# LariWa/Fractal-Image-Compression

Measured on AMD Instinct MI355X. Metric: range-block matches/sec (8x8 R, 16x16 D, 8 iso), higher is better.
Workload: dtype u8

## Files before the change

### fractal-image-compression_amd/capi.py

```python
import ctypes as C
import os
import sys
import re

import numpy as np

_HERE = os.path.dirname(os.path.abspath(__file__))
SO_PATH = os.path.join(_HERE, "libfic_hip.so")
HEADER_PATH = os.path.join(os.path.dirname(_HERE), "include", "fic.h")

FIC_OK = 0
ERROR_NAMES = {
    -1: "FIC_E_GEOMETRY", -2: "FIC_E_WINDOW", -3: "FIC_E_ARGUMENT", -4: "FIC_E_NO_DEVICE",
    -5: "FIC_E_HIP", -6: "FIC_E_NOT_GREY", -7: "FIC_E_STATE", -8: "FIC_E_CAPACITY",
}


class FicError(Exception):

    def __init__(self, code, message):
        super().__init__(f"{ERROR_NAMES.get(code, code)}: {message}")
        self.code = code


def declared_symbols():
    text = open(HEADER_PATH).read()
    return sorted(set(re.findall(r"FIC_API\s+[\w\s\*]+?\b(fic_\w+)\s*\(", text)))


_lib = None


def _torch_first():
    t = sys.modules.get("torch")
    if t is not None:
        try:
            if t.cuda.is_available():
                t.cuda.init()
        except Exception:
            pass


def lib():
    global _lib
    if _lib is not None:
        return _lib
    so = os.environ.get("FIC_HIP_SO") or SO_PATH
    if not os.path.exists(so):
        raise FicError(-5, f"{so} is missing: build it with __graft_entry__.build() "
                           "(hipcc --offload-arch=gfx950); there is no fallback path")
    _torch_first()
    L = C.CDLL(so)
    vp, ip = C.c_void_p, C.POINTER(C.c_int)
    i32p, f32p, u8p = C.POINTER(C.c_int32), C.POINTER(C.c_float), C.POINTER(C.c_uint8)
    sig = {
        "fic_version": (C.c_char_p, []),
        "fic_last_error": (C.c_char_p, []),
        "fic_last_error_code": (C.c_int, []),
        "fic_device_count": (C.c_int, []),
        "fic_geometry": (C.c_int, [C.c_int, C.c_int, C.c_int, ip, ip, ip, ip]),
        "fic_is_greyscale_argb": (C.c_int, [i32p, C.c_int, C.c_int]),
        "fic_encode_gray_argb": (C.c_int, [i32p] + [C.c_int] * 6 + [i32p, f32p, f32p, i32p, i32p]),
        "fic_encode_gray_u8": (C.c_int, [u8p] + [C.c_int] * 6 + [i32p, f32p, f32p, i32p, i32p]),
        "fic_encode_gray_argb_multi": (C.c_int, [i32p] + [C.c_int] * 6 + [i32p, f32p, f32p, i32p, i32p]),
        "fic_encode_gray_u8_multi": (C.c_int, [u8p] + [C.c_int] * 6 + [i32p, f32p, f32p, i32p, i32p]),
        "fic_write_run_gray": (C.c_int64, [i32p, C.c_int, C.c_int, C.c_int, C.c_int, C.c_int, u8p, C.c_int64]),
        "fic_ctx_create": (vp, [C.c_int] * 7),
        "fic_ctx_destroy": (None, [vp]),
        "fic_ctx_set_gray_host": (C.c_int, [vp, u8p]),
        "fic_ctx_set_argb_host": (C.c_int, [vp, i32p]),
        "fic_ctx_set_gray_device": (C.c_int, [vp, vp]),
        "fic_ctx_encode": (C.c_int, [vp, C.c_int, C.c_int, vp]),
        "fic_ctx_sync": (C.c_int, [vp]),
        "fic_ctx_get_results_host": (C.c_int, [vp, i32p, f32p, f32p, i32p, i32p, i32p, f32p]),
        "fic_ctx_result_device_ptrs": (C.c_int, [vp] + [C.POINTER(vp)] * 7),
        "fic_ctx_records_device_ptr": (C.c_int, [vp, C.POINTER(vp)]),
        "fic_ctx_collage_host": (C.c_int, [vp, i32p]),
        "fic_encode_rgb_argb": (C.c_int, [i32p] + [C.c_int] * 5 + [i32p, f32p, f32p, f32p, f32p, i32p, i32p]),
        "fic_rgb_ctx_create": (vp, [C.c_int] * 6),
        "fic_encode_rgb_iso_argb": (C.c_int, [i32p] + [C.c_int] * 6 + [i32p, f32p, f32p, f32p, f32p, i32p, i32p, i32p]),
        "fic_rgb_ctx_create_iso": (vp, [C.c_int] * 7),
        "fic_rgb_ctx_get_iso_host": (C.c_int, [vp, i32p]),
        "fic_rgb_ctx_destroy": (None, [vp]),
        "fic_rgb_ctx_set_argb_host": (C.c_int, [vp, i32p]),
        "fic_rgb_ctx_set_argb_device": (C.c_int, [vp, vp]),
        "fic_rgb_ctx_encode": (C.c_int, [vp, C.c_int, vp]),
        "fic_rgb_ctx_sync": (C.c_int, [vp]),
        "fic_rgb_ctx_set_option": (C.c_int, [vp, C.c_char_p, C.c_int]),
        "fic_rgb_ctx_last_sweep": (C.c_int, [vp]),
        "fic_rgb_ctx_get_results_host": (C.c_int, [vp, i32p, f32p, f32p, f32p, f32p, i32p, i32p]),
        "fic_rgb_ctx_decode_host": (C.c_int, [vp, i32p, f32p, ip]),
        "fic_write_run_rgb": (C.c_int64, [i32p, C.c_int, C.c_int, C.c_int, C.c_int, C.c_int, u8p, C.c_int64]),
        "fic_decode_gray_run": (C.c_int, [u8p, C.c_int64, C.c_int, u8p, C.c_int64, ip, ip, f32p, ip]),
        "fic_ctx_decode_host": (C.c_int, [vp, u8p, f32p, ip]),
        "fic_ctx_set_option": (C.c_int, [vp, C.c_char_p, C.c_int]),
        "fic_ctx_sweep_time": (C.c_int, [vp, C.POINTER(C.c_double), ip, C.c_int]),
        "fic_ctx_info": (C.c_int, [vp, ip]),
        "fic_sweep_ranges_per_pool_read": (C.c_int, [C.c_int, C.c_int, C.c_int]),
        "fic_ctx_last_kernel": (C.c_int, [vp, C.c_char_p, C.c_int]),
        "fic_ctx_sweep_stats": (C.c_int, [vp, C.POINTER(C.c_uint64), C.c_int]),
        "fic_debug_rccl_selftest": (C.c_int, [C.c_int]),
        "fic_debug_gather_fallbacks": (C.c_int, []),
        "fic_debug_float_sum": (C.c_int, [C.c_int, C.c_float, C.POINTER(C.c_uint32), C.c_int, f32p]),
        "fic_debug_float_sum_fallbacks": (C.c_int, []),
        "fic_debug_decode_gray_run": (C.c_int, [u8p, C.c_int64, C.c_int, u8p, C.c_int64, f32p, ip, ip]),
        "fic_debug_sqrt_f64": (C.c_int, [C.c_int, C.c_uint32, C.c_uint32, C.POINTER(C.c_double)]),
        "fic_ctx_debug_pool_host": (C.c_int, [vp, u8p, C.POINTER(C.c_uint32), C.POINTER(C.c_uint32), u8p]),
        "fic_ctx_debug_q_host": (C.c_int, [vp, C.c_int, vp, C.c_int64, C.POINTER(C.c_int64)]),
        "fic_rgb_ctx_debug_q_host": (C.c_int, [vp, C.c_int, vp, C.c_int64, C.POINTER(C.c_int64)]),
        "fic_rgb_ctx_last_kernel": (C.c_int, [vp, C.c_char_p, C.c_int]),
        "fic_rgb_ctx_sweep_stats": (C.c_int, [vp, C.POINTER(C.c_uint64), C.c_int]),
        "fic_encode_gray_quadtree_u8": (C.c_int, [u8p] + [C.c_int] * 6 + [C.c_float, C.c_int, i32p, C.c_int64, ip]),
        "fic_encode_gray_quadtree_argb": (C.c_int, [i32p] + [C.c_int] * 6 + [C.c_float, C.c_int, i32p, C.c_int64, ip]),
        "fic_write_run_quadtree": (C.c_int64, [i32p] + [C.c_int] * 7 + [u8p, C.c_int64]),
        "fic_decode_quadtree_run": (C.c_int, [u8p, C.c_int64, C.c_int, u8p, C.c_int64, ip, ip, f32p, ip]),
        "fic_debug_quadtree_sse": (C.c_int, [u8p] + [C.c_int] * 7 + [C.POINTER(C.c_uint32), C.c_int64]),
        "fic_encode_rgb_quadtree_argb": (C.c_int, [i32p] + [C.c_int] * 5 + [C.c_float, C.c_int, i32p, C.c_int64, ip]),
        "fic_write_run_rgb_quadtree": (C.c_int64, [i32p] + [C.c_int] * 6 + [u8p, C.c_int64]),
        "fic_decode_rgb_quadtree_run": (C.c_int, [u8p, C.c_int64, C.c_int, i32p, C.c_int64, ip, ip, f32p, ip]),
        "fic_debug_rgb_quadtree_sse": (C.c_int, [i32p] + [C.c_int] * 6 + [C.POINTER(C.c_uint32), C.c_int64]),
        "fic_decode_gray_run_zoom": (C.c_int, [u8p, C.c_int64, C.c_int, C.c_int, u8p, C.c_int64, ip, ip, f32p, ip]),
        "fic_decode_rgb_run_zoom": (C.c_int, [u8p, C.c_int64, C.c_int, C.c_int, i32p, C.c_int64, ip, ip, f32p, ip]),
        "fic_decode_quadtree_run_zoom": (C.c_int, [u8p, C.c_int64, C.c_int, C.c_int, u8p, C.c_int64, ip, ip, f32p, ip]),
        "fic_decode_rgb_quadtree_run_zoom": (C.c_int, [u8p, C.c_int64, C.c_int, C.c_int, i32p, C.c_int64, ip, ip, f32p, ip]),
        "fic_ctx_decode_zoom_host": (C.c_int, [vp, C.c_int, u8p, f32p, ip]),
    }
    for name, (res, args) in sig.items():
        fn = getattr(L, name)
        fn.restype = res
        fn.argtypes = args
    _lib = L
    return L


def has_xcheck():
    so = os.environ.get("FIC_HIP_SO") or SO_PATH
    if not os.path.exists(so):
        return False
    return b"+xcheck" in lib().fic_version()


def last_error():
    return lib().fic_last_error().decode("utf-8", "replace")


def check(rc):
    if rc < 0:
        raise FicError(rc, last_error())
    return rc


def ptr(a, t):
    return None if a is None else a.ctypes.data_as(C.POINTER(t))


def geometry(w, h, B):
    v = [C.c_int() for _ in range(4)]
    check(lib().fic_geometry(w, h, B, *[C.byref(x) for x in v]))
    return tuple(x.value for x in v)


def _decode_run_zoom(fn, run, header_bytes, what, dtype, device, avg_error_in, zoom):
    buf = np.frombuffer(bytes(run), np.uint8)
    if buf.size < header_bytes:
        raise FicError(-3, f"{what} shorter than its header")
    z = int(zoom)
    w = int.from_bytes(bytes(run[4:8]), "big", signed=True)
    h = int.from_bytes(bytes(run[8:12]), "big", signed=True)
    cap = max(w, 0) * max(h, 0) * (z * z if z in (1, 2, 4) else 1)
    if cap >= 2 ** 31:
        cap = 0
    out = np.zeros(max(cap, 1), dtype)
    avg = C.c_float(avg_error_in)
    it, wo, ho = C.c_int(), C.c_int(), C.c_int()
    check(fn(ptr(buf, C.c_uint8), buf.size, z, device, ptr(out, C.c_uint8 if dtype == np.uint8 else C.c_int32), cap, C.byref(wo),
             C.byref(ho), C.byref(avg), C.byref(it)))
    return out[:cap], np.float32(avg.value), it.value, wo.value, ho.value


def decode_gray_run(run, device=0, avg_error_in=0.0, zoom=1):
    if zoom != 1:
        out, avg, it, w, h = _decode_run_zoom(lib().fic_decode_gray_run_zoom, run, 20, "run stream", np.uint8, device, avg_error_in, zoom)
        return out.reshape(h, w), avg, it
    buf = np.frombuffer(bytes(run), np.uint8)
    if buf.size < 20:
        raise FicError(-3, "run stream shorter than its header")
    w = int.from_bytes(bytes(run[4:8]), "big", signed=True)
    h = int.from_bytes(bytes(run[8:12]), "big", signed=True)
    cap = max(w, 0) * max(h, 0)
    out = np.zeros(max(cap, 1), np.uint8)
    avg = C.c_float(avg_error_in)
    it, wo, ho = C.c_int(), C.c_int(), C.c_int()
    check(lib().fic_decode_gray_run(ptr(buf, C.c_uint8), buf.size, device, ptr(out, C.c_uint8), cap, C.byref(wo),
                                    C.byref(ho), C.byref(avg), C.byref(it)))
    return out[:cap].reshape(h, w), np.float32(avg.value), it.value


def encode_gray_oneshot(gray, B, wK, n_iso=1, device=0):
    g = np.ascontiguousarray(gray, np.uint8)
    h, w = g.shape
    Rw, Rh, Dw, Dh = geometry(w, h, B)
    nr = Rw * Rh
    r = {"idx_local": np.zeros(nr, np.int32), "a": np.zeros(nr, np.float32), "b": np.zeros(nr, np.float32),
         "iso": np.zeros(nr, np.int32), "qrows": np.zeros((nr, 3), np.int32)}
    check(lib().fic_encode_gray_u8(ptr(g, C.c_uint8), w, h, B, Dw if wK is None else wK, n_iso, device,
                                   ptr(r["idx_local"], C.c_int32), ptr(r["a"], C.c_float), ptr(r["b"], C.c_float),
                                   ptr(r["iso"], C.c_int32), ptr(r["qrows"], C.c_int32)))
    return r


def encode_gray_multi(gray, B, wK, n_iso=1, n_gpus=1, width=None, height=None):
    if width is not None:
        g = np.ascontiguousarray(gray, np.int32).reshape(-1)
        w, h = int(width), int(height)
        if g.size != w * h:
            raise FicError(-3, "argb has the wrong number of pixels")
        fn, p = lib().fic_encode_gray_argb_multi, ptr(g, C.c_int32)
    else:
        g = np.ascontiguousarray(gray, np.uint8)
        h, w = g.shape
        fn, p = lib().fic_encode_gray_u8_multi, ptr(g, C.c_uint8)
    Rw, Rh, Dw, Dh = geometry(w, h, B)
    nr = Rw * Rh
    r = {"idx_local": np.zeros(nr, np.int32), "a": np.zeros(nr, np.float32), "b": np.zeros(nr, np.float32),
         "iso": np.zeros(nr, np.int32), "qrows": np.zeros((nr, 3), np.int32)}
    check(fn(p, w, h, B, Dw if wK is None else wK, n_iso, n_gpus, ptr(r["idx_local"], C.c_int32), ptr(r["a"], C.c_float),
             ptr(r["b"], C.c_float), ptr(r["iso"], C.c_int32), ptr(r["qrows"], C.c_int32)))
    return r


def release_cache():
    lib().fic_release_cache.restype = None
    lib().fic_release_cache()


def decode_rgb_run(run, device=0, avg_error_in=0.0, zoom=1):
    L = lib()
    if zoom != 1:
        return _decode_run_zoom(L.fic_decode_rgb_run_zoom, run, 20, "run stream", np.int32, device, avg_error_in, zoom)
    L.fic_decode_rgb_run.restype = C.c_int
    L.fic_decode_rgb_run.argtypes = [C.POINTER(C.c_uint8), C.c_int64, C.c_int, C.POINTER(C.c_int32), C.c_int64,
                                     C.POINTER(C.c_int), C.POINTER(C.c_int), C.POINTER(C.c_float), C.POINTER(C.c_int)]
    buf = np.frombuffer(bytes(run), np.uint8)
    if buf.size < 20:
        raise FicError(-3, "run stream shorter than its header")
    w = int.from_bytes(bytes(run[4:8]), "big", signed=True)
    h = int.from_bytes(bytes(run[8:12]), "big", signed=True)
    cap = max(w, 0) * max(h, 0)
    out = np.zeros(max(cap, 1), np.int32)
    avg = C.c_float(avg_error_in)
    it, wo, ho = C.c_int(), C.c_int(), C.c_int()
    check(L.fic_decode_rgb_run(ptr(buf, C.c_uint8), buf.size, device, ptr(out, C.c_int32), cap, C.byref(wo), C.byref(ho),
                               C.byref(avg), C.byref(it)))
    return out[:cap], np.float32(avg.value), it.value, w, h


def encode_rgb(argb, w, h, B, wK, device=0, want_collage=False, n_iso=1):
    Rw, Rh, Dw, Dh = geometry(w, h, B)
    nr = Rw * Rh
    argb = np.ascontiguousarray(argb, np.int32).reshape(-1)
    if argb.size != w * h:
        raise FicError(-3, "argb has the wrong number of pixels")
    r = {"idx_local": np.zeros(nr, np.int32), "a": np.zeros(nr, np.float32), "bR": np.zeros(nr, np.float32),
         "bG": np.zeros(nr, np.float32), "bB": np.zeros(nr, np.float32), "iso": np.zeros(nr, np.int32),
         "qrows": np.zeros((nr, 5), np.int32)}
    col = np.zeros(w * h, np.int32) if want_collage else None
    check(lib().fic_encode_rgb_iso_argb(ptr(argb, C.c_int32), w, h, B, wK, n_iso, device, ptr(r["idx_local"], C.c_int32),
                                        ptr(r["a"], C.c_float), ptr(r["bR"], C.c_float), ptr(r["bG"], C.c_float),
                                        ptr(r["bB"], C.c_float), ptr(r["iso"], C.c_int32), ptr(r["qrows"], C.c_int32),
                                        ptr(col, C.c_int32)))
    if want_collage:
        r["collage"] = col
    return r


class RgbEncoder:

    def __init__(self, width, height, B, wK, planes=1, device=0, n_iso=1):
        L = lib()
# ... 236 lines not shown
```

### fractal-image-compression_amd/csrc/fic_capi.cpp

```cpp
#include "fic_internal.h"

namespace ficd {

thread_local std::string g_err;
thread_local int g_err_code = 0;

int fail(int code, const char* fmt, ...)
{
    char buf[512];
    va_list ap;
    va_start(ap, fmt);
    vsnprintf(buf, sizeof(buf), fmt, ap);
    va_end(ap);
    g_err = buf;
    g_err_code = code;
    return code;
}

int check_device(int device)
{
    int ndev = fic_device_count();
    if (ndev <= 0 || device < 0 || device >= ndev) return fail(FIC_E_NO_DEVICE, "no HIP device %d (this library has no CPU path)", device);
    HIP_TRY(hipSetDevice(device));
    return FIC_OK;
// ... 183 lines not shown
    nchunks = (g.Nd + chunk_len - 1) / chunk_len;
    if (fic_launch_sweep_fast(c->b, g, tile0, ntiles, chunk_len, nchunks, s)) return fail(FIC_E_HIP, "k_sweep_fast launch failed");
    *nchunks_out = nchunks;
    return FIC_OK;
}

int d4_available(const FicGeom& g) { return g.full && g.n_iso == 8 && g.NR == 1 && fic_d4_words(g.B) > 0; }
int d4_prep(fic_ctx* c, hipStream_t s)
{
    const FicGeom& g = c->g;
    const size_t NW = (size_t)fic_d4_words(g.B), P = (size_t)g.planes;
    if (!c->d4_rng) HIP_TRY(hipMalloc((void**)&c->d4_rng, P * g.tiles * NW * 64 * 4));
    if (!c->d4_pool) HIP_TRY(hipMalloc((void**)&c->d4_pool, P * g.Nd_pad * NW * 4));
    if (fic_launch_d4_prep(c->b, c->d4_rng, c->d4_pool, g, s)) return fail(FIC_E_HIP, "k_range_d4 / k_pool_d4 launch failed");
    return FIC_OK;
}
int d4_sweep(fic_ctx* c, int tile0, int ntiles, hipStream_t s, int* nchunks_out)
{
    const FicGeom& g = c->g;
    int nchunks = valu_chunk_count(c, (long long)ntiles * g.planes);
    const int chunk_len = (g.Nd + nchunks - 1) / nchunks;
    nchunks = (g.Nd + chunk_len - 1) / chunk_len;
    if (fic_launch_sweep_d4(c->b, c->d4_rng, c->d4_pool, g, tile0, ntiles, chunk_len, nchunks, s))
        return fail(FIC_E_HIP, "k_sweep_d4 launch failed");
    *nchunks_out = nchunks;
    return FIC_OK;
}

#ifdef FIC_BUILD_XCHECK
struct MatrixCoreShape {
    bool iso8;
    bool bf16;
    int steps;
    int ndtiles, ndtiles_alloc;
    int nctiles_alloc;
    int G8, ngroups8;
    int ct1;
};
MatrixCoreShape matrix_core_shape(const FicGeom& g, int kind)
{
    MatrixCoreShape m;
    m.iso8 = g.n_iso == 8;
    m.bf16 = kind == 3 && (g.B <= 8 || g.n_iso == 8);
    m.steps = m.bf16 ? fic_bf16_steps(g.B) : (g.n <= 32 ? 1 : g.n / 32);
    m.ndtiles = (g.Nd + 31) / 32;
    m.ndtiles_alloc = m.ndtiles + 1;
    m.nctiles_alloc = g.Nr_pad / 32 + 32;
    m.G8 = m.bf16 ? fic_bf16_group8(g.B) : fic_mfma8_group(g.B);
    m.ngroups8 = (g.Nr_pad + m.G8 - 1) / m.G8;
    m.ct1 = m.bf16 ? fic_bf16_ct1(g.B) : fic_mfma1_ct(g.B);
    return m;
}
int matrix_core_prep(fic_ctx* c, int kind, hipStream_t s)
{
    const FicGeom& g = c->g;
    const MatrixCoreShape m = matrix_core_shape(g, kind);
    const size_t P = (size_t)g.planes;
    if ((c->mfma_poolB || c->mfma_rngA || c->mfma_sw || c->mfma_rconst) && c->mfma_bf16 != (int)m.bf16) {
        HIP_TRY(hipStreamSynchronize(s));
        void* old[] = {c->mfma_poolB, c->mfma_rngA, c->mfma_sw, c->mfma_rconst};
        for (void* p : old) if (p) (void)hipFree(p);
        c->mfma_poolB = c->mfma_rngA = c->mfma_sw = nullptr;
        c->mfma_rconst = nullptr;
    }
    {
        c->mfma_bf16 = (int)m.bf16;
        const size_t rtiles = m.iso8 ? (size_t)m.ngroups8 * (m.G8 / 4) : (size_t)m.nctiles_alloc;
        if (!c->mfma_poolB) HIP_TRY(hipMalloc(&c->mfma_poolB, P * m.ndtiles_alloc * m.steps * 64 * 16));
        if (!c->mfma_rngA) HIP_TRY(hipMalloc(&c->mfma_rngA, P * rtiles * m.steps * 64 * 16));
        if (!c->mfma_sw) HIP_TRY(hipMalloc(&c->mfma_sw, P * m.ndtiles_alloc * 32 * 8));
        if (!m.bf16 && !c->mfma_rconst)
            HIP_TRY(hipMalloc((void**)&c->mfma_rconst, m.iso8 ? P * rtiles * 16 * sizeof(int) : P * rtiles * 32 * 16));
    }
    if (m.bf16) {
        const int rtiles = m.iso8 ? m.ngroups8 * (m.G8 / 4) : m.nctiles_alloc;
        if (fic_launch_bf16_prep(c->b, c->mfma_poolB, c->mfma_sw, c->mfma_rngA, g, m.ndtiles_alloc, rtiles, s))
            return fail(FIC_E_HIP, "bf16 fragment prep launch failed");
    } else if (m.iso8) {
        if (fic_launch_mfma_prep_pool(c->b.pool_pix, c->mfma_poolB, g, m.ndtiles_alloc, s) ||
            fic_launch_mfma_prep_range(c->b.rng_pix, c->b.rng_st, c->mfma_rngA, c->mfma_rconst, g, m.ngroups8, s))
            return fail(FIC_E_HIP, "mfma prep launch failed");
    } else if (fic_launch_mfma1_prep(c->b, c->mfma_poolB, c->mfma_sw, c->mfma_rngA, c->mfma_rconst, g, m.ndtiles_alloc,
                                     m.nctiles_alloc, s)) {
        return fail(FIC_E_HIP, "mfma1 prep launch failed");
    }
    return FIC_OK;
}
int matrix_core_sweep(fic_ctx* c, int kind, int tile0, int tile1, hipStream_t s, int* nchunks_out)
{
    const FicGeom& g = c->g;
    const MatrixCoreShape m = matrix_core_shape(g, kind);
    const int tsz = 64 * g.NR;
    int nchunks = c->opt_chunks;
    if (nchunks <= 0) {
        const long long ranges = (long long)(tile1 - tile0) * tsz;
        const long long per_wg = m.iso8 ? m.G8 : 32LL * m.ct1;
        const long long base_wg = (ranges + per_wg - 1) / per_wg * g.planes;
        long long want = (4096 + base_wg - 1) / base_wg;
        long long cap = m.ndtiles / 256;
        if (cap < 1) cap = 1;
        long long nc = want < cap ? want : cap;
        if (base_wg * nc < 1024) {
            long long cap2 = m.ndtiles / 32;
            if (cap2 < 1) cap2 = 1;
            long long fill = (1024 + base_wg - 1) / base_wg;
            nc = fill < cap2 ? fill : cap2;
        }
        nchunks = (int)(nc < 1 ? 1 : nc);
    }
    if (nchunks > m.ndtiles) nchunks = m.ndtiles;
    const int tiles_per_chunk = (m.ndtiles + nchunks - 1) / nchunks;
    nchunks = (m.ndtiles + tiles_per_chunk - 1) / tiles_per_chunk;
    if (m.iso8) {
        const int g0 = (tile0 * tsz) / m.G8, g1 = (tile1 * tsz + m.G8 - 1) / m.G8;
        const int rc = m.bf16 ? fic_launch_sweep_bf16(c->b, c->mfma_poolB, c->mfma_sw, c->mfma_rngA, g, m.ngroups8 * (m.G8 / 4), g0,
                                                      g1 - g0, m.ndtiles, m.ndtiles_alloc, tiles_per_chunk, nchunks, s)
                              : fic_launch_sweep_mfma(c->b, c->mfma_poolB, c->mfma_rngA, c->mfma_rconst, g, m.ngroups8, g0,
                                                      g1 - g0, m.ndtiles, m.ndtiles_alloc, tiles_per_chunk, nchunks, s);
        if (rc) return fail(FIC_E_HIP, "8-isometry matrix-core sweep launch failed");
    } else {
        const int ct_begin = tile0 * (tsz / 32), ct_end = tile1 * (tsz / 32);
        const int rc = m.bf16 ? fic_launch_sweep_bf16_1(c->b, c->mfma_poolB, c->mfma_sw, c->mfma_rngA, g, ct_begin, ct_end,
                                                        m.ndtiles, m.ndtiles_alloc, m.nctiles_alloc, tiles_per_chunk, nchunks, s)
                              : fic_launch_sweep_mfma1(c->b, c->mfma_poolB, c->mfma_sw, c->mfma_rngA, c->mfma_rconst, g, ct_begin,
                                                       ct_end, m.ndtiles, m.ndtiles_alloc, m.nctiles_alloc, tiles_per_chunk,
                                                       nchunks, s);
        if (rc) return fail(FIC_E_HIP, "1-isometry matrix-core sweep launch failed");
    }
    *nchunks_out = nchunks;
    return FIC_OK;
}

#else
int matrix_core_prep(fic_ctx*, int, hipStream_t) { return fail(FIC_E_ARGUMENT, "sweep 3 / 4 (cross-check kernels) are not in this build (FIC_BUILD_XCHECK=0)"); }
int matrix_core_sweep(fic_ctx*, int, int, int, hipStream_t, int*) { return fail(FIC_E_ARGUMENT, "sweep 3 / 4 (cross-check kernels) are not in this build (FIC_BUILD_XCHECK=0)"); }
#endif
struct QShape {
    int ndtiles, ndtiles_alloc;
    int unroll;
    int CT;
    int nct_alloc;
};
QShape q_shape(const FicGeom& g)
{
    QShape q;
    q.ndtiles = (g.Nd + 31) / 32;
    q.unroll = fic_q_unroll(g.B, g.n_iso);
    q.ndtiles_alloc = q.ndtiles + 2 * q.unroll;
    q.CT = fic_q_ct(g.B);
    const int nct = g.Nr_pad * fic_q_cols_per_range(g.B, g.n_iso) / 32;
    q.nct_alloc = (nct + q.CT - 1) / q.CT * q.CT + q.CT;
    return q;
}
int q_prep(fic_ctx* c, int tile0, int tile1, hipStream_t s)
{
    const FicGeom& g = c->g;
    const QShape q = q_shape(g);
    const size_t P = (size_t)g.planes, NK = (size_t)g.n / 16;
    if (!c->q_pool) HIP_TRY(hipMalloc(&c->q_pool, P * q.ndtiles_alloc * NK * 64 * 16));
    if (!c->q_flat) HIP_TRY(hipMalloc(&c->q_flat, P * q.ndtiles_alloc * sizeof(uint32_t)));
    if (!c->q_rng) {
        HIP_TRY(hipMalloc(&c->q_rng, P * q.nct_alloc * NK * 64 * 16));
        HIP_TRY(hipMemsetAsync(c->q_rng, 0, P * q.nct_alloc * NK * 64 * 16, s));
    }
    if (!c->q_rngC) HIP_TRY(hipMalloc(&c->q_rngC, P * g.Nr_pad * fic_q_cols_per_range(g.B, g.n_iso) * g.n));
    if (!c->q_E) HIP_TRY(hipMalloc(&c->q_E, P * g.Nr_pad * sizeof(float)));
    if (!c->q_thg) HIP_TRY(hipMalloc(&c->q_thg, (P * g.Nr_pad + (size_t)2 * q.CT * 32 + 64) * sizeof(uint32_t)));
    const int tsz = 64 * g.NR;
    const int grp0 = tile0 * tsz / 64, grp1 = tile1 * tsz / 64;
    if (fic_launch_q_prep(c->b, c->q_pool, c->q_flat, c->q_rng, c->q_rngC, c->q_E, c->q_thg, g, q.ndtiles_alloc, q.nct_alloc, grp0, grp1 - grp0, s))
        return fail(FIC_E_HIP, "k_pool_q / k_range_q launch failed");
    return FIC_OK;
}
int q_sweep(fic_ctx* c, int tile0, int tile1, hipStream_t s, int* nchunks_out, bool fused_fin = false, int r_begin = 0, int r_count = 0)
{
    const FicGeom& g = c->g;
    const QShape q = q_shape(g);
    const int tsz = 64 * g.NR;
    const int cpr = fic_q_cols_per_range(g.B, g.n_iso);
    const int ct_begin = tile0 * tsz * cpr / 32, ct_end = tile1 * tsz * cpr / 32;
    int nchunks = c->opt_chunks;
    if (nchunks <= 0) {
        const long long base_wg = (long long)((ct_end - ct_begin + q.CT - 1) / q.CT) * g.planes;
        const long long resident = 256LL * fic_q_resident(g.B);
        auto ceil_div = [](long long a, long long b) { return (a + b - 1) / b; };
        const long long min_tiles = g.n_iso == 8 ? 30 : 14;
        long long fill = base_wg < resident ? ceil_div(2 * resident, base_wg) : 1;
        if (fill > q.ndtiles / min_tiles) fill = q.ndtiles / min_tiles;
        long long bal = ceil_div(8 * resident, base_wg);
        if (bal > q.ndtiles / 1024) bal = q.ndtiles / 1024;
        const long long nc = fill > bal ? fill : bal;
        nchunks = (int)(nc < 1 ? 1 : nc);
    }
    if (nchunks > q.ndtiles) nchunks = q.ndtiles;
    int tiles_per_chunk = (q.ndtiles + nchunks - 1) / nchunks;
    tiles_per_chunk = (tiles_per_chunk + q.unroll - 1) / q.unroll * q.unroll;
    nchunks = (q.ndtiles + tiles_per_chunk - 1) / tiles_per_chunk;
    if (fused_fin && !c->q_fin) {
        const size_t nfin = (size_t)g.planes * (q.nct_alloc / q.CT + 1);
        HIP_TRY(hipMalloc((void**)&c->q_fin, nfin * sizeof(unsigned int)));
        HIP_TRY(hipMemsetAsync(c->q_fin, 0, nfin * sizeof(unsigned int), s));
    }
    if (fic_launch_sweep_q(c->b, c->q_pool, c->q_flat, c->q_rng, c->q_rngC, c->q_E, c->q_thg, g, ct_begin, ct_end, q.ndtiles, q.ndtiles_alloc,
                           q.nct_alloc, tiles_per_chunk, nchunks, s, c->q_stats, c->opt_noflag, fused_fin ? &c->o : nullptr, c->q_fin,
                           r_begin, r_count))
        return fail(FIC_E_HIP, "k_sweep_q launch failed");
    *nchunks_out = nchunks;
    c->last_tiles_per_chunk = tiles_per_chunk;
    return FIC_OK;
}

}

extern "C" {

#ifdef FIC_BUILD_XCHECK
const char* fic_version(void) { return "fic-hip 0.3 (gfx950, +xcheck sweeps)"; }
#else
const char* fic_version(void) { return "fic-hip 0.3 (gfx950)"; }
#endif
const char* fic_last_error(void) { return g_err.c_str(); }
int fic_last_error_code(void) { return g_err_code; }

int fic_device_count(void)
{
    int n = 0;
    if (hipGetDeviceCount(&n) != hipSuccess) return 0;
    return n;
}

int fic_geometry(int w, int h, int B, int* Rw, int* Rh, int* Dw, int* Dh)
{
    FicGeom g;
    int rc = make_geometry(w, h, B, 1, 1, 1, &g);
    if (rc) return rc;
    if (Rw) *Rw = g.Rw;
    if (Rh) *Rh = g.Rh;
    if (Dw) *Dw = g.Dw;
    if (Dh) *Dh = g.Dh;
    return FIC_OK;
}

int fic_is_greyscale_argb(const int32_t* argb, int w, int h)
{
    if (!argb || w <= 0 || h <= 0) return fail(FIC_E_ARGUMENT, "fic_is_greyscale_argb: bad argument");
    size_t n = (size_t)w * h;
    for (size_t i = 0; i < n; i++) {
        int r = (argb[i] >> 16) & 0xff, g = (argb[i] >> 8) & 0xff, b = argb[i] & 0xff;
        if (r != g || g != b) return 0;
    }
    return 1;
}

int64_t fic_write_run_gray(const int32_t* qrows, int n_ranges, int w, int h, int B, int wK, uint8_t* out,
                           int64_t capacity)
{
    if (!qrows || !out || n_ranges < 0) return fail(FIC_E_ARGUMENT, "fic_write_run_gray: bad argument");
    int64_t need = 20 + 12 * (int64_t)n_ranges;
    if (capacity < need) return fail(FIC_E_CAPACITY, "fic_write_run_gray: need %lld bytes, have %lld", (long long)need, (long long)capacity);
    const int32_t hdr[5] = {0, w, h, B, wK};
    for (int i = 0; i < 5; i++) put_be32(out + 4 * i, hdr[i]);
    uint8_t* p = out + 20;
    for (int64_t i = 0; i < 3 * (int64_t)n_ranges; i++, p += 4) put_be32(p, qrows[i]);
    return need;
}

fic_ctx* fic_ctx_create(int device, int w, int h, int B, int wK, int n_iso, int planes)
{
    FicGeom g;
    if (make_geometry(w, h, B, wK, n_iso, planes, &g)) return nullptr;
    int ndev = fic_device_count();
    if (ndev <= 0) { fail(FIC_E_NO_DEVICE, "no HIP device visible (this library has no CPU path)"); return nullptr; }
    if (device < 0 || device >= ndev) { fail(FIC_E_NO_DEVICE, "device %d out of range (0..%d)", device, ndev - 1); return nullptr; }
    if (hipSetDevice(device) != hipSuccess) { fail(FIC_E_HIP, "hipSetDevice(%d) failed", device); return nullptr; }
    fic_ctx* c = new fic_ctx();
    c->device = device;
    c->g = g;
    memset(&c->b, 0, sizeof(c->b));
    memset(&c->o, 0, sizeof(c->o));
    const size_t P = (size_t)planes;
    int rc = FIC_OK;
    auto A = [&](int r) { if (rc == FIC_OK) rc = r; };
    A(dev_alloc(&c->b.scaled, P * g.Ws * g.Hs));
    A(dev_alloc(&c->b.pool_pix, P * g.Nd_pad * g.n));
    A(dev_alloc(&c->b.pool_st, P * g.Nd_pad));
    A(dev_alloc(&c->b.pool_var, P * g.Nd_pad));
    A(dev_alloc(&c->b.pool_s64, P * g.Nd_pad));
    A(dev_alloc(&c->b.rng_st, P * g.Nr_pad));
    A(dev_alloc(&c->b.key, P * g.Nr_pad));
    A(dev_alloc(&c->o.idx_local, P * g.Nr));
    A(dev_alloc(&c->o.idx_global, P * g.Nr));
    A(dev_alloc(&c->o.iso, P * g.Nr));
    A(dev_alloc(&c->o.a, P * g.Nr));
    A(dev_alloc(&c->o.b, P * g.Nr));
    A(dev_alloc(&c->o.err, P * g.Nr));
    A(dev_alloc(&c->o.qrows, P * g.Nr * 3));
    A(dev_alloc(&c->o.records, P * g.Nr * 6));
    if (rc == FIC_OK) {
        hipError_t e = hipMemset(c->b.pool_pix, 0, P * g.Nd_pad * g.n);
        if (e == hipSuccess) e = hipMemset(c->b.pool_st, 0, P * g.Nd_pad * sizeof(FicDomStat));
        if (e == hipSuccess) e = hipMemset(c->b.pool_var, 0, P * g.Nd_pad * sizeof(uint32_t));
        if (e == hipSuccess) e = hipMemset(c->b.pool_s64, 0, P * g.Nd_pad * sizeof(double));
        if (e == hipSuccess) e = hipStreamSynchronize(nullptr);
        if (e != hipSuccess) rc = fail(FIC_E_HIP, "hipMemset: %s", hipGetErrorString(e));
    }
    if (rc != FIC_OK) {
        ctx_free_all(c);
        delete c;
        return nullptr;
    }
    return c;
}

void fic_ctx_destroy(fic_ctx* c)
{
    if (!c) return;
    (void)hipSetDevice(c->device);
    (void)hipDeviceSynchronize();
    ctx_free_all(c);
    delete c;
}

int fic_ctx_set_gray_host(fic_ctx* c, const uint8_t* gray)
{
    if (!c || !gray) return fail(FIC_E_ARGUMENT, "fic_ctx_set_gray_host: null argument");
    std::lock_guard<std::mutex> lk(c->mu);
    HIP_TRY(hipSetDevice(c->device));
    size_t bytes = (size_t)c->g.planes * c->g.W * c->g.H;
    if (!c->gray_own) { int rc = dev_alloc(&c->gray_own, bytes); if (rc) return rc; }
    HIP_TRY(hipStreamSynchronize(c->last_stream));
    HIP_TRY(hipMemcpy(c->gray_own, gray, bytes, hipMemcpyHostToDevice));
    c->b.gray = c->gray_own;
    c->have_input = true;
    return FIC_OK;
}

int fic_ctx_set_argb_host(fic_ctx* c, const int32_t* argb)
{
    if (!c || !argb) return fail(FIC_E_ARGUMENT, "fic_ctx_set_argb_host: null argument");
    std::lock_guard<std::mutex> lk(c->mu);
    HIP_TRY(hipSetDevice(c->device));
    size_t npix = (size_t)c->g.planes * c->g.W * c->g.H;
    if (!c->gray_own) { int rc = dev_alloc(&c->gray_own, npix); if (rc) return rc; }
    if (!c->argb_stage) { int rc = dev_alloc(&c->argb_stage, npix); if (rc) return rc; }
    HIP_TRY(hipStreamSynchronize(c->last_stream));
    HIP_TRY(hipMemcpy(c->argb_stage, argb, npix * sizeof(int32_t), hipMemcpyHostToDevice));
    if (fic_launch_argb_to_gray(c->argb_stage, c->gray_own, npix, nullptr)) return fail(FIC_E_HIP, "k_argb_to_gray launch failed");
    HIP_TRY(hipStreamSynchronize(nullptr));
    c->b.gray = c->gray_own;
    c->have_input = true;
    return FIC_OK;
}

int fic_ctx_set_gray_device(fic_ctx* c, const void* dev_gray)
{
    if (!c || !dev_gray) return fail(FIC_E_ARGUMENT, "fic_ctx_set_gray_device: null argument");
    std::lock_guard<std::mutex> lk(c->mu);
    c->b.gray = (uint8_t*)dev_gray;
    c->have_input = true;
    return FIC_OK;
}

int fic_ctx_encode(fic_ctx* c, int range_begin, int range_count, void* hip_stream)
{
    if (!c) return fail(FIC_E_ARGUMENT, "fic_ctx_encode: null context");
    std::lock_guard<std::mutex> lk(c->mu);
    if (!c->have_input) return fail(FIC_E_STATE, "fic_ctx_encode: no input image set");
    const FicGeom& g = c->g;
    if (range_count < 0) range_count = g.Nr - range_begin;
    if (range_begin < 0 || range_count < 0 || range_begin + range_count > g.Nr)
        return fail(FIC_E_ARGUMENT, "fic_ctx_encode: range span [%d,%d) outside 0..%d", range_begin, range_begin + range_count, g.Nr);
    HIP_TRY(hipSetDevice(c->device));
    hipStream_t s = (hipStream_t)hip_stream;
    c->last_stream = s;
    if (range_count == 0) return FIC_OK;

    int kind = c->opt_sweep;
    if (kind == 0) {
        const long long pairs = (long long)g.planes * range_count * g.Nd;
        const int valu = d4_available(g) ? 5 : 2;
        kind = !g.full ? 1 : ((pairs >= 2000000LL && g.Nd < (1 << 24)) ? 6 : valu);
        const char* env = getenv("FIC_SWEEP");
        if (env && env[0] >= '2' && env[0] <= '6' && env[1] == '\0' && g.full) {
            const int want = env[0] - '0';
            kind = want == 5 ? valu : want;
        }
    }
    if (kind >= 2 && !g.full) return fail(FIC_E_ARGUMENT, "fast sweep needs full search (wK == Dw == Dh)");
#ifndef FIC_BUILD_XCHECK
    if (kind == 3 || kind == 4) return fail(FIC_E_ARGUMENT, "sweep %d (cross-check kernel) is not in this build (FIC_BUILD_XCHECK=0)", kind);
#endif
    if (kind == 5 && !d4_available(g)) return fail(FIC_E_ARGUMENT, "sweep 5 (k_sweep_d4) needs full search, n_iso = 8 and B = 8");
    if (kind == 6 && g.Nd >= (1 << 24)) return fail(FIC_E_ARGUMENT, "sweep 6 (k_sweep_q) needs a pool of fewer than 2^24 blocks");
    const int tsz = 64 * g.NR;
    const int tile0 = range_begin / tsz;
    const int tile1 = (range_begin + range_count + tsz - 1) / tsz;
    const int ntiles = tile1 - tile0;
    int nchunks = 1;
    int rc = FIC_OK;
    bool fused_prep = false;
    if (kind == 6) {
        const QShape q = q_shape(g);
        fused_prep = fic_q_prep_fused(g, q.ndtiles_alloc, tile1 * (64 * g.NR) / 64 - tile0 * (64 * g.NR) / 64) != 0;
    }
    if (!fused_prep && fic_launch_scale(c->b.gray, c->b.scaled, g, s)) return fail(FIC_E_HIP, "k_scale launch failed");
    if (kind == 6) {
        rc = q_prep(c, tile0, tile1, s);
    } else {
        if (fic_launch_pool(c->b.scaled, c->b.pool_pix, c->b.pool_st, c->b.pool_var, c->b.pool_s64, g, s))
            return fail(FIC_E_HIP, "k_pool launch failed");
        if (kind != 5 && !c->b.rng_pix) {
            int rca = dev_alloc(&c->b.rng_pix, (size_t)g.planes * g.Nr_pad * g.n_iso * g.DW);
            if (rca) return rca;
        }
        if (fic_launch_range(c->b.gray, c->b.rng_pix, c->b.rng_st, g, s, kind == 5 ? 0 : 1)) return fail(FIC_E_HIP, "k_range launch failed");
        HIP_TRY(hipMemset2DAsync(c->b.key + (size_t)tile0 * tsz, (size_t)g.Nr_pad * sizeof(unsigned long long), 0xFF,
                                 (size_t)ntiles * tsz * sizeof(unsigned long long), (size_t)g.planes, s));
        if (kind == 5) rc = d4_prep(c, s);
        else if (kind >= 3) rc = matrix_core_prep(c, kind, s);
    }
    if (rc == FIC_OK) rc = time_begin(c, s);
    if (rc == FIC_OK) {
        if (kind == 1) {
            if (fic_launch_sweep_generic(c->b, g, range_begin, range_count, s)) rc = fail(FIC_E_HIP, "k_sweep_generic launch failed");
        } else if (kind == 6) {
            rc = q_sweep(c, tile0, tile1, s, &nchunks, fused_prep, range_begin, range_count);
        } else if (kind == 5) {
            rc = d4_sweep(c, tile0, tile1 - tile0, s, &nchunks);
        } else if (kind >= 3) {
            rc = matrix_core_sweep(c, kind, tile0, tile1, s, &nchunks);
        } else {
            rc = valu_sweep(c, tile0, tile1 - tile0, s, &nchunks);
        }
    }
    if (rc == FIC_OK) rc = time_end(c, s);
    if (rc != FIC_OK) return rc;
    c->last_chunks = nchunks;
    c->last_kind = kind;
    c->last_fused = fused_prep ? 1 : 0;
    if (!fused_prep &&
        fic_launch_finalize(c->b, c->o, g, range_begin, range_count, s, (kind == 5 || kind == 6) ? 1 : 0)) return fail(FIC_E_HIP, "k_finalize launch failed");
    c->encoded_any = true;
    return FIC_OK;
}

int fic_ctx_sync(fic_ctx* c)
{
    if (!c) return fail(FIC_E_ARGUMENT, "fic_ctx_sync: null context");
    HIP_TRY(hipSetDevice(c->device));
    HIP_TRY(hipStreamSynchronize(c->last_stream));
    return FIC_OK;
}

int fic_ctx_get_results_host(fic_ctx* c, int32_t* idx_local, float* a, float* b, int32_t* iso, int32_t* qrows,
                             int32_t* idx_global, float* err)
{
    if (!c) return fail(FIC_E_ARGUMENT, "fic_ctx_get_results_host: null context");
    if (!c->encoded_any) return fail(FIC_E_STATE, "fic_ctx_get_results_host: nothing encoded yet");
    HIP_TRY(hipSetDevice(c->device));
    HIP_TRY(hipStreamSynchronize(c->last_stream));
    size_t n = (size_t)c->g.planes * c->g.Nr;
    if (n > (size_t)65536) {
        if (idx_local) HIP_TRY(hipMemcpy(idx_local, c->o.idx_local, n * 4, hipMemcpyDeviceToHost));
        if (a) HIP_TRY(hipMemcpy(a, c->o.a, n * 4, hipMemcpyDeviceToHost));
        if (b) HIP_TRY(hipMemcpy(b, c->o.b, n * 4, hipMemcpyDeviceToHost));
        if (iso) HIP_TRY(hipMemcpy(iso, c->o.iso, n * 4, hipMemcpyDeviceToHost));
        if (qrows) HIP_TRY(hipMemcpy(qrows, c->o.qrows, n * 12, hipMemcpyDeviceToHost));
    } else if (idx_local || a || b || iso || qrows) {
        std::lock_guard<std::mutex> lk(c->mu);
        if (!c->host_rec) HIP_TRY(hipHostMalloc((void**)&c->host_rec, n * 6 * sizeof(int32_t), hipHostMallocDefault));
        HIP_TRY(hipMemcpy(c->host_rec, c->o.records, n * 6 * sizeof(int32_t), hipMemcpyDeviceToHost));
        const int32_t* r = c->host_rec;
        for (size_t i = 0; i < n; i++, r += 6) {
            if (idx_local) idx_local[i] = r[0];
            if (a) memcpy(&a[i], &r[1], 4);
            if (b) memcpy(&b[i], &r[2], 4);
            if (iso) iso[i] = r[3];
            if (qrows) { qrows[3 * i] = r[0]; qrows[3 * i + 1] = r[4]; qrows[3 * i + 2] = r[5]; }
        }
    }
    if (idx_global) HIP_TRY(hipMemcpy(idx_global, c->o.idx_global, n * 4, hipMemcpyDeviceToHost));
    if (err) HIP_TRY(hipMemcpy(err, c->o.err, n * 4, hipMemcpyDeviceToHost));
    return FIC_OK;
}

int fic_ctx_result_device_ptrs(fic_ctx* c, void** idx_local, void** a, void** b, void** iso, void** qrows,
                               void** idx_global, void** err)
{
    if (!c) return fail(FIC_E_ARGUMENT, "fic_ctx_result_device_ptrs: null context");
    if (idx_local) *idx_local = c->o.idx_local;
    if (a) *a = c->o.a;
    if (b) *b = c->o.b;
    if (iso) *iso = c->o.iso;
    if (qrows) *qrows = c->o.qrows;
    if (idx_global) *idx_global = c->o.idx_global;
    if (err) *err = c->o.err;
    return FIC_OK;
}

int fic_ctx_records_device_ptr(fic_ctx* c, void** records)
{
    if (!c || !records) return fail(FIC_E_ARGUMENT, "fic_ctx_records_device_ptr: null argument");
    *records = c->o.records;
    return FIC_OK;
}

int fic_ctx_collage_host(fic_ctx* c, int32_t* argb_out)
{
    if (!c || !argb_out) return fail(FIC_E_ARGUMENT, "fic_ctx_collage_host: null argument");
    std::lock_guard<std::mutex> lk(c->mu);
    if (!c->encoded_any) return fail(FIC_E_STATE, "fic_ctx_collage_host: nothing encoded yet");
    HIP_TRY(hipSetDevice(c->device));
    size_t npix = (size_t)c->g.planes * c->g.W * c->g.H;
    if (!c->collage) { int rc = dev_alloc(&c->collage, npix); if (rc) return rc; }
    if (fic_launch_collage(c->b, c->o, c->collage, c->g, c->last_stream)) return fail(FIC_E_HIP, "k_collage launch failed");
    HIP_TRY(hipStreamSynchronize(c->last_stream));
    HIP_TRY(hipMemcpy(argb_out, c->collage, npix * sizeof(int32_t), hipMemcpyDeviceToHost));
    return FIC_OK;
}

int fic_ctx_set_option(fic_ctx* c, const char* name, int value)
{
    if (!c || !name) return fail(FIC_E_ARGUMENT, "fic_ctx_set_option: null argument");
    if (!strcmp(name, "sweep")) {
        if (value < 0 || value > 6)
            return fail(FIC_E_ARGUMENT, "sweep must be 0 (auto), 1 (generic), 2 (fast, VALU), 3 (matrix-core, exact covariances), 4 (matrix-core, i8 operands), 5 (VALU, group-Fourier isometries) or 6 (matrix-core, normalised f16 prune GEMM)");
        c->opt_sweep = value;
    } else if (!strcmp(name, "chunks")) {
        if (value < 0) return fail(FIC_E_ARGUMENT, "chunks must be >= 0");
        c->opt_chunks = value;
    } else if (!strcmp(name, "q_shape")) {
        if (value < 0 || value > 2) return fail(FIC_E_ARGUMENT, "q_shape must be 0 (by pool size), 1 (16x16x32) or 2 (32x32x16)");
        c->g.q_shape = value;
    } else if (!strcmp(name, "q_eshift")) {
        if (value < -12 || value > 4) return fail(FIC_E_ARGUMENT, "q_eshift must be in -12..4");
        c->g.q_eshift = value;
    } else if (!strcmp(name, "q_noflag")) {
        c->opt_noflag = value ? 1 : 0;
    } else if (!strcmp(name, "time_sweep")) {
        c->opt_time = value ? 1 : 0;
    } else if (!strcmp(name, "sweep_stats")) {
        HIP_TRY(hipSetDevice(c->device));
        if (value && !c->q_stats) {
            HIP_TRY(hipMalloc((void**)&c->q_stats, 8 * sizeof(unsigned long long)));
            HIP_TRY(hipMemset(c->q_stats, 0, 8 * sizeof(unsigned long long)));
            HIP_TRY(hipStreamSynchronize(nullptr));
        } else if (!value && c->q_stats) {
            HIP_TRY(hipStreamSynchronize(c->last_stream));
            (void)hipFree(c->q_stats);
            c->q_stats = nullptr;
        }
    } else {
        return fail(FIC_E_ARGUMENT, "unknown option '%s'", name);
    }
    return FIC_OK;
}

int fic_ctx_sweep_time(fic_ctx* c, double* total_ms, int* launches, int reset)
{
    if (!c) return fail(FIC_E_ARGUMENT, "fic_ctx_sweep_time: null context");
    std::lock_guard<std::mutex> lk(c->mu);
    HIP_TRY(hipSetDevice(c->device));
    int rc = flush_events(c);
    if (rc) return rc;
    if (total_ms) *total_ms = c->acc_ms;
    if (launches) *launches = c->acc_n;
    if (reset) { c->acc_ms = 0.0; c->acc_n = 0; }
    return FIC_OK;
}

int fic_ctx_sweep_stats(fic_ctx* c, uint64_t* out8, int reset)
{
    if (!c || !out8) return fail(FIC_E_ARGUMENT, "fic_ctx_sweep_stats: null argument");
    std::lock_guard<std::mutex> lk(c->mu);
    if (!c->q_stats) return fail(FIC_E_STATE, "fic_ctx_sweep_stats: set the option \"sweep_stats\" first");
    HIP_TRY(hipSetDevice(c->device));
    HIP_TRY(hipStreamSynchronize(c->last_stream));
    HIP_TRY(hipMemcpy(out8, c->q_stats, 8 * sizeof(uint64_t), hipMemcpyDeviceToHost));
    if (reset) {
        HIP_TRY(hipMemset(c->q_stats, 0, 8 * sizeof(uint64_t)));
        HIP_TRY(hipStreamSynchronize(nullptr));
    }
    return FIC_OK;
}

int fic_ctx_info(fic_ctx* c, int* out10)
{
    if (!c || !out10) return fail(FIC_E_ARGUMENT, "fic_ctx_info: null argument");
    const FicGeom& g = c->g;
    int v[10] = {g.Rw, g.Rh, g.Nr, g.Dw, g.Dh, g.Nd, g.NR, g.tiles, c->last_chunks, c->last_kind};
    memcpy(out10, v, sizeof(v));
    return FIC_OK;
}

int fic_ctx_last_kernel(fic_ctx* c, char* out, int capacity)
{
    if (!c || !out || capacity < 1) return fail(FIC_E_ARGUMENT, "fic_ctx_last_kernel: bad argument");
    const FicGeom& g = c->g;
    const int NK = g.n / 16, kind = c->last_kind;
    const char* multi = c->last_chunks > 1 ? "true" : "false";
    const bool shorts = kind == 6 && fic_q_multi_kind(c->last_chunks, c->last_tiles_per_chunk) == 2;
    char buf[96];
    if (kind == 6 && fic_q_shape16(g) && shorts) snprintf(buf, sizeof(buf), "k_sweep_q16s<%d>", NK);
    else if (kind == 6 && fic_q_shape16(g)) snprintf(buf, sizeof(buf), "k_sweep_q16<%d, %s>", NK, multi);
    else if (kind == 6 && shorts) snprintf(buf, sizeof(buf), "k_sweep_qs<%d, %d>", NK, g.n_iso == 1 ? 0 : (g.B == 4 ? 1 : 2));
    else if (kind == 6) snprintf(buf, sizeof(buf), "k_sweep_q<%d, %d, %s>", NK, g.n_iso == 1 ? 0 : (g.B == 4 ? 1 : 2), multi);
    else if (kind == 5) snprintf(buf, sizeof(buf), "k_sweep_d4");
    else if (kind == 2) snprintf(buf, sizeof(buf), "k_sweep_fast");
    else if (kind == 1) snprintf(buf, sizeof(buf), "k_sweep_generic");
    else if (kind == 3 || kind == 4) {
        const bool bf16 = kind == 3 && (g.B <= 8 || g.n_iso == 8);
        snprintf(buf, sizeof(buf), "%s%s", bf16 ? "k_sweep_bf16" : "k_sweep_mfma", g.n_iso == 8 ? "" : (bf16 ? "_1" : "1"));
    } else snprintf(buf, sizeof(buf), "(none)");
    snprintf(out, (size_t)capacity, "%s%s", buf, kind == 6 && c->last_fused ? " after k_prep_q8, finalising" : "");
    return FIC_OK;
}

int fic_sweep_ranges_per_pool_read(int kind, int B, int n_iso)
{
    if ((B != 4 && B != 8 && B != 16) || (n_iso != 1 && n_iso != 8)) return 0;
    if (kind == 6) return fic_q_ctw_host(B) * 32 / fic_q_cols_per_range(B, n_iso);
    if (kind == 2 || kind == 5) {
        int NR = 1, NC = 1;
        fic_fast_variant(B, n_iso, &NR, &NC);
        return 64 * (kind == 5 ? 1 : NR);
    }
    return 0;
}

int fic_debug_sqrt_f64(int device, uint32_t first, uint32_t count, double* out)
{
    if (!out || count == 0) return fail(FIC_E_ARGUMENT, "fic_debug_sqrt_f64: bad argument");
    int rc = check_device(device);
    if (rc) return rc;
    double* d = nullptr;
    HIP_TRY(hipMalloc((void**)&d, (size_t)count * sizeof(double)));
    if (fic_launch_sqrt_probe(d, first, count, nullptr)) rc = fail(FIC_E_HIP, "k_sqrt_probe launch failed");
    if (rc == FIC_OK) {
        hipError_t e = hipMemcpy(out, d, (size_t)count * sizeof(double), hipMemcpyDeviceToHost);
        if (e != hipSuccess) rc = fail(FIC_E_HIP, "hipMemcpy: %s", hipGetErrorString(e));
    }
    (void)hipFree(d);
    return rc;
}

int fic_ctx_debug_pool_host(fic_ctx* c, uint8_t* pix, uint32_t* sum, uint32_t* var, uint8_t* scaled)
{
    if (!c) return fail(FIC_E_ARGUMENT, "fic_ctx_debug_pool_host: null context");
    if (!c->encoded_any) return fail(FIC_E_STATE, "fic_ctx_debug_pool_host: nothing encoded yet");
    HIP_TRY(hipSetDevice(c->device));
    HIP_TRY(hipStreamSynchronize(c->last_stream));
    const FicGeom& g = c->g;
    for (int p = 0; p < g.planes; p++) {
        if (pix)
            HIP_TRY(hipMemcpy(pix + (size_t)p * g.Nd * g.n, c->b.pool_pix + (size_t)p * g.Nd_pad * g.n, (size_t)g.Nd * g.n,
                              hipMemcpyDeviceToHost));
        if (var)
            HIP_TRY(hipMemcpy(var + (size_t)p * g.Nd, c->b.pool_var + (size_t)p * g.Nd_pad, (size_t)g.Nd * 4,
                              hipMemcpyDeviceToHost));
        if (sum) {
            std::vector<FicDomStat> st(g.Nd);
            HIP_TRY(hipMemcpy(st.data(), c->b.pool_st + (size_t)p * g.Nd_pad, (size_t)g.Nd * sizeof(FicDomStat),
                              hipMemcpyDeviceToHost));
            for (int i = 0; i < g.Nd; i++) sum[(size_t)p * g.Nd + i] = st[i].sum;
        }
    }
    if (scaled) HIP_TRY(hipMemcpy(scaled, c->b.scaled, (size_t)g.planes * g.Ws * g.Hs, hipMemcpyDeviceToHost));
    return FIC_OK;
}

int fic_ctx_debug_q_host(fic_ctx* c, int which, void* out, int64_t capacity, int64_t* size)
{
    if (!c || !size) return fail(FIC_E_ARGUMENT, "fic_ctx_debug_q_host: null argument");
    if (!c->encoded_any || !c->q_pool) return fail(FIC_E_STATE, "fic_ctx_debug_q_host: no encode through the default sweep (\"sweep\" = 6) yet");
    const FicGeom& g = c->g;
    const QShape q = q_shape(g);
    const size_t P = (size_t)g.planes, NK = (size_t)g.n / 16;
    const void* src = nullptr;
    size_t bytes = 0;
    switch (which) {
    case 0: src = c->q_pool; bytes = P * q.ndtiles_alloc * NK * 64 * 16; break;
    case 1: src = c->q_flat; bytes = P * q.ndtiles_alloc * sizeof(uint32_t); break;
    case 2: src = c->q_rng; bytes = P * q.nct_alloc * NK * 64 * 16; break;
    case 3: src = c->q_E; bytes = P * g.Nr_pad * sizeof(float); break;
    case 4: src = c->b.rng_st; bytes = P * g.Nr_pad * sizeof(FicRngStat); break;
    case 5: src = c->q_rngC; bytes = P * g.Nr_pad * fic_q_cols_per_range(g.B, g.n_iso) * g.n; break;
    default: return fail(FIC_E_ARGUMENT, "fic_ctx_debug_q_host: which must be 0..5");
    }
    *size = (int64_t)bytes;
    if (!out) return FIC_OK;
    if (capacity < (int64_t)bytes) return fail(FIC_E_CAPACITY, "fic_ctx_debug_q_host: %zu bytes needed", bytes);
    HIP_TRY(hipSetDevice(c->device));
    HIP_TRY(hipStreamSynchronize(c->last_stream));
    HIP_TRY(hipMemcpy(out, src, bytes, hipMemcpyDeviceToHost));
    return FIC_OK;
}

}

int ficd::encode_oneshot(const uint8_t* gray, const int32_t* argb, int w, int h, int B, int wK, int n_iso, int device,
                          int32_t* idx_local, float* a, float* b, int32_t* iso, int32_t* qrows)
{
    if ((!gray && !argb) || !idx_local || !a || !b) return fail(FIC_E_ARGUMENT, "fic_encode_gray: null argument");
    fic_ctx* c = cache_take(device, w, h, B, wK, n_iso);
    if (!c) c = fic_ctx_create(device, w, h, B, wK, n_iso, 1);
    if (!c) return g_err_code ? g_err_code : FIC_E_HIP;
    int rc = gray ? fic_ctx_set_gray_host(c, gray) : fic_ctx_set_argb_host(c, argb);
    if (rc == FIC_OK) rc = fic_ctx_encode(c, 0, -1, nullptr);
    if (rc == FIC_OK) rc = fic_ctx_get_results_host(c, idx_local, a, b, iso, qrows, nullptr, nullptr);
    ErrKeep keep;
    if (rc == FIC_OK) cache_give(c);
    else fic_ctx_destroy(c);
    return rc;
}

extern "C" {

void fic_release_cache(void)
{
    std::vector<fic_ctx*> drop;
    {
        std::lock_guard<std::mutex> lk(g_cache_mu);
        drop.swap(g_cache);
    }
    for (fic_ctx* c : drop) fic_ctx_destroy(c);
    release_rgb_cache();
    release_comms();
    release_decoder_arenas();
}

int fic_encode_gray_argb(const int32_t* argb, int w, int h, int B, int wK, int n_iso, int device, int32_t* idx_local,
                         float* a, float* b, int32_t* iso, int32_t* qrows)
{
    return encode_oneshot(nullptr, argb, w, h, B, wK, n_iso, device, idx_local, a, b, iso, qrows);
}

int fic_encode_gray_u8(const uint8_t* gray, int w, int h, int B, int wK, int n_iso, int device, int32_t* idx_local,
                       float* a, float* b, int32_t* iso, int32_t* qrows)
{
    return encode_oneshot(gray, nullptr, w, h, B, wK, n_iso, device, idx_local, a, b, iso, qrows);
}

}
```

### fractal-image-compression_amd/csrc/fic_internal.h

```cpp
#pragma once
#include <hip/hip_runtime.h>
#include <stdarg.h>
#include <stdio.h>
#include <stdlib.h>
#include <string.h>
#include <functional>
#include <mutex>
#include <string>
#include <vector>

#include "../../include/fic.h"
#include "fic_device.h"
#include "fic_launch.h"

namespace ficd {

extern thread_local std::string g_err;
extern thread_local int g_err_code;
int fail(int code, const char* fmt, ...) __attribute__((format(printf, 2, 3)));

#define HIP_TRY(expr)                                                                              \
    do {                                                                                           \
        hipError_t e_ = (expr);                                                                    \
        if (e_ != hipSuccess) return ficd::fail(FIC_E_HIP, "%s: %s", #expr, hipGetErrorString(e_)); \
    } while (0)

struct ErrKeep {
    std::string msg = g_err;
    int code = g_err_code;
    ~ErrKeep() { g_err = msg; g_err_code = code; }
};

int make_geometry(int w, int h, int B, int wK, int n_iso, int planes, FicGeom* out);
int make_decode_geometry(int w, int h, int B, int wK, int n_iso, int planes, int zoom, FicGeom* out);

template <typename T>
int dev_alloc(T** p, size_t count)
{
    HIP_TRY(hipMalloc((void**)p, count * sizeof(T)));
    return FIC_OK;
}
inline size_t align256(size_t v) { return (v + 255) & ~(size_t)255; }

int check_device(int device);

inline void put_be32(uint8_t* p, int32_t v)
{
    uint32_t u = (uint32_t)v;
    p[0] = (uint8_t)(u >> 24); p[1] = (uint8_t)(u >> 16); p[2] = (uint8_t)(u >> 8); p[3] = (uint8_t)u;
}
inline int32_t get_be32(const uint8_t* p)
{
    return (int32_t)(((uint32_t)p[0] << 24) | ((uint32_t)p[1] << 16) | ((uint32_t)p[2] << 8) | (uint32_t)p[3]);
}

fic_ctx* cache_take(int device, int w, int h, int B, int wK, int n_iso);
void cache_give(fic_ctx* c);
int encode_oneshot(const uint8_t* gray, const int32_t* argb, int w, int h, int B, int wK, int n_iso, int device,
                   int32_t* idx_local, float* a, float* b, int32_t* iso, int32_t* qrows);

fic_rgb_ctx* rgb_cache_take(int device, int w, int h, int B, int wK, int n_iso = 1);
void rgb_cache_give(fic_rgb_ctx* c);
void rgb_ctx_views(const fic_rgb_ctx* c, const int32_t** argb, const int32_t** scaled, const int32_t** qrows5);

struct Arena {
    int device = -1;
    size_t bytes = 0;
    char* base = nullptr;
};
int arena_take(int device, size_t bytes, Arena* out);
void arena_give(const Arena& a);
struct DecodeKind {
    size_t px_bytes;
    uint32_t px_start;
    const char* name;
    const char* paint_line;
};
constexpr DecodeKind kDecodeGrey{1, 128u, "decode", "FC:394"}, kDecodeRgb{4, 0xff808080u, "decodeRGB", "FC:477"};
int decode_loop(const DecodeKind& kind, int planes, size_t npix, void* d_image, FicDecodeState* d_state, const float* avg_in,
                float* avg_out, int* iters_out, int* seq_out, hipStream_t s, const std::function<int(int)>& iteration);

void release_decoder_arenas();
void release_rgb_cache();
void release_comms();

}

struct fic_ctx {
    int device = 0;
    FicGeom g;
    FicBuffers b;
    FicOutputs o;
    uint8_t* gray_own = nullptr;
    int32_t* argb_stage = nullptr;
    int32_t* collage = nullptr;
    int32_t* host_rec = nullptr;
    uint8_t* decoded = nullptr;
    FicDecodeState* dec_state = nullptr;
    uint32_t* dec_sq = nullptr;
    void* mfma_poolB = nullptr;
    void* mfma_rngA = nullptr;
    void* mfma_sw = nullptr;
    int* mfma_rconst = nullptr;
    int mfma_bf16 = 0;
    void* q_pool = nullptr;
    void* q_flat = nullptr;
    void* q_rng = nullptr;
    void* q_rngC = nullptr;
    void* q_E = nullptr;
    void* q_thg = nullptr;
    unsigned int* q_fin = nullptr;
    unsigned long long* q_stats = nullptr;
    uint32_t* d4_rng = nullptr;
    uint32_t* d4_pool = nullptr;
    bool have_input = false;
    bool encoded_any = false;
    hipStream_t last_stream = nullptr;
    hipStream_t own_stream = nullptr;
    int opt_sweep = 0, opt_chunks = 0, opt_time = 0, opt_noflag = 0;
    int last_chunks = 0, last_kind = 0, last_fused = 0, last_tiles_per_chunk = 0;
    std::vector<hipEvent_t> ev;
    double acc_ms = 0.0;
    int acc_n = 0;
    std::mutex mu;
};
```

### fractal-image-compression_amd/csrc/fic_launch.h

```cpp
#pragma once
#include <hip/hip_runtime.h>
#include <stdint.h>
#include "fic_device.h"

struct FicBuffers {
    uint8_t* gray;
    uint8_t* scaled;
    uint8_t* pool_pix;
    FicDomStat* pool_st;
    uint32_t* pool_var;
    double* pool_s64;
    uint32_t* rng_pix;
    FicRngStat* rng_st;
    unsigned long long* key;
};

struct FicOutputs {
    int32_t* idx_local;
    int32_t* idx_global;
    int32_t* iso;
    float* a;
    float* b;
    float* err;
    int32_t* qrows;
    int32_t* records;
};

#ifdef __HIPCC__
#include "fic_devfn.h"
__device__ __forceinline__ void finalize_store(const FicOutputs& out, const FicGeom& g, int plane, int j, unsigned long long kk, int wloc,
                                               int gi, int k, uint32_t acc, FicDomStat ds, FicRngStat rs, uint32_t varu)
{
    int dM = (int)(ds.sum >> g.lgn);
    int cov = (int)acc - rs.rM * (int)ds.sum - dM * rs.rem;
    float var = (float)varu;
    float a = __fdiv_rn((float)cov, var);
    if (a < -1.0f) a = -1.0f;
    else if (a > 1.0f) a = 1.0f;
    float b = __fsub_rn((float)rs.rM, __fmul_rn(a, (float)dM));
    size_t o = (size_t)plane * g.Nr + j;
    const int qa = java_f2i(__fmul_rn(a, 100.0f)), qb = java_f2i(b);
    out.qrows[3 * o + 0] = wloc;
    out.qrows[3 * o + 1] = qa;
    out.qrows[3 * o + 2] = qb;
    if (a != a) a = __uint_as_float(0x7FC00000u);
    if (b != b) b = __uint_as_float(0x7FC00000u);
    out.idx_local[o] = wloc;
    out.idx_global[o] = gi;
    out.iso[o] = k;
    out.a[o] = a;
    out.b[o] = b;
    out.err[o] = f32_from_orderable((uint32_t)(kk >> 32));
    int32_t* rec = out.records + 6 * o;
    rec[0] = wloc;
    rec[1] = (int32_t)__float_as_uint(a);
    rec[2] = (int32_t)__float_as_uint(b);
    rec[3] = k;
    rec[4] = qa;
    rec[5] = qb;
}
#endif

int fic_launch_argb_to_gray(const int32_t* argb, uint8_t* gray, size_t npix, hipStream_t s);
int fic_launch_scale(const uint8_t* gray, uint8_t* scaled, const FicGeom& g, hipStream_t s);
int fic_launch_pool(const uint8_t* scaled, uint8_t* pool_pix, FicDomStat* st, uint32_t* var, double* s64,
                    const FicGeom& g, hipStream_t s);
int fic_launch_range(const uint8_t* gray, uint32_t* rng_pix, FicRngStat* rst, const FicGeom& g, hipStream_t s,
                     int with_copies = 1);
int fic_launch_sweep_generic(const FicBuffers& b, const FicGeom& g, int r_begin, int r_count, hipStream_t s);
int fic_fast_variant(int B, int n_iso, int* NR, int* NC);
int fic_launch_sweep_fast(const FicBuffers& b, const FicGeom& g, int tile0, int ntiles, int chunk_len, int nchunks,
                          hipStream_t s);
int fic_launch_finalize(const FicBuffers& b, const FicOutputs& out, const FicGeom& g, int r_begin, int r_count,
                        hipStream_t s, int from_gray = 0);
int fic_launch_collage(const FicBuffers& b, const FicOutputs& out, int32_t* collage, const FicGeom& g, hipStream_t s);
int fic_launch_sqrt_probe(double* out, uint32_t first, uint32_t count, hipStream_t s);

struct FicRgbOutputs {
    int32_t* idx_local;
    int32_t* idx_global;
    float* a;
    float* bR;
    float* bG;
    float* bB;
    int32_t* qrows;
    int32_t* iso = nullptr;
};
struct FicRgbBuffers {
    int32_t* argb;
    int32_t* scaled;
    uint16_t* pool_sum;
    float* pool_cf;
    FicRgbDomStat* pool_st;
    int16_t* rng_t;
    FicRgbRngStat* rng_st;
    unsigned long long* key;
};
struct FicRgbQ {
    void *poolQ = nullptr, *dflat = nullptr, *rngQ = nullptr, *qst = nullptr, *rngE = nullptr, *theta_g = nullptr, *amax = nullptr;
    int ndtiles = 0, ndtiles_alloc = 0, nct_alloc = 0, tiles_per_chunk = 0, nchunks = 0;
    unsigned long long* stats = nullptr;
};
int fic_launch_rgb_encode(const FicRgbBuffers& b, const FicRgbOutputs& out, int32_t* collage, const FicGeom& g,
                          hipStream_t s, const FicRgbQ* q = nullptr);
int fic_launch_rgbq(const uint16_t* pool_sum, const FicRgbDomStat* pool_st, const int16_t* rng_t, const FicRgbRngStat* rng_st,
                    unsigned long long* key, void* poolQ, void* dflat, void* rngQ, void* qst, void* rngE, void* theta_g, void* amax,
                    const FicGeom& g, int ndtiles, int ndtiles_alloc, int nct_alloc, int tiles_per_chunk, int nchunks, hipStream_t s,
                    unsigned long long* stats = nullptr);

int fic_mfma8_group(int B);
int fic_launch_mfma_prep_pool(const uint8_t* pool_pix, void* poolB, const FicGeom& g, int ndtiles_alloc, hipStream_t s);
int fic_launch_mfma_prep_range(const uint32_t* rng_pix, const FicRngStat* rng_st, void* rngA, int* rconst,
                               const FicGeom& g, int ngroups, hipStream_t s);
int fic_launch_sweep_mfma(const FicBuffers& b, const void* poolB, const void* rngA, const int* rconst, const FicGeom& g,
                          int ngroups, int group0, int ngroups_launch, int ndtiles, int ndtiles_alloc, int tiles_per_chunk,
                          int nchunks, hipStream_t s);
int fic_mfma1_ct(int B);
int fic_launch_mfma1_prep(const FicBuffers& b, void* poolA, void* pool_sw, void* rngB, void* rconst, const FicGeom& g,
                          int ndtiles_alloc, int nctiles_alloc, hipStream_t s);
int fic_launch_sweep_mfma1(const FicBuffers& b, const void* poolA, const void* pool_sw, const void* rngB,
                           const void* rconst, const FicGeom& g, int ct_begin, int ct_end, int ndtiles, int ndtiles_alloc,
                           int nctiles_alloc, int tiles_per_chunk, int nchunks, hipStream_t s);
int fic_bf16_steps(int B);
int fic_bf16_group8(int B);
int fic_bf16_ct1(int B);
int fic_launch_bf16_prep(const FicBuffers& b, void* poolF, void* pool_w, void* rngF, const FicGeom& g, int ndtiles_alloc,
                         int nrtiles_alloc, hipStream_t s);
int fic_launch_sweep_bf16(const FicBuffers& b, const void* poolF, const void* pool_w, const void* rngF, const FicGeom& g,
                          int nrtiles_alloc, int group0, int ngroups_launch, int ndtiles, int ndtiles_alloc, int tiles_per_chunk, int nchunks,
                          hipStream_t s);
int fic_launch_sweep_bf16_1(const FicBuffers& b, const void* poolF, const void* pool_w, const void* rngF, const FicGeom& g,
                            int ct_begin, int ct_end, int ndtiles, int ndtiles_alloc, int nctiles_alloc, int tiles_per_chunk,
                            int nchunks, hipStream_t s);
int fic_d4_words(int B);
int fic_launch_d4_prep(const FicBuffers& b, uint32_t* rng_d4, uint32_t* pool_d4, const FicGeom& g, hipStream_t s);
int fic_launch_sweep_d4(const FicBuffers& b, const uint32_t* rng_d4, const uint32_t* pool_d4, const FicGeom& g, int tile0,
                        int ntiles, int chunk_len, int nchunks, hipStream_t s);
int fic_q_ct(int B);
int fic_q_ctw_host(int B);
int fic_q_prep_fused(const FicGeom& g, int ndtiles_alloc, int ngrp);
int fic_q_shape16(const FicGeom& g);
int fic_q_multi_kind(int nchunks, int tiles_per_chunk);
int fic_q_cols_per_range(int B, int n_iso);
int fic_q_unroll(int B, int n_iso);
int fic_q_resident(int B);
int fic_launch_q_prep(const FicBuffers& b, void* poolQ, void* dflat, void* rngQ, void* rngC, void* rngE, void* theta_g,
                      const FicGeom& g, int ndtiles_alloc, int nct_alloc, int grp0, int ngrp, hipStream_t s);
int fic_launch_sweep_q(const FicBuffers& b, const void* poolQ, const void* dflat, const void* rngQ, const void* rngC, const void* rngE,
                       void* theta_g, const FicGeom& g, int ct_begin, int ct_end, int ndtiles, int ndtiles_alloc,
                       int nct_alloc, int tiles_per_chunk, int nchunks, hipStream_t s, unsigned long long* stats = nullptr, int dbg_noflag = 0,
                       const FicOutputs* fin_out = nullptr, unsigned int* fin_count = nullptr, int r_begin = 0, int r_count = 0);
int fic_launch_decode_iteration_rgb(int32_t* scaled, int32_t* image, const int32_t* qrows5, FicDecodeState* state,
                                    uint32_t* sqbuf, int counter, const FicGeom& g, hipStream_t s,
                                    const int32_t* iso = nullptr);
int fic_launch_scale_rgb(const int32_t* argb, int32_t* scaled, const FicGeom& g, hipStream_t s);

int fic_launch_float_sum_probe(float carry, const uint32_t* vals, int count, uint32_t* maps, float* out2, hipStream_t s);
size_t fic_float_sum_map_words(size_t count);
size_t fic_decode_sq_words(size_t planes, size_t wh);
int fic_launch_decode_step(FicDecodeState* state, uint32_t* sqbuf, int counter, int wh, int planes, hipStream_t s);
int fic_launch_decode_iteration(uint8_t* scaled, uint8_t* image, const int32_t* qrows, const int32_t* iso,
                                FicDecodeState* state, uint32_t* sqbuf, int counter, const FicGeom& g, hipStream_t s);

struct QtGrey {
    using Px = uint8_t;
    static constexpr int QW = 3;
    static constexpr bool kIso = true;
    static constexpr int kLeafInts = 3 + QW + 1;
};
struct QtRgb {
    using Px = int32_t;
    static constexpr int QW = 5;
    static constexpr bool kIso = false;
    static constexpr int kLeafInts = 3 + QW;
};
struct FicQtLeaf {
    int32_t x, y, gi, sqoff, q[4];
};
template <typename Fmt>
int fic_launch_leaf_sse(const typename Fmt::Px* image, const typename Fmt::Px* scaled, const int32_t* qrows, const int32_t* iso,
                        uint32_t* sse, const FicGeom& g, hipStream_t s);
template <typename Fmt>
int fic_launch_qt_compact(const uint32_t* const* sse, const int32_t* const* qrows, const int32_t* const* iso, const int* Rw,
                          int nl, int B_max, int Rw_top, int Ntop, float threshold, int* counts, int* offs, int32_t* leaves,
                          hipStream_t s);
template <typename Fmt>
int fic_launch_decode_paint_leaves(const typename Fmt::Px* scaled, typename Fmt::Px* image, const FicQtLeaf* lv, int n,
                                   FicDecodeState* state, uint32_t* sqbuf, int counter, const FicGeom& g, hipStream_t s);
```

### fractal-image-compression_amd/csrc/fic_q.hip

```cpp
#include <hip/hip_runtime.h>
#include <stdint.h>
#include <math.h>
#include <string.h>
#include <stdlib.h>
#include <type_traits>
#include "fic_device.h"
#include "fic_launch.h"
#include "fic_devfn.h"

typedef int v4i __attribute__((ext_vector_type(4)));
typedef float v16f __attribute__((ext_vector_type(16)));
typedef _Float16 f16x8 __attribute__((ext_vector_type(8)));

#define FIC_Q_LEVEL 0.99999237060546875f
#define FIC_Q_TAU_ALL 3.0e38f
#define FIC_Q_TAU_NONE (-1.0f)
#define FIC_Q_LMIN 0.26f
#define FIC_Q_ECOEF 7.0e-4f
#define FIC_Q_EABS 1.6e-5f
#define FIC_Q_QCAP 1280
#define FIC_Q_QFLUSH 256

#ifndef FIC_Q_CTW_B8
#define FIC_Q_CTW_B8 4
#endif
#ifndef FIC_Q_CTW_B4
#define FIC_Q_CTW_B4 8
#endif
#ifndef FIC_Q_WPG
#define FIC_Q_WPG 4
#endif
#ifndef FIC_Q_WAVES_B8
#define FIC_Q_WAVES_B8 2
#endif
#ifndef FIC_Q_WAVES_B4
#define FIC_Q_WAVES_B4 3
#endif
__host__ __device__ constexpr int fic_q_ctw(int NK) { return NK == 4 ? FIC_Q_CTW_B8 : (NK < 4 ? FIC_Q_CTW_B4 : 2); }
#define FIC_Q_THG_NONE 0xBF800000u
#ifndef FIC_Q_GFAST_TILES
#define FIC_Q_GFAST_TILES 48
#endif
#ifndef FIC_Q_SEED
#define FIC_Q_SEED 1
#endif
#define FIC_Q_UNROLL 2

#ifndef FIC_Q_SHAPE16
#define FIC_Q_SHAPE16 1
#endif
__device__ __forceinline__ void frag_slot(int shape16, int NK, int s, int lane, int& row, int& p0)
{
    if (!shape16) {
        row = lane & 31;
        p0 = 16 * s + 8 * (lane >> 5);
    } else {
        const int KS = NK >> 1;
        row = 16 * (s / KS) + (lane & 15);
        p0 = 32 * (s % KS) + 8 * (lane >> 4);
    }
}

__device__ __forceinline__ float q_escale(const FicGeom& g) { return __int_as_float((127 - g.q_eshift) << 23); }

__device__ __forceinline__ int f16_pair(float lo, float hi)
{
    typedef _Float16 h2 __attribute__((ext_vector_type(2)));
    h2 v = {(_Float16)lo, (_Float16)hi};
    return __builtin_bit_cast(int, v);
}

template <int B, bool FUSE>
__device__ __forceinline__ void pool_q_body(int dtile, int plane, const uint8_t* __restrict__ scaled_in, const uint8_t* __restrict__ gray,
                                            uint8_t* __restrict__ scaled_out, uint8_t* __restrict__ pool_pix,
                                            FicDomStat* __restrict__ pool_st, uint32_t* __restrict__ pool_var,
                                            double* __restrict__ pool_s64, v4i* __restrict__ poolQ,
                                            uint32_t* __restrict__ dflat, const FicGeom& g, int ndtiles_alloc, int folded, int shape16)
{
    __shared__ __attribute__((aligned(16))) uint8_t pix[32][256 + 16];
    __shared__ int s_sum[32][16], s_sq[32][16];
    __shared__ float s_w[32];
    __shared__ int s_mean[32];
    __shared__ int s_nonflat;
    constexpr int n = B * B, NK = n / 16;
    if (threadIdx.x == 0) s_nonflat = 0;
    for (int t = threadIdx.x; t < 32 * B; t += 256) {
        const int i = t / B, ry = t % B;
        const int d = dtile * 32 + i;
        uint32_t w[B / 4];
#pragma unroll
        for (int q = 0; q < B / 4; q++) w[q] = 0u;
        if (d < g.Nd) {
            const int c = d % g.Dw, r = d / g.Dw;
            const size_t so = (size_t)plane * g.Ws * g.Hs + (size_t)(r * g.abstand + ry) * g.Ws + c * g.abstand;
            if constexpr (!FUSE) {
                __builtin_memcpy(w, scaled_in + so, B);
            } else {
                const int ys = r * g.abstand + ry, xs0 = c * g.abstand;
                const uint8_t* im = gray + (size_t)plane * g.W * g.H + (size_t)(2 * ys) * g.W + 2 * xs0;
                uint32_t top[B / 2], bot[B / 2];
                __builtin_memcpy(top, im, 2 * B);
                __builtin_memcpy(bot, im + g.W, 2 * B);
#pragma unroll
                for (int x = 0; x < B; x++) {
                    const uint32_t t2 = top[x >> 1] >> (16 * (x & 1)), b2 = bot[x >> 1] >> (16 * (x & 1));
                    const int tap4 = (2 * (xs0 + x) + 1 >= g.H) ? 128 : (int)((b2 >> 8) & 0xffu);
                    const int m = (int)(t2 & 0xffu) + (int)((t2 >> 8) & 0xffu) + (int)(b2 & 0xffu) + tap4;
                    w[x >> 2] |= (uint32_t)(m / 4) << (8 * (x & 3));
                }
                __builtin_memcpy(scaled_out + so, w, B);
            }
        }
        uint32_t sum = 0, sq = 0;
#pragma unroll
        for (int q = 0; q < B / 4; q++) {
            sum = __builtin_amdgcn_sad_u8(w[q], 0u, sum);
            sq = __builtin_amdgcn_udot4(w[q], w[q], sq, false);
            *(uint32_t*)&pix[i][ry * B + 4 * q] = w[q];
        }
        s_sum[i][ry] = (int)sum;
        s_sq[i][ry] = (int)sq;
    }
    __syncthreads();
    for (int t = threadIdx.x; t < 32 * n / 16; t += 256) {
        const int i = t / (n / 16), q = t % (n / 16);
        const int d = dtile * 32 + i;
        if (d < g.Nd) *(uint4*)(pool_pix + ((size_t)plane * g.Nd_pad + d) * n + 16 * q) = *(const uint4*)&pix[i][16 * q];
    }
    if (threadIdx.x < 32) {
        const int i = threadIdx.x, d = dtile * 32 + i;
        int S = 0, Q = 0;
        for (int t = 0; t < B; t++) { S += s_sum[i][t]; Q += s_sq[i][t]; }
        const int m = S >> g.lgn;
        const int var = Q - 2 * m * S + n * m * m;
        const double s64 = __dsqrt_rn((double)var);
        const float s32 = (float)s64;
        float w = 0.0f;
        if (d < g.Nd) {
            const size_t o = (size_t)plane * g.Nd_pad + d;
            FicDomStat st;
            st.sum = (uint32_t)S;
            st.s32 = s32;
            pool_st[o] = st;
            pool_var[o] = (uint32_t)var;
            pool_s64[o] = s64;
            if (var != 0) { w = __fdiv_rn(1.0f, s32); atomicOr(&s_nonflat, 1); }
        }
        s_w[i] = w;
        s_mean[i] = m;
    }
    __syncthreads();
    for (int t = threadIdx.x; t < NK * 64; t += 256) {
        const int lane = t & 63, m = t >> 6;
        int i, pos0;
        frag_slot(shape16, NK, m, lane, i, pos0);
        const int h = lane >> 5;
        const float w = s_w[i];
        const int dM = s_mean[i];
        v4i v;
        if (!folded) {
            const uint2 pw = *(const uint2*)&pix[i][pos0];
            int px[8];
#pragma unroll
            for (int u = 0; u < 8; u++) px[u] = (int)(((u < 4 ? pw.x : pw.y) >> (8 * (u & 3))) & 0xffu);
#pragma unroll
            for (int u = 0; u < 4; u++)
                v[u] = f16_pair(__fmul_rn((float)(px[2 * u] - dM), w), __fmul_rn((float)(px[2 * u + 1] - dM), w));
        } else {
            const bool odd = m >= NK / 2;
            const int p0 = 16 * (odd ? m - NK / 2 : m) + 8 * h;
            const uint2 pw = *(const uint2*)&pix[i][p0], qw = *(const uint2*)&pix[i][n - 8 - p0];
            float f[8];
#pragma unroll
            for (int u = 0; u < 8; u++) {
                const int a = (int)(((u < 4 ? pw.x : pw.y) >> (8 * (u & 3))) & 0xffu);
                const int b = (int)(((u < 4 ? qw.y : qw.x) >> (8 * (3 - (u & 3)))) & 0xffu);
                f[u] = __fmul_rn(__fmul_rn((float)(odd ? a - b : a + b - 2 * dM), w), 0.5f);
            }
#pragma unroll
            for (int u = 0; u < 4; u++) v[u] = f16_pair(f[2 * u], f[2 * u + 1]);
        }
        poolQ[((size_t)plane * ndtiles_alloc + dtile) * NK * 64 + t] = v;
    }
    if (threadIdx.x == 0) dflat[(size_t)plane * ndtiles_alloc + dtile] = s_nonflat ? 0u : 1u;
}
template <int B>
__global__ __launch_bounds__(256) void k_pool_q(const uint8_t* __restrict__ scaled, uint8_t* __restrict__ pool_pix,
                                                FicDomStat* __restrict__ pool_st, uint32_t* __restrict__ pool_var,
                                                double* __restrict__ pool_s64, v4i* __restrict__ poolQ,
                                                uint32_t* __restrict__ dflat, FicGeom g, int ndtiles_alloc, int folded, int shape16)
{
    pool_q_body<B, false>(blockIdx.x, blockIdx.y, scaled, nullptr, nullptr, pool_pix, pool_st, pool_var, pool_s64, poolQ, dflat, g,
                          ndtiles_alloc, folded, shape16);
}

__global__ __launch_bounds__(256) void k_range_q(const uint8_t* __restrict__ gray, FicRngStat* __restrict__ rng_st,
                                                 float* __restrict__ rngE, unsigned long long* __restrict__ key,
                                                 uint32_t* __restrict__ theta_g, v4i* __restrict__ rngQ,
                                                 uint32_t* __restrict__ rngC, FicGeom g, int nct_alloc, int grp0, int mode,
                                                 int staged, int shape16)
{
    __shared__ __attribute__((aligned(16))) uint8_t blk[64 * (256 + 4)];
    extern __shared__ __attribute__((aligned(16))) uint8_t cpy[];
    __shared__ int s_rM[64];
    const int plane = blockIdx.y;
    const int grp = grp0 + blockIdx.x;
    const int B = g.B, n = g.n, DW = g.DW, NK = n / 16;
    const int lgB = B == 4 ? 2 : (B == 8 ? 3 : 4);
    const int stride = n + 4;
    const int j0 = grp * 64;
    const uint8_t* img = gray + (size_t)plane * g.W * g.H;
    for (int i = threadIdx.x; i < 64 * DW; i += 256) {
        const int l = i / DW, wd = i % DW;
        const int j = j0 + l;
        uint32_t v = 0;
        if (j < g.Nr) {
            const int pos = wd * 4;
            const uint8_t* p = img + (size_t)((j / g.Rw) * B + (pos >> lgB)) * g.W + (j % g.Rw) * B + (pos & (B - 1));
            v = *(const uint32_t*)p;
        }
        *(uint32_t*)&blk[l * stride + wd * 4] = v;
    }
    __syncthreads();
    {
        const int l = threadIdx.x >> 2, part = threadIdx.x & 3;
        const uint32_t* w = (const uint32_t*)(blk + l * stride) + part * (DW / 4);
        uint32_t S = 0, Q = 0;
        for (int i = 0; i < DW / 4; i++) {
            S = __builtin_amdgcn_sad_u8(w[i], 0u, S);
            Q = __builtin_amdgcn_udot4(w[i], w[i], Q, false);
        }
        S += (uint32_t)__builtin_amdgcn_update_dpp(0, (int)S, 0xB1, 0xF, 0xF, true);
        Q += (uint32_t)__builtin_amdgcn_update_dpp(0, (int)Q, 0xB1, 0xF, 0xF, true);
        S += (uint32_t)__builtin_amdgcn_update_dpp(0, (int)S, 0x4E, 0xF, 0xF, true);
        Q += (uint32_t)__builtin_amdgcn_update_dpp(0, (int)Q, 0x4E, 0xF, 0xF, true);
        const int j = j0 + l;
        const int rM = (int)(S >> g.lgn);
        if (part == 0) {
            s_rM[l] = rM;
            if (j < g.Nr_pad) {
                const int ss = (int)Q - 2 * rM * (int)S + n * rM * rM;
                const size_t o = (size_t)plane * g.Nr_pad + j;
                FicRngStat st;
                st.rM = j < g.Nr ? rM : 0;
                st.rem = j < g.Nr ? (int)S - (rM << g.lgn) : 0;
                rng_st[o] = st;
                rngE[o] = __fmul_rn(__fadd_rn(__fmul_rn(__fsqrt_rn((float)ss), FIC_Q_ECOEF), FIC_Q_EABS), q_escale(g));
                key[o] = FIC_KEY_NONE;
                theta_g[o] = FIC_Q_THG_NONE;
            }
        }
    }
    __syncthreads();
    const int cpr = mode == 0 ? 1 : (mode == 1 ? 8 : 4);
    const int lgc = mode == 0 ? 0 : (mode == 1 ? 3 : 2);
    const int cols = 64 * cpr;
    const int ct0 = (j0 * cpr) / 32;
    const int cstride = n + 8;
    for (int t = threadIdx.x; t < cols * DW; t += 256) {
        const int col = t / DW, wd = t % DW;
        const int l = col >> lgc, c = col & (cpr - 1);
        if (j0 + l >= g.Nr_pad) break;
        const int k = mode == 2 ? (c == 0 ? 0 : (c == 1 ? 1 : (c == 2 ? 4 : 6))) : c;
        int ax, bx, cx, ay, by, cy;
        iso_affine(iso_inverse(k), B - 1, ax, bx, cx, ay, by, cy);
        const int s0 = cx + cy * B, sx = ax + ay * B, sy = bx + by * B;
        const uint8_t* b = blk + l * stride;
        uint32_t w = 0;
        if (k == 0) {
            w = *(const uint32_t*)(b + 4 * wd);
        } else {
#pragma unroll
            for (int u = 0; u < 4; u++) {
                const int p = 4 * wd + u;
                w |= (uint32_t)b[s0 + sx * (p & (B - 1)) + sy * (p >> lgB)] << (8 * u);
            }
        }
        rngC[((size_t)plane * g.Nr_pad * cpr + (size_t)j0 * cpr + col) * DW + wd] = w;
        if (staged) *(uint32_t*)(cpy + col * cstride + 4 * wd) = w;
    }
    if (staged) __syncthreads();
    for (int t = threadIdx.x; t < (cols / 32) * NK * 64; t += 256) {
        const int lane = t & 63, m = (t >> 6) % NK, ctl = (t >> 6) / NK;
        int c32, pos0;
        frag_slot(shape16, NK, m, lane, c32, pos0);
        const int col = ctl * 32 + c32, h = lane >> 5;
        const int l = col >> lgc, c = col & (cpr - 1);
        const int rM = s_rM[l];
        const bool real = j0 + l < g.Nr;
        int a[8];
        if (staged) {
            const uint8_t* cp = cpy + col * cstride;
            if (mode != 2) {
                const uint2 w = *(const uint2*)(cp + pos0);
#pragma unroll
                for (int u = 0; u < 8; u++) a[u] = (int)(((u < 4 ? w.x : w.y) >> (8 * (u & 3))) & 0xffu) - rM;
            } else {
                const bool odd = m >= NK / 2;
                const int q0 = 16 * (odd ? m - NK / 2 : m) + 8 * h;
                const uint2 w = *(const uint2*)(cp + q0), v = *(const uint2*)(cp + n - 8 - q0);
#pragma unroll
                for (int u = 0; u < 8; u++) {
                    const int c0 = (int)(((u < 4 ? w.x : w.y) >> (8 * (u & 3))) & 0xffu);
                    const int c1 = (int)(((u < 4 ? v.y : v.x) >> (8 * (3 - (u & 3)))) & 0xffu);
                    a[u] = odd ? c0 - c1 : c0 + c1 - 2 * rM;
                }
            }
        } else {
            const int k = mode == 2 ? (c == 0 ? 0 : (c == 1 ? 1 : (c == 2 ? 4 : 6))) : c;
            int ax, bx, cx, ay, by, cy;
            iso_affine(iso_inverse(k), B - 1, ax, bx, cx, ay, by, cy);
            const int s0 = cx + cy * B, sx = ax + ay * B, sy = bx + by * B;
            const uint8_t* b = blk + l * stride;
            if (mode != 2) {
                const int p0 = pos0;
#pragma unroll
                for (int u = 0; u < 8; u++) {
                    const int p = p0 + u;
                    a[u] = (int)b[s0 + sx * (p & (B - 1)) + sy * (p >> lgB)] - rM;
                }
            } else {
                const bool odd = m >= NK / 2;
                const int q0 = 16 * (odd ? m - NK / 2 : m) + 8 * h;
#pragma unroll
                for (int u = 0; u < 8; u++) {
                    const int p = q0 + u, pr = n - 1 - p;
                    const int c0 = b[s0 + sx * (p & (B - 1)) + sy * (p >> lgB)], c1 = b[s0 + sx * (pr & (B - 1)) + sy * (pr >> lgB)];
                    a[u] = odd ? c0 - c1 : c0 + c1 - 2 * rM;
                }
            }
        }
        v4i v;
#pragma unroll
        for (int u = 0; u < 4; u++) v[u] = real ? f16_pair((float)a[2 * u], (float)a[2 * u + 1]) : 0;
        if (ct0 + ctl < nct_alloc) rngQ[((size_t)plane * nct_alloc + ct0 + ctl) * NK * 64 + (size_t)m * 64 + lane] = v;
    }
}

__device__ __forceinline__ void t4x4_bytes(uint32_t a, uint32_t b, uint32_t c, uint32_t d, uint32_t& o0, uint32_t& o1, uint32_t& o2, uint32_t& o3)
{
    const uint32_t t0 = __builtin_amdgcn_perm(b, a, 0x06020400u), t1 = __builtin_amdgcn_perm(b, a, 0x07030501u);
    const uint32_t t2 = __builtin_amdgcn_perm(d, c, 0x06020400u), t3 = __builtin_amdgcn_perm(d, c, 0x07030501u);
    o0 = __builtin_amdgcn_perm(t2, t0, 0x05040100u);
    o1 = __builtin_amdgcn_perm(t3, t1, 0x05040100u);
    o2 = __builtin_amdgcn_perm(t2, t0, 0x07060302u);
    o3 = __builtin_amdgcn_perm(t3, t1, 0x07060302u);
}
__device__ __forceinline__ void b8_transpose(const uint32_t (&r)[16], uint32_t (&o)[16])
{
#pragma unroll
    for (int ty = 0; ty < 2; ty++)
#pragma unroll
        for (int tx = 0; tx < 2; tx++)
            t4x4_bytes(r[2 * (4 * ty + 0) + tx], r[2 * (4 * ty + 1) + tx], r[2 * (4 * ty + 2) + tx], r[2 * (4 * ty + 3) + tx],
                       o[2 * (4 * tx + 0) + ty], o[2 * (4 * tx + 1) + ty], o[2 * (4 * tx + 2) + ty], o[2 * (4 * tx + 3) + ty]);
}
__device__ __forceinline__ void b8_mirror(const uint32_t (&r)[16], uint32_t (&o)[16])
{
#pragma unroll
    for (int y = 0; y < 8; y++) {
        o[2 * y] = __builtin_bswap32(r[2 * y + 1]);
        o[2 * y + 1] = __builtin_bswap32(r[2 * y]);
    }
}
template <int MODE>
__device__ __forceinline__ void range_q8_body(int grp, int plane, const uint8_t* __restrict__ gray, FicRngStat* __restrict__ rng_st,
                                              float* __restrict__ rngE, unsigned long long* __restrict__ key,
                                              uint32_t* __restrict__ theta_g, v4i* __restrict__ rngQ,
                                              uint32_t* __restrict__ rngC, const FicGeom& g, int nct_alloc, int shape16)
{
    constexpr int B = 8, n = 64, DW = 16, NK = 4, CPR = MODE == 0 ? 1 : 4, STR = 80;
    __shared__ __attribute__((aligned(16))) uint8_t blk[64 * STR];
    __shared__ __attribute__((aligned(16))) uint8_t cpy[MODE == 0 ? 16 : 256 * STR];
    __shared__ int s_rM[64];
    const int j0 = grp * 64;
    const uint8_t* img = gray + (size_t)plane * g.W * g.H;
    for (int i = threadIdx.x; i < 64 * B; i += 256) {
        const int l = i >> 3, ry = i & 7;
        const int j = j0 + l;
        uint2 v = make_uint2(0u, 0u);
        if (j < g.Nr) v = *(const uint2*)(img + (size_t)((j / g.Rw) * B + ry) * g.W + (j % g.Rw) * B);
        *(uint2*)&blk[l * STR + ry * B] = v;
    }
    __syncthreads();
    {
        const int l = threadIdx.x >> 2, part = threadIdx.x & 3;
        const uint4 w4 = *(const uint4*)(blk + l * STR + part * 16);
        const uint32_t w[4] = {w4.x, w4.y, w4.z, w4.w};
        uint32_t S = 0, Q = 0;
#pragma unroll
        for (int i = 0; i < 4; i++) {
            S = __builtin_amdgcn_sad_u8(w[i], 0u, S);
            Q = __builtin_amdgcn_udot4(w[i], w[i], Q, false);
        }
        S += (uint32_t)__builtin_amdgcn_update_dpp(0, (int)S, 0xB1, 0xF, 0xF, true);
        Q += (uint32_t)__builtin_amdgcn_update_dpp(0, (int)Q, 0xB1, 0xF, 0xF, true);
        S += (uint32_t)__builtin_amdgcn_update_dpp(0, (int)S, 0x4E, 0xF, 0xF, true);
        Q += (uint32_t)__builtin_amdgcn_update_dpp(0, (int)Q, 0x4E, 0xF, 0xF, true);
        const int j = j0 + l;
        const int rM = (int)(S >> 6);
        if (part == 0) {
            s_rM[l] = rM;
            if (j < g.Nr_pad) {
                const int ss = (int)Q - 2 * rM * (int)S + n * rM * rM;
                const size_t o = (size_t)plane * g.Nr_pad + j;
                FicRngStat st;
                st.rM = j < g.Nr ? rM : 0;
                st.rem = j < g.Nr ? (int)S - (rM << 6) : 0;
                rng_st[o] = st;
                rngE[o] = __fmul_rn(__fadd_rn(__fmul_rn(__fsqrt_rn((float)ss), FIC_Q_ECOEF), FIC_Q_EABS), q_escale(g));
                key[o] = FIC_KEY_NONE;
                theta_g[o] = FIC_Q_THG_NONE;
            }
        }
    }
    if constexpr (MODE == 2) {
        const int c = threadIdx.x >> 6, l = threadIdx.x & 63;
        uint32_t r[16], o[16];
#pragma unroll
        for (int q = 0; q < 4; q++) {
            const uint4 v = *(const uint4*)(blk + l * STR + 16 * q);
            r[4 * q] = v.x; r[4 * q + 1] = v.y; r[4 * q + 2] = v.z; r[4 * q + 3] = v.w;
        }
        if (c == 0) {
#pragma unroll
            for (int q = 0; q < 16; q++) o[q] = r[q];
        } else if (c == 1) {
            uint32_t m[16];
            b8_mirror(r, m);
            b8_transpose(m, o);
        } else if (c == 2) {
            b8_mirror(r, o);
        } else {
            b8_transpose(r, o);
        }
#pragma unroll
        for (int q = 0; q < 4; q++) *(uint4*)(cpy + (l * 4 + c) * STR + 16 * q) = make_uint4(o[4 * q], o[4 * q + 1], o[4 * q + 2], o[4 * q + 3]);
    }
    __syncthreads();
    const uint8_t* const cps = MODE == 0 ? blk : cpy;
    constexpr int cols = 64 * CPR;
    const int ct0 = (j0 * CPR) / 32;
    for (int t = threadIdx.x; t < cols * 4; t += 256) {
        const int col = t >> 2, q = t & 3;
        if (j0 + col / CPR < g.Nr_pad)
            *(uint4*)(rngC + ((size_t)plane * g.Nr_pad * CPR + (size_t)j0 * CPR + col) * DW + 4 * q) = *(const uint4*)(cps + col * STR + 16 * q);
    }
    for (int t = threadIdx.x; t < (cols / 32) * NK * 64; t += 256) {
        const int lane = t & 63, m = (t >> 6) % NK, ctl = (t >> 6) / NK;
        int c32, pos0;
        frag_slot(MODE == 0 ? shape16 : 0, NK, m, lane, c32, pos0);
        const int col = ctl * 32 + c32, h = lane >> 5;
        const int l = col / CPR;
        const int rM = s_rM[l];
        const bool real = j0 + l < g.Nr;
        const uint8_t* cp = cps + col * STR;
        int a[8];
        if constexpr (MODE != 2) {
            const uint2 w = *(const uint2*)(cp + pos0);
#pragma unroll
            for (int u = 0; u < 8; u++) a[u] = (int)(((u < 4 ? w.x : w.y) >> (8 * (u & 3))) & 0xffu) - rM;
        } else {
            const bool odd = m >= NK / 2;
            const int q0 = 16 * (odd ? m - NK / 2 : m) + 8 * h;
            const uint2 w = *(const uint2*)(cp + q0), v = *(const uint2*)(cp + n - 8 - q0);
#pragma unroll
            for (int u = 0; u < 8; u++) {
                const int c0 = (int)(((u < 4 ? w.x : w.y) >> (8 * (u & 3))) & 0xffu);
                const int c1 = (int)(((u < 4 ? v.y : v.x) >> (8 * (3 - (u & 3)))) & 0xffu);
                a[u] = odd ? c0 - c1 : c0 + c1 - 2 * rM;
            }
        }
        v4i v;
#pragma unroll
        for (int u = 0; u < 4; u++) v[u] = real ? f16_pair((float)a[2 * u], (float)a[2 * u + 1]) : 0;
        if (ct0 + ctl < nct_alloc) rngQ[((size_t)plane * nct_alloc + ct0 + ctl) * NK * 64 + (size_t)m * 64 + lane] = v;
    }
}

template <int MODE>
__global__ __launch_bounds__(256) void k_range_q8(const uint8_t* __restrict__ gray, FicRngStat* __restrict__ rng_st,
                                                  float* __restrict__ rngE, unsigned long long* __restrict__ key,
                                                  uint32_t* __restrict__ theta_g, v4i* __restrict__ rngQ,
                                                  uint32_t* __restrict__ rngC, FicGeom g, int nct_alloc, int grp0, int shape16)
{
    range_q8_body<MODE>(grp0 + blockIdx.x, blockIdx.y, gray, rng_st, rngE, key, theta_g, rngQ, rngC, g, nct_alloc, shape16);
}
template <int MODE>
__global__ __launch_bounds__(256) void k_prep_q8(const uint8_t* __restrict__ gray, uint8_t* __restrict__ scaled, uint8_t* __restrict__ pool_pix,
                                                 FicDomStat* __restrict__ pool_st, uint32_t* __restrict__ pool_var,
                                                 double* __restrict__ pool_s64, v4i* __restrict__ poolQ, uint32_t* __restrict__ dflat,
                                                 FicRngStat* __restrict__ rng_st, float* __restrict__ rngE,
                                                 unsigned long long* __restrict__ key, uint32_t* __restrict__ theta_g,
                                                 v4i* __restrict__ rngQ, uint32_t* __restrict__ rngC, FicGeom g, int ndtiles_alloc,
                                                 int nct_alloc, int grp0, int shape16)
{
    if ((int)blockIdx.x < ndtiles_alloc)
        pool_q_body<8, true>(blockIdx.x, blockIdx.y, nullptr, gray, scaled, pool_pix, pool_st, pool_var, pool_s64, poolQ, dflat, g, ndtiles_alloc,
                             MODE == 2 ? 1 : 0, shape16);
    else
        range_q8_body<MODE>(grp0 + (int)blockIdx.x - ndtiles_alloc, blockIdx.y, gray, rng_st, rngE, key, theta_g, rngQ, rngC, g, nct_alloc, shape16);
}

struct QArgs {
    const v4i* poolQ;
    const uint32_t* dflat;
    const uint8_t* pool_pix;
    const FicDomStat* pool_st;
    const double* pool_s64;
    const v4i* rngQ;
    const uint32_t* rngC;
    const FicRngStat* rng_st;
    const float* rngE;
    unsigned long long* key;
    uint32_t* theta_g;
    const int16_t* rgb_rng;
    const uint16_t* rgb_pool;
    const FicRgbDomStat* rgb_dst;
    unsigned long long* stats;
    int Nd, Nd_pad, Nr, Nr_pad, n, lgn, W, H, Rw;
    int ndtiles, ndtiles_loop, ndtiles_alloc, nct_alloc;
    int ct_begin, ct_end;
    int nctg;
    int tiles_per_chunk, nchunks, planes;
    unsigned int* fin_count;
    FicOutputs out;
    FicGeom geom;
    const uint8_t* gray;
    const uint32_t* pool_var;
    int r_begin, r_end;
    int dbg_noflag;
};

__device__ __forceinline__ v16f mfma_f16(v4i a, v4i b, v16f c)
{
    return __builtin_amdgcn_mfma_f32_32x32x16_f16(__builtin_bit_cast(f16x8, a), __builtin_bit_cast(f16x8, b), c, 0, 0, 0);
}
__device__ __forceinline__ float max3f(float a, float b, float c) { return fmaxf(fmaxf(a, b), c); }
__device__ __forceinline__ float max16_abs(const v16f& a)
{
    const float m0 = max3f(fabsf(a[0]), fabsf(a[1]), fabsf(a[2]));
    const float m1 = max3f(fabsf(a[3]), fabsf(a[4]), fabsf(a[5]));
    const float m2 = max3f(fabsf(a[6]), fabsf(a[7]), fabsf(a[8]));
    const float m3 = max3f(fabsf(a[9]), fabsf(a[10]), fabsf(a[11]));
    const float m4 = max3f(fabsf(a[12]), fabsf(a[13]), fabsf(a[14]));
    return max3f(max3f(m0, m1, m2), max3f(m3, m4, fabsf(a[15])), 0.0f);
}
__device__ __forceinline__ float max16_sum(const v16f& a, const v16f& b)
{
    float v[16];
#pragma unroll
    for (int e = 0; e < 16; e++) v[e] = fabsf(a[e]) + fabsf(b[e]);
    const float m0 = fmaxf(fmaxf(v[0], v[1]), v[2]), m1 = fmaxf(fmaxf(v[3], v[4]), v[5]), m2 = fmaxf(fmaxf(v[6], v[7]), v[8]);
    const float m3 = fmaxf(fmaxf(v[9], v[10]), v[11]), m4 = fmaxf(fmaxf(v[12], v[13]), v[14]);
    return fmaxf(fmaxf(fmaxf(m0, m1), m2), fmaxf(fmaxf(m3, m4), v[15]));
}

template <int MODE> struct QMode {
    static constexpr int CSHIFT = (MODE == 0 || MODE == 3) ? 0 : ((MODE == 1 || MODE == 4) ? 3 : 2);
    static constexpr int NISO = (MODE == 0 || MODE == 3) ? 1 : 8;
    static constexpr bool RGB = MODE == 3 || MODE == 4;
};
template <int MODE> __device__ __forceinline__ int q_col_iso(int c) { return MODE == 2 ? (c == 0 ? 0 : (c == 1 ? 1 : (c == 2 ? 4 : 6))) : c; }

__device__ __forceinline__ void q_key_min(unsigned long long* keyp, unsigned long long best)
{
    if (best < __hip_atomic_load(keyp, __ATOMIC_RELAXED, __HIP_MEMORY_SCOPE_AGENT)) atomicMin(keyp, best);
}

template <int NK, int MODE>
__device__ __forceinline__ void q_flush(const QArgs& A, const uint32_t* myq, int qn, int plane, int ctw0, int lane)
{
    constexpr int NISO = QMode<MODE>::NISO, CSHIFT = QMode<MODE>::CSHIFT;
    constexpr int B = NK == 1 ? 4 : (NK == 4 ? 8 : 16);
    const FicRngStat* rst = A.rng_st + (size_t)plane * A.Nr_pad;
    const double* p64 = A.pool_s64 + (size_t)plane * A.Nd_pad;
    const FicDomStat* pst = A.pool_st + (size_t)plane * A.Nd_pad;
    unsigned long long* keyp = A.key + (size_t)plane * A.Nr_pad;
    const uint32_t* cop = A.rngC + (size_t)plane * A.Nr_pad * (1 << CSHIFT) * (A.n / 4);
    for (int base = 0; base < qn; base += 64) {
        const int i = base + lane;
        if (i < qn) {
            const uint32_t ent = myq[i];
            const uint32_t d = ent & 0x00FFFFFFu;
            if (d >= (uint32_t)A.Nd) continue;
            const int col = ctw0 * 32 + (int)(ent >> 24);
            if constexpr (MODE == 4) {
                const int j = col >> 3, k = col & 7;
                const FicRngStat rs = rst[j];
                const FicRgbDomStat ds = A.rgb_dst[d];
                const int16_t* rt = A.rgb_rng + (size_t)j * (B * B);
                const uint16_t* ps = A.rgb_pool + (size_t)d * (B * B);
                int ax, bx, cx, ay, by, cy;
                iso_affine(k, B - 1, ax, bx, cx, ay, by, cy);
                const int ox = ay * B + ax, oy = by * B + bx, o0 = cy * B + cx;
                float kov = 0.0f;
                for (int y = 0; y < B; y++) {
#pragma unroll 4
                    for (int x = 0; x < B; x++)
                        kov = __fadd_rn(kov, (float)((int)rt[y * B + x] * ((int)ps[o0 + x * ox + y * oy] - ds.msum)));
                }
                const float vRf = (float)rs.rem;
                float r = (rs.rem == 0 || ds.vD == 0) ? 0.0f : __fdiv_rn(kov, __fmul_rn(vRf, (float)ds.vD));
                r = __fmul_rn(r, r);
                const float e = __fmul_rn(__fmul_rn(vRf, vRf), __fsub_rn(1.0f, r));
                q_key_min(&keyp[j], ((unsigned long long)f32_orderable(e) << 32) | (d * 8u + (uint32_t)k));
                continue;
            }
            if constexpr (MODE == 3) {
                const FicRngStat rs = rst[col];
                const FicRgbDomStat ds = A.rgb_dst[d];
                const uint4* rt = (const uint4*)(A.rgb_rng + (size_t)col * (B * B));
                const uint4* ps = (const uint4*)(A.rgb_pool + (size_t)d * (B * B));
                float kov = 0.0f;
#pragma unroll 4
                for (int q = 0; q < B * B / 8; q++) {
                    const uint4 r4 = rt[q], p4 = ps[q];
                    const uint32_t rw[4] = {r4.x, r4.y, r4.z, r4.w}, pw[4] = {p4.x, p4.y, p4.z, p4.w};
#pragma unroll
                    for (int u = 0; u < 4; u++) {
                        kov = __fadd_rn(kov, (float)((int)(int16_t)(rw[u] & 0xffffu) * ((int)(pw[u] & 0xffffu) - ds.msum)));
                        kov = __fadd_rn(kov, (float)((int)(int16_t)(rw[u] >> 16) * ((int)(pw[u] >> 16) - ds.msum)));
                    }
                }
                const float vRf = (float)rs.rem;
                float r = (rs.rem == 0 || ds.vD == 0) ? 0.0f : __fdiv_rn(kov, __fmul_rn(vRf, (float)ds.vD));
                r = __fmul_rn(r, r);
                const float e = __fmul_rn(__fmul_rn(vRf, vRf), __fsub_rn(1.0f, r));
                q_key_min(&keyp[col], ((unsigned long long)f32_orderable(e) << 32) | d);
                continue;
            }
            const int j = col >> CSHIFT, k = q_col_iso<MODE>(col & ((1 << CSHIFT) - 1));
            const int k2 = k == 0 ? 2 : (k == 1 ? 3 : k + 1);
            const unsigned long long cur = __hip_atomic_load(&keyp[j], __ATOMIC_RELAXED, __HIP_MEMORY_SCOPE_AGENT);
            const FicRngStat rs = rst[j];
            const int Sd = (int)pst[d].sum;
            const double s64 = p64[d];
            const uint4* cw = (const uint4*)(cop + (size_t)col * (B * B / 4));
            const uint4* dw = (const uint4*)(A.pool_pix + ((size_t)plane * A.Nd_pad + d) * A.n);
            uint32_t s = 0, s2 = 0;
#pragma unroll
            for (int q = 0; q < B * B / 16; q++) {
                const uint4 c4 = cw[q], d4 = dw[q];
                s = __builtin_amdgcn_udot4(c4.x, d4.x, s, false);
                s = __builtin_amdgcn_udot4(c4.y, d4.y, s, false);
                s = __builtin_amdgcn_udot4(c4.z, d4.z, s, false);
                s = __builtin_amdgcn_udot4(c4.w, d4.w, s, false);
                if constexpr (MODE == 2) {
                    const uint4 m4 = dw[B * B / 16 - 1 - q];
                    s2 = __builtin_amdgcn_udot4(c4.x, __builtin_bswap32(m4.w), s2, false);
                    s2 = __builtin_amdgcn_udot4(c4.y, __builtin_bswap32(m4.z), s2, false);
                    s2 = __builtin_amdgcn_udot4(c4.z, __builtin_bswap32(m4.y), s2, false);
                    s2 = __builtin_amdgcn_udot4(c4.w, __builtin_bswap32(m4.x), s2, false);
                }
            }
            const int base_c = rs.rM * Sd + (Sd >> A.lgn) * rs.rem;
            const float err = exact_error((int)s - base_c, rs.rem, s64);
            unsigned long long best = ((unsigned long long)f32_orderable(err) << 32) | (d * (uint32_t)NISO + (uint32_t)k);
            if constexpr (MODE == 2) {
                const float err2 = exact_error((int)s2 - base_c, rs.rem, s64);
                const unsigned long long b2 = ((unsigned long long)f32_orderable(err2) << 32) | (d * (uint32_t)NISO + (uint32_t)k2);
                best = b2 < best ? b2 : best;
            }
            if (best < cur) atomicMin(&keyp[j], best);
        }
    }
}

template <int MODE, bool SEED = false>
__device__ __forceinline__ float q_share_max(float v)
{
    if constexpr (QMode<MODE>::CSHIFT >= 2) {
        v = fmaxf(v, __uint_as_float((uint32_t)__builtin_amdgcn_update_dpp(0, (int)__float_as_uint(v), 0xB1, 0xF, 0xF, true)));
        v = fmaxf(v, __uint_as_float((uint32_t)__builtin_amdgcn_update_dpp(0, (int)__float_as_uint(v), 0x4E, 0xF, 0xF, true)));
    }
    if constexpr (QMode<MODE>::CSHIFT == 3)
        v = fmaxf(v, __uint_as_float((uint32_t)__builtin_amdgcn_update_dpp(0, (int)__float_as_uint(v), 0x141, 0xF, 0xF, true)));
    if constexpr (SEED) {
        const int partner = (int)((threadIdx.x & 63u) ^ 32u) << 2;
        return fmaxf(v, __int_as_float(__builtin_amdgcn_ds_bpermute(partner, __float_as_int(v))));
    } else {
        const uint32_t u = __float_as_uint(v);
        const auto r = __builtin_amdgcn_permlane32_swap(u, u, false, false);
        return fmaxf(__uint_as_float(r[0]), __uint_as_float(r[1]));
    }
}

template <int NK, int MODE>
__device__ __forceinline__ void q_finalize_tail(const QArgs& A, int plane, int gx, int* s_wdone, int lane)
{
    (void)lane;
    if constexpr (QMode<MODE>::RGB) {
        return;
    } else {
        constexpr int CSHIFT = QMode<MODE>::CSHIFT, NISO = QMode<MODE>::NISO;
        constexpr int B = NK == 1 ? 4 : (NK == 4 ? 8 : 16);
        constexpr int CT = FIC_Q_WPG * fic_q_ctw(NK);
        asm volatile("s_waitcnt vmcnt(0) lgkmcnt(0)" ::: "memory");
        __syncthreads();
        if (threadIdx.x == 0) {
            unsigned int* cnt = A.fin_count + (size_t)plane * A.nctg + gx;
            const int last = __hip_atomic_fetch_add(cnt, 1u, __ATOMIC_RELAXED, __HIP_MEMORY_SCOPE_AGENT) == (unsigned)A.nchunks - 1u;
            if (last) __hip_atomic_store(cnt, 0u, __ATOMIC_RELAXED, __HIP_MEMORY_SCOPE_AGENT);
            *s_wdone = last;
        }
        __syncthreads();
        if (!*(volatile int*)s_wdone) return;
        const FicGeom& g = A.geom;
        const int j0 = ((A.ct_begin + gx * CT) * 32) >> CSHIFT, nj = (CT * 32) >> CSHIFT;
        for (int jj = (int)threadIdx.x; jj < nj; jj += 64 * FIC_Q_WPG) {
            const int j = j0 + jj;
            if (j < A.r_begin || j >= A.r_end) continue;
            unsigned long long kk;
            const unsigned long long none = FIC_KEY_NONE;
            asm volatile("global_atomic_umin_x2 %0, %1, %2, off sc0\n\ts_waitcnt vmcnt(0)"
                         : "=&v"(kk) : "v"(A.key + (size_t)plane * A.Nr_pad + j), "v"(none) : "memory");
            const uint32_t c = (uint32_t)kk;
            const int wloc = (int)(c / (uint32_t)NISO), k = (int)(c % (uint32_t)NISO);
            const int gi = wloc;
            const uint32_t* pp = (const uint32_t*)(A.pool_pix + ((size_t)plane * A.Nd_pad + gi) * A.n);
            const uint8_t* blk = A.gray + (size_t)plane * g.W * g.H + (size_t)((j / g.Rw) * B) * g.W + (j % g.Rw) * B;
            uint32_t acc = 0, s2;
            iso_dot<B, false>(blk, g.W, k, pp, acc, s2);
            finalize_store(A.out, g, plane, j, kk, wloc, gi, k, acc, A.pool_st[(size_t)plane * A.Nd_pad + gi],
                           A.rng_st[(size_t)plane * A.Nr_pad + j], A.pool_var[(size_t)plane * A.Nd_pad + gi]);
        }
    }
}

template <int NK, int MODE, bool MULTI, bool GFAST>
__device__ __forceinline__ void sweep_q_body(const QArgs& A)
{
    constexpr int CTW = fic_q_ctw(NK), CT = FIC_Q_WPG * CTW;
    constexpr int CSHIFT = QMode<MODE>::CSHIFT;
    constexpr bool FOLD = MODE == 2;
    constexpr int NKA = FOLD ? NK / 2 : NK;
    __shared__ uint32_t sQ[FIC_Q_WPG][FIC_Q_QCAP + 4];
    const int lane = threadIdx.x & 63;
    const int wave = __builtin_amdgcn_readfirstlane(threadIdx.x >> 6);
    int combo_, gx_;
    xcd_decode(blockIdx.x, A.nchunks * A.planes, A.nctg, combo_, gx_);
    const int plane = combo_ / A.nchunks;
    const int chunk = combo_ % A.nchunks;
    const int ctw0 = A.ct_begin + gx_ * CT + wave * CTW;
    const int dt0 = chunk * A.tiles_per_chunk;
    int dt1 = dt0 + A.tiles_per_chunk;
    if (dt1 > A.ndtiles_loop) dt1 = A.ndtiles_loop;
    __shared__ int s_wdone;
    if (dt0 >= A.ndtiles || ctw0 >= A.ct_end) {
        if (A.fin_count) q_finalize_tail<NK, MODE>(A, plane, gx_, &s_wdone, lane);
        return;
    }
    const unsigned long long clk0 = A.stats ? clock64() : 0ull, tick0 = A.stats ? wall_clock64() : 0ull;
    int nci = A.ct_end - ctw0;
    if (nci > CTW) nci = CTW;

    const int jcol = lane & 31, half = lane >> 5;
    const FicRngStat* rst = A.rng_st + (size_t)plane * A.Nr_pad;
    uint32_t* const thg = A.theta_g + (size_t)plane * A.Nr_pad;
    uint32_t* const myq = sQ[wave];
    uint32_t* const myqn = myq + FIC_Q_QCAP;
    const uint32_t myqn_lds = (uint32_t)(uintptr_t)(__attribute__((address_space(3))) uint32_t*)myqn;
    if (lane == 0) *myqn = 0u;

    v4i rb[CTW][NK];
    {
        const v4i* rp = A.rngQ + ((size_t)plane * A.nct_alloc + ctw0) * NK * 64 + lane;
#pragma unroll
        for (int ci = 0; ci < CTW; ci++)
#pragma unroll
            for (int m = 0; m < NK; m++) rb[ci][m] = rp[(ci * NK + m) * 64];
    }
    float tau[CTW], E[CTW], lmn[CTW];
    float gl[GFAST ? CTW : 1];
#pragma unroll
    for (int ci = 0; ci < (GFAST ? CTW : 1); ci++) gl[ci] = -1.0f;
    uint32_t okbits = 0, raise = 0;
#pragma unroll
    for (int ci = 0; ci < CTW; ci++) {
        const int col = (ctw0 + ci) * 32 + jcol;
        const int j = col >> CSHIFT;
        const bool ok = j < A.Nr && ci < nci;
        const int rem = ok ? rst[j].rem : 0;
        E[ci] = ok ? A.rngE[(size_t)plane * A.Nr_pad + j] : 0.0f;
        tau[ci] = (ok && rem != 0 && !A.dbg_noflag) ? FIC_Q_TAU_NONE : FIC_Q_TAU_ALL;
        lmn[ci] = FIC_Q_LMIN * (float)rem;
        okbits |= ok ? 1u << ci : 0u;
        raise |= (ok && rem != 0) ? 1u << ci : 0u;
    }

    const v4i* pa = A.poolQ + (size_t)plane * A.ndtiles_alloc * NK * 64 + lane;
    const uint32_t AS4* pflat = (const uint32_t AS4*)(uintptr_t)(A.dflat + (size_t)plane * A.ndtiles_alloc);
    const v16f zero = {0, 0, 0, 0, 0, 0, 0, 0, 0, 0, 0, 0, 0, 0, 0, 0};
    int qn = 0;
    unsigned st_slow = 0, st_pairs = 0;

    auto flush = [&]() __attribute__((always_inline)) {
        q_flush<NK, MODE>(A, myq, qn, plane, ctw0, lane);
        qn = 0;
        if (lane == 0) *myqn = 0u;
        __builtin_amdgcn_s_waitcnt(0x0F70);
    };
    auto val = [&](const v16f& acc, const v16f& acc2, int e) __attribute__((always_inline)) {
        return FOLD ? fabsf(acc[e]) + fabsf(acc2[e]) : fabsf(acc[e]);
    };
    auto slow_tile = [&](const v16f& acc, const v16f& acc2, float mx, int ci, int dt, bool first) __attribute__((always_inline)) {
        if (!first && __builtin_amdgcn_ballot_w64(mx > 0.0f) == 0 && pflat[dt] != 0u) return;
        st_slow++;
        const bool ok = (okbits >> ci) & 1u;
        const bool mayraise = (raise >> ci) & 1u;
        const int colw = ci * 32 + jcol;
        const int jg = ((ctw0 + ci) * 32 + jcol) >> CSHIFT;
        const uint32_t g = (MULTI && !GFAST && mayraise) ? thg[jg] : FIC_Q_THG_NONE;
        const uint32_t ent0 = (uint32_t)(dt * 32 + 4 * half) | ((uint32_t)colw << 24);
        if (first) {
            const float lo = __fsub_rn(q_share_max<MODE>(ok ? mx : 0.0f), E[ci]);
            if (mayraise && lo >= lmn[ci]) tau[ci] = fmaxf(tau[ci], __fsub_rn(__fmul_rn(lo, FIC_Q_LEVEL), E[ci]));
        }
        const bool cand0 = first && dt == 0 && half == 0 && ok && (jcol & ((1 << CSHIFT) - 1)) == 0;
        uint32_t hm = 0;
#pragma unroll
        for (int e = 15; e >= 0; e--)
            hm = __builtin_amdgcn_alignbit(hm, __float_as_uint(__fsub_rn(tau[ci], val(acc, acc2, e))), 31);
        if (!ok) hm = 0;
        if (cand0) hm |= 1u;
        const int cnt = __builtin_popcount(hm);
        if (cnt != 0) {
            uint32_t w;
            asm volatile("ds_add_rtn_u32 %0, %1, %2\n\ts_waitcnt lgkmcnt(0)" : "=v"(w) : "v"(myqn_lds), "v"((uint32_t)cnt) : "memory");
            int e = __builtin_ctz(hm);
            myq[w] = ent0 + (uint32_t)((e & 3) + 8 * (e >> 2));
            for (uint32_t h = hm & (hm - 1); h; h &= h - 1) {
                e = __builtin_ctz(h);
                myq[++w] = ent0 + (uint32_t)((e & 3) + 8 * (e >> 2));
            }
        }
        const float mp = cnt != 0 ? mx : -1.0f;
        const float lo2 = q_share_max<MODE>((mayraise && mp >= 0.0f) ? __fsub_rn(mp, E[ci]) : -1.0f);
        if (mayraise && lo2 >= 0.0f) {
            const float lb = __fsub_rn(__fmul_rn(lo2, FIC_Q_LEVEL), E[ci]);
            tau[ci] = fmaxf(tau[ci], lb);
            if (MULTI && lo2 >= lmn[ci] && lb > 0.0f && half == 0 && (jcol & ((1 << CSHIFT) - 1)) == 0) atomicMax((int*)&thg[jg], __float_as_int(lb));
        }
        if (MULTI && !GFAST && mayraise) tau[ci] = fmaxf(tau[ci], __uint_as_float(g));
        const int tot = __builtin_amdgcn_readfirstlane((int)*(volatile __attribute__((address_space(3))) uint32_t*)(__attribute__((address_space(3))) uint32_t*)myqn);
        st_pairs += (unsigned)(tot - qn);
        qn = tot;
        if (qn > FIC_Q_QFLUSH) flush();
    };
    auto tile_mfma = [&](const v4i (&at)[NK], const v4i (&bt)[NK], v16f& acc, v16f& acc2) __attribute__((always_inline)) {
        acc = zero;
#pragma unroll
        for (int m = 0; m < NKA; m++) acc = mfma_f16(at[m], bt[m], acc);
        if constexpr (FOLD) {
            acc2 = zero;
#pragma unroll
            for (int m = NKA; m < NK; m++) acc2 = mfma_f16(at[m], bt[m], acc2);
        }
    };

    v4i a0[NK], a1[NK];
    v16f acc, acc2 = zero;
    if constexpr (MULTI && FIC_Q_SEED) {
        if (dt0 != 0) {
#pragma unroll
            for (int m = 0; m < NK; m++) a0[m] = pa[(size_t)m * 64];
#pragma unroll
            for (int ci = 0; ci < CTW; ci++) {
                tile_mfma(a0, rb[ci], acc, acc2);
                const float mx = FOLD ? max16_sum(acc, acc2) : max16_abs(acc);
                const bool ok = (okbits >> ci) & 1u, mayraise = (raise >> ci) & 1u;
                const float lo = __fsub_rn(q_share_max<MODE, true>(ok ? mx : 0.0f), E[ci]);
                if (mayraise && lo > 0.0f) tau[ci] = fmaxf(tau[ci], __fsub_rn(__fmul_rn(lo, FIC_Q_LEVEL), E[ci]));
            }
        }
    }
#pragma unroll
    for (int m = 0; m < NK; m++) a0[m] = pa[((size_t)dt0 * NK + m) * 64];
#pragma unroll
    for (int m = 0; m < NK; m++) a1[m] = pa[((size_t)(dt0 + 1) * NK + m) * 64];
    tile_mfma(a0, rb[0], acc, acc2);

    auto refresh_thg = [&](auto ph) __attribute__((always_inline)) {
        if constexpr (MULTI && GFAST) {
            constexpr int PH = decltype(ph)::value, H = CTW / 2;
#pragma unroll
            for (int c = PH * H; c < PH * H + H; c++) {
                tau[c] = fmaxf(tau[c], gl[c]);
                gl[c] = __uint_as_float(thg[((ctw0 + c) * 32 + jcol) >> CSHIFT]);
            }
        }
    };
    auto step = [&](int dt, v4i (&ac)[NK], const v4i (&an)[NK], const bool first, auto ph) __attribute__((always_inline)) {
#pragma unroll
        for (int ci = 0; ci < CTW; ci++) {
            v16f nacc, nacc2 = zero;
            if (ci + 1 < CTW) tile_mfma(ac, rb[ci + 1], nacc, nacc2);
            else tile_mfma(an, rb[0], nacc, nacc2);
            if (ci == CTW - 2) {
#pragma unroll
                for (int m = 0; m < NK; m++) ac[m] = pa[((size_t)(dt + 2) * NK + m) * 64];
                refresh_thg(ph);
            }
            const float mx = FOLD ? max16_sum(acc, acc2) : max16_abs(acc);
            const bool hit = mx > tau[ci];
            if constexpr (NK == 4 && !FOLD) {
                __builtin_amdgcn_sched_group_barrier(0x8, 2, 0);
                __builtin_amdgcn_sched_group_barrier(0x2, 3, 0);
                __builtin_amdgcn_sched_group_barrier(0x8, 1, 0);
                __builtin_amdgcn_sched_group_barrier(0x2, 3, 0);
                __builtin_amdgcn_sched_group_barrier(0x8, 1, 0);
                __builtin_amdgcn_sched_group_barrier(0x2, 3, 0);
            } else if constexpr (NK == 4 && FOLD) {
#ifndef FIC_Q_SCHED
#define FIC_Q_SCHED 3
#endif
#if FIC_Q_SCHED == 0
                __builtin_amdgcn_sched_group_barrier(0x8, 2, 0);
                __builtin_amdgcn_sched_group_barrier(0x2, 8, 0);
                __builtin_amdgcn_sched_group_barrier(0x8, 1, 0);
                __builtin_amdgcn_sched_group_barrier(0x2, 8, 0);
                __builtin_amdgcn_sched_group_barrier(0x8, 1, 0);
                __builtin_amdgcn_sched_group_barrier(0x2, 9, 0);
#elif FIC_Q_SCHED == 2
                __builtin_amdgcn_sched_group_barrier(0x8, 4, 0);
                __builtin_amdgcn_sched_group_barrier(0x2, 25, 0);
#elif FIC_Q_SCHED == 3
                __builtin_amdgcn_sched_group_barrier(0x8, 1, 0);
                __builtin_amdgcn_sched_group_barrier(0x2, 6, 0);
                __builtin_amdgcn_sched_group_barrier(0x8, 1, 0);
                __builtin_amdgcn_sched_group_barrier(0x2, 6, 0);
                __builtin_amdgcn_sched_group_barrier(0x8, 1, 0);
                __builtin_amdgcn_sched_group_barrier(0x2, 6, 0);
                __builtin_amdgcn_sched_group_barrier(0x8, 1, 0);
                __builtin_amdgcn_sched_group_barrier(0x2, 7, 0);
#endif
            }
            if (__builtin_expect((__builtin_amdgcn_ballot_w64(hit) != 0) | first, 0)) slow_tile(acc, acc2, mx, ci, dt, first);
            acc = nacc;
            if constexpr (FOLD) acc2 = nacc2;
        }
    };
#ifdef FIC_Q_PHASES
    const unsigned long long ph1 = clock64();
#endif
    for (int dt = dt0; dt < dt1; dt += 2) {
        step(dt, a0, a1, dt == dt0, std::integral_constant<int, 0>());
        step(dt + 1, a1, a0, false, std::integral_constant<int, 1>());
    }
#ifdef FIC_Q_PHASES
    const unsigned long long ph2 = clock64();
#endif
    flush();
#ifdef FIC_Q_PHASES
    if (A.stats && lane == 0 && (blockIdx.x & 15) == 0 && wave == 0) {
        atomicAdd(&A.stats[0], ph1 - clk0);
        atomicAdd(&A.stats[1], ph2 - ph1);
        atomicAdd(&A.stats[2], (unsigned long long)clock64() - ph2);
        atomicAdd(&A.stats[4], (unsigned long long)(clock64() - clk0));
        atomicAdd(&A.stats[5], (unsigned long long)(wall_clock64() - tick0));
        atomicAdd(&A.stats[6], 1ull);
        atomicAdd(&A.stats[3], (unsigned long long)st_slow);
        atomicAdd(&A.stats[7], (unsigned long long)st_pairs);
    }
    if (false)
#endif
    if (A.stats && lane == 0) {
        atomicAdd(&A.stats[0], (unsigned long long)(dt1 - dt0) * (unsigned)nci);
        atomicAdd(&A.stats[1], (unsigned long long)st_slow);
        atomicAdd(&A.stats[2], (unsigned long long)st_pairs);
        atomicAdd(&A.stats[3], 1ull);
        if ((blockIdx.x & 15) == 0 && wave == 0) {
            atomicAdd(&A.stats[4], (unsigned long long)(clock64() - clk0));
            atomicAdd(&A.stats[5], (unsigned long long)(wall_clock64() - tick0));
            atomicAdd(&A.stats[6], 1ull);
        }
    }
    if (A.fin_count) q_finalize_tail<NK, MODE>(A, plane, gx_, &s_wdone, lane);
}

typedef float v4f __attribute__((ext_vector_type(4)));
__device__ __forceinline__ v4f mfma16_f16(v4i a, v4i b, v4f c)
{
    return __builtin_amdgcn_mfma_f32_16x16x32_f16(__builtin_bit_cast(f16x8, a), __builtin_bit_cast(f16x8, b), c, 0, 0, 0);
}
__device__ __forceinline__ float max8_abs(const v4f& x0, const v4f& x1)
{
    const float m0 = max3f(fabsf(x0[0]), fabsf(x0[1]), fabsf(x0[2])), m1 = max3f(fabsf(x0[3]), fabsf(x1[0]), fabsf(x1[1]));
    return max3f(m0, m1, max3f(fabsf(x1[2]), fabsf(x1[3]), 0.0f));
}
template <bool SEED = false>
__device__ __forceinline__ float q16_share_max(float v)
{
    const int partner = (int)((threadIdx.x & 63u) ^ 16u) << 2;
    const float w = fmaxf(v, __int_as_float(__builtin_amdgcn_ds_bpermute(partner, __float_as_int(v))));
    if constexpr (SEED) return fmaxf(w, __int_as_float(__builtin_amdgcn_ds_bpermute((int)((threadIdx.x & 63u) ^ 32u) << 2, __float_as_int(w))));
    const uint32_t uw = __float_as_uint(w);
    const auto q = __builtin_amdgcn_permlane32_swap(uw, uw, false, false);
    return fmaxf(__uint_as_float(q[0]), __uint_as_float(q[1]));
}
template <int NK, bool MULTI, bool GFAST>
__device__ __forceinline__ void sweep_q16_body(const QArgs& A)
{
    constexpr int CTW = fic_q_ctw(NK), CT = FIC_Q_WPG * CTW, CU = 2 * CTW, KS = NK / 2;
    __shared__ uint32_t sQ[FIC_Q_WPG][FIC_Q_QCAP + 4];
    const int lane = threadIdx.x & 63;
    const int wave = __builtin_amdgcn_readfirstlane(threadIdx.x >> 6);
    int combo_, gx_;
    xcd_decode(blockIdx.x, A.nchunks * A.planes, A.nctg, combo_, gx_);
    const int plane = combo_ / A.nchunks;
    const int chunk = combo_ % A.nchunks;
    const int ctw0 = A.ct_begin + gx_ * CT + wave * CTW;
    const int dt0 = chunk * A.tiles_per_chunk;
    int dt1 = dt0 + A.tiles_per_chunk;
    if (dt1 > A.ndtiles_loop) dt1 = A.ndtiles_loop;
    __shared__ int s_wdone;
    if (dt0 >= A.ndtiles || ctw0 >= A.ct_end) {
        if (A.fin_count) q_finalize_tail<NK, 0>(A, plane, gx_, &s_wdone, lane);
        return;
    }
    const unsigned long long clk0 = A.stats ? clock64() : 0ull, tick0 = A.stats ? wall_clock64() : 0ull;
    int nci = A.ct_end - ctw0;
    if (nci > CTW) nci = CTW;

    const int c16 = lane & 15, g4 = lane >> 4;
    const FicRngStat* rst = A.rng_st + (size_t)plane * A.Nr_pad;
    uint32_t* const thg = A.theta_g + (size_t)plane * A.Nr_pad;
    uint32_t* const myq = sQ[wave];
    uint32_t* const myqn = myq + FIC_Q_QCAP;
    const uint32_t myqn_lds = (uint32_t)(uintptr_t)(__attribute__((address_space(3))) uint32_t*)myqn;
    if (lane == 0) *myqn = 0u;

    v4i rb[CTW][NK];
    {
        const v4i* rp = A.rngQ + ((size_t)plane * A.nct_alloc + ctw0) * NK * 64 + lane;
#pragma unroll
        for (int ci = 0; ci < CTW; ci++)
#pragma unroll
            for (int m = 0; m < NK; m++) rb[ci][m] = rp[(ci * NK + m) * 64];
    }
    float tau[CU], E[CU], lmn[CU];
    float gl[GFAST ? CU : 1];
#pragma unroll
    for (int cj = 0; cj < (GFAST ? CU : 1); cj++) gl[cj] = -1.0f;
    uint32_t okbits = 0, raise = 0;
#pragma unroll
    for (int cj = 0; cj < CU; cj++) {
        const int j = ctw0 * 32 + cj * 16 + c16;
        const bool ok = j < A.Nr && (cj >> 1) < nci;
        const int rem = ok ? rst[j].rem : 0;
        E[cj] = ok ? A.rngE[(size_t)plane * A.Nr_pad + j] : 0.0f;
        tau[cj] = (ok && rem != 0 && !A.dbg_noflag) ? FIC_Q_TAU_NONE : FIC_Q_TAU_ALL;
        lmn[cj] = FIC_Q_LMIN * (float)rem;
        okbits |= ok ? 1u << cj : 0u;
        raise |= (ok && rem != 0) ? 1u << cj : 0u;
    }
    const v4i* pa = A.poolQ + (size_t)plane * A.ndtiles_alloc * NK * 64 + lane;
    const uint32_t AS4* pflat = (const uint32_t AS4*)(uintptr_t)(A.dflat + (size_t)plane * A.ndtiles_alloc);
    const v4f zero = {0, 0, 0, 0};
    int qn = 0;
    unsigned st_slow = 0, st_pairs = 0;

    auto flush = [&]() __attribute__((always_inline)) {
        q_flush<NK, 0>(A, myq, qn, plane, ctw0, lane);
        qn = 0;
        if (lane == 0) *myqn = 0u;
        __builtin_amdgcn_s_waitcnt(0x0F70);
    };
    auto val = [&](const v4f& x0, const v4f& x1, int e) __attribute__((always_inline)) { return fabsf(e < 4 ? x0[e] : x1[e - 4]); };
    auto slow_unit = [&](const v4f& x0, const v4f& x1, float mx, int cj, int dt, bool first) __attribute__((always_inline)) {
        if (!first && __builtin_amdgcn_ballot_w64(mx > 0.0f) == 0 && pflat[dt] != 0u) return;
        st_slow++;
        const bool ok = (okbits >> cj) & 1u;
        const bool mayraise = (raise >> cj) & 1u;
        const int colw = cj * 16 + c16;
        const int jg = ctw0 * 32 + colw;
        const uint32_t g = (MULTI && !GFAST && mayraise) ? thg[jg] : FIC_Q_THG_NONE;
        const uint32_t ent0 = (uint32_t)(dt * 32 + 4 * g4) | ((uint32_t)colw << 24);
        if (first) {
            const float lo = __fsub_rn(q16_share_max<>(ok ? mx : 0.0f), E[cj]);
            if (mayraise && lo >= lmn[cj]) tau[cj] = fmaxf(tau[cj], __fsub_rn(__fmul_rn(lo, FIC_Q_LEVEL), E[cj]));
        }
        const bool cand0 = first && dt == 0 && g4 == 0 && ok;
        uint32_t hm = 0;
#pragma unroll
        for (int e = 7; e >= 0; e--)
            hm = __builtin_amdgcn_alignbit(hm, __float_as_uint(__fsub_rn(tau[cj], val(x0, x1, e))), 31);
        if (!ok) hm = 0;
        if (cand0) hm |= 1u;
        const int cnt = __builtin_popcount(hm);
        if (cnt != 0) {
            uint32_t w;
            asm volatile("ds_add_rtn_u32 %0, %1, %2\n\ts_waitcnt lgkmcnt(0)" : "=v"(w) : "v"(myqn_lds), "v"((uint32_t)cnt) : "memory");
            int e = __builtin_ctz(hm);
            myq[w] = ent0 + (uint32_t)((e & 3) + 16 * (e >> 2));
            for (uint32_t h = hm & (hm - 1); h; h &= h - 1) {
                e = __builtin_ctz(h);
                myq[++w] = ent0 + (uint32_t)((e & 3) + 16 * (e >> 2));
            }
        }
        const float mp = cnt != 0 ? mx : -1.0f;
        const float lo2 = q16_share_max<>((mayraise && mp >= 0.0f) ? __fsub_rn(mp, E[cj]) : -1.0f);
        if (mayraise && lo2 >= 0.0f) {
            const float lb = __fsub_rn(__fmul_rn(lo2, FIC_Q_LEVEL), E[cj]);
            tau[cj] = fmaxf(tau[cj], lb);
            if (MULTI && lo2 >= lmn[cj] && lb > 0.0f && g4 == 0) atomicMax((int*)&thg[jg], __float_as_int(lb));
        }
        if (MULTI && !GFAST && mayraise) tau[cj] = fmaxf(tau[cj], __uint_as_float(g));
        const int tot = __builtin_amdgcn_readfirstlane((int)*(volatile __attribute__((address_space(3))) uint32_t*)(__attribute__((address_space(3))) uint32_t*)myqn);
        st_pairs += (unsigned)(tot - qn);
        qn = tot;
        if (qn > FIC_Q_QFLUSH) flush();
    };
    auto unit_mfma = [&](const v4i (&at)[NK], int cj, v4f& x0, v4f& x1) __attribute__((always_inline)) {
        x0 = zero;
        x1 = zero;
#pragma unroll
        for (int ks = 0; ks < KS; ks++) x0 = mfma16_f16(at[ks], rb[cj >> 1][(cj & 1) * KS + ks], x0);
#pragma unroll
        for (int ks = 0; ks < KS; ks++) x1 = mfma16_f16(at[KS + ks], rb[cj >> 1][(cj & 1) * KS + ks], x1);
    };

    v4i a0[NK], a1[NK];
    v4f x0, x1;
    if constexpr (MULTI && FIC_Q_SEED) {
        if (dt0 != 0) {
#pragma unroll
            for (int m = 0; m < NK; m++) a0[m] = pa[(size_t)m * 64];
#pragma unroll
            for (int cj = 0; cj < CU; cj++) {
                unit_mfma(a0, cj, x0, x1);
                const float mx = max8_abs(x0, x1);
                const bool ok = (okbits >> cj) & 1u, mayraise = (raise >> cj) & 1u;
                const float lo = __fsub_rn(q16_share_max<true>(ok ? mx : 0.0f), E[cj]);
                if (mayraise && lo > 0.0f) tau[cj] = fmaxf(tau[cj], __fsub_rn(__fmul_rn(lo, FIC_Q_LEVEL), E[cj]));
            }
        }
    }
#pragma unroll
    for (int m = 0; m < NK; m++) a0[m] = pa[((size_t)dt0 * NK + m) * 64];
#pragma unroll
    for (int m = 0; m < NK; m++) a1[m] = pa[((size_t)(dt0 + 1) * NK + m) * 64];
    unit_mfma(a0, 0, x0, x1);
    auto refresh_thg = [&](auto ph) __attribute__((always_inline)) {
        if constexpr (MULTI && GFAST) {
            constexpr int PH = decltype(ph)::value, H = CU / 2;
#pragma unroll
            for (int c = PH * H; c < PH * H + H; c++) {
                tau[c] = fmaxf(tau[c], gl[c]);
                gl[c] = __uint_as_float(thg[ctw0 * 32 + c * 16 + c16]);
            }
        }
    };
    auto step = [&](int dt, v4i (&ac)[NK], const v4i (&an)[NK], const bool first, auto ph) __attribute__((always_inline)) {
#pragma unroll
        for (int cj = 0; cj < CU; cj++) {
            v4f n0, n1;
            if (cj + 1 < CU) unit_mfma(ac, cj + 1, n0, n1);
            else unit_mfma(an, 0, n0, n1);
            if (cj == CU - 2) {
#pragma unroll
                for (int m = 0; m < NK; m++) ac[m] = pa[((size_t)(dt + 2) * NK + m) * 64];
                refresh_thg(ph);
            }
            const float mx = max8_abs(x0, x1);
            const bool hit = mx > tau[cj];
            if (__builtin_expect((__builtin_amdgcn_ballot_w64(hit) != 0) | first, 0)) slow_unit(x0, x1, mx, cj, dt, first);
            x0 = n0;
            x1 = n1;
        }
    };
    for (int dt = dt0; dt < dt1; dt += 2) {
        step(dt, a0, a1, dt == dt0, std::integral_constant<int, 0>());
        step(dt + 1, a1, a0, false, std::integral_constant<int, 1>());
    }
    flush();
    if (A.stats && lane == 0) {
        atomicAdd(&A.stats[0], (unsigned long long)(dt1 - dt0) * (unsigned)nci);
        atomicAdd(&A.stats[1], (unsigned long long)st_slow);
        atomicAdd(&A.stats[2], (unsigned long long)st_pairs);
        atomicAdd(&A.stats[3], 1ull);
        if ((blockIdx.x & 15) == 0 && wave == 0) {
            atomicAdd(&A.stats[4], (unsigned long long)(clock64() - clk0));
            atomicAdd(&A.stats[5], (unsigned long long)(wall_clock64() - tick0));
            atomicAdd(&A.stats[6], 1ull);
        }
    }
    if (A.fin_count) q_finalize_tail<NK, 0>(A, plane, gx_, &s_wdone, lane);
}

template <int NK, int MODE, bool MULTI>
__global__ __launch_bounds__(64 * FIC_Q_WPG, NK == 4 ? FIC_Q_WAVES_B8 : (NK < 4 ? FIC_Q_WAVES_B4 : 1)) void k_sweep_q(QArgs A)
{
    sweep_q_body<NK, MODE, MULTI, false>(A);
}
template <int NK, int MODE>
__global__ __launch_bounds__(64 * FIC_Q_WPG, NK == 4 ? FIC_Q_WAVES_B8 : (NK < 4 ? FIC_Q_WAVES_B4 : 1)) void k_sweep_qs(QArgs A)
{
    sweep_q_body<NK, MODE, true, true>(A);
}
template <int NK, bool MULTI>
__global__ __launch_bounds__(64 * FIC_Q_WPG, NK == 4 ? FIC_Q_WAVES_B8 : 1) void k_sweep_q16(QArgs A)
{
    sweep_q16_body<NK, MULTI, false>(A);
}
template <int NK>
__global__ __launch_bounds__(64 * FIC_Q_WPG, NK == 4 ? FIC_Q_WAVES_B8 : 1) void k_sweep_q16s(QArgs A)
{
    sweep_q16_body<NK, true, true>(A);
}

template <int NK, int MODE>
static void q_launch_nm(int multi, dim3 grid, dim3 block, hipStream_t s, const QArgs& A)
{
    if (multi == 2) hipLaunchKernelGGL((k_sweep_qs<NK, MODE>), grid, block, 0, s, A);
    else if (multi) hipLaunchKernelGGL((k_sweep_q<NK, MODE, true>), grid, block, 0, s, A);
    else hipLaunchKernelGGL((k_sweep_q<NK, MODE, false>), grid, block, 0, s, A);
}
int fic_q_multi_kind(int nchunks, int tiles_per_chunk) { return nchunks <= 1 ? 0 : (tiles_per_chunk <= FIC_Q_GFAST_TILES ? 2 : 1); }
static bool q_launch(int NK, int mode, int multi, dim3 grid, dim3 block, hipStream_t s, const QArgs& A, int shape16 = 0)
{
    if (shape16 && mode == 0 && NK == 4) {
        if (multi == 2) hipLaunchKernelGGL((k_sweep_q16s<4>), grid, block, 0, s, A);
        else if (multi) hipLaunchKernelGGL((k_sweep_q16<4, true>), grid, block, 0, s, A);
        else hipLaunchKernelGGL((k_sweep_q16<4, false>), grid, block, 0, s, A);
    } else if (shape16 && mode == 0 && NK == 16) {
        if (multi == 2) hipLaunchKernelGGL((k_sweep_q16s<16>), grid, block, 0, s, A);
        else if (multi) hipLaunchKernelGGL((k_sweep_q16<16, true>), grid, block, 0, s, A);
        else hipLaunchKernelGGL((k_sweep_q16<16, false>), grid, block, 0, s, A);
    } else if (NK == 1 && mode == 0) q_launch_nm<1, 0>(multi, grid, block, s, A);
    else if (NK == 1 && mode == 1) q_launch_nm<1, 1>(multi, grid, block, s, A);
    else if (NK == 1 && mode == 3) q_launch_nm<1, 3>(multi, grid, block, s, A);
    else if (NK == 4 && mode == 0) q_launch_nm<4, 0>(multi, grid, block, s, A);
    else if (NK == 4 && mode == 2) q_launch_nm<4, 2>(multi, grid, block, s, A);
    else if (NK == 4 && mode == 3) q_launch_nm<4, 3>(multi, grid, block, s, A);
    else if (NK == 16 && mode == 0) q_launch_nm<16, 0>(multi, grid, block, s, A);
    else if (NK == 16 && mode == 2) q_launch_nm<16, 2>(multi, grid, block, s, A);
    else if (NK == 16 && mode == 3) q_launch_nm<16, 3>(multi, grid, block, s, A);
    else if (NK == 1 && mode == 4) q_launch_nm<1, 4>(multi, grid, block, s, A);
    else if (NK == 4 && mode == 4) q_launch_nm<4, 4>(multi, grid, block, s, A);
    else if (NK == 16 && mode == 4) q_launch_nm<16, 4>(multi, grid, block, s, A);
    else return false;
    return true;
}
int fic_q_ct(int B) { return FIC_Q_WPG * fic_q_ctw(B * B / 16); }
int fic_q_ctw_host(int B) { return fic_q_ctw(B * B / 16); }
int fic_q_mode(int B, int n_iso) { return n_iso == 1 ? 0 : (B == 4 ? 1 : 2); }
int fic_q_cols_per_range(int B, int n_iso) { const int m = fic_q_mode(B, n_iso); return m == 0 ? 1 : (m == 1 ? 8 : 4); }
int fic_q_unroll(int B, int n_iso) { (void)B; (void)n_iso; return FIC_Q_UNROLL; }
int fic_q_shape16(const FicGeom& g)
{
    const long long ndtiles = (g.Nd + 31) / 32;
    int want = g.q_shape;
    if (want == 0) {
        const char* env = getenv("FIC_Q_SHAPE");
        if (env && (env[0] == '1' || env[0] == '2') && env[1] == '\0') want = env[0] - '0';
    }
    if (!FIC_Q_SHAPE16 || g.n_iso != 1 || g.B < 8 || want == 2) return 0;
    return (want == 1 || ndtiles * (g.n / 16) >= 100000) ? 1 : 0;
}
int fic_q_resident(int B) { return (B == 4 ? FIC_Q_WAVES_B4 : (B == 8 ? FIC_Q_WAVES_B8 : 1)) * 4 / FIC_Q_WPG; }

int fic_q_prep_fused(const FicGeom& g, int ndtiles_alloc, int ngrp)
{
    return (g.B == 8 && (long long)g.planes * (ndtiles_alloc + ngrp) <= 1024) ? 1 : 0;
}
int fic_launch_q_prep(const FicBuffers& b, void* poolQ, void* dflat, void* rngQ, void* rngC, void* rngE, void* theta_g,
                      const FicGeom& g, int ndtiles_alloc, int nct_alloc, int grp0, int ngrp, hipStream_t s)
{
    const int mode = fic_q_mode(g.B, g.n_iso);
    const int shape16 = fic_q_shape16(g);
    if (fic_q_prep_fused(g, ndtiles_alloc, ngrp)) {
        auto pk = mode == 0 ? k_prep_q8<0> : k_prep_q8<2>;
        hipLaunchKernelGGL(pk, dim3(ndtiles_alloc + ngrp, g.planes), dim3(256), 0, s, (const uint8_t*)b.gray, b.scaled, b.pool_pix, b.pool_st,
                           b.pool_var, b.pool_s64, (v4i*)poolQ, (uint32_t*)dflat, b.rng_st, (float*)rngE, b.key, (uint32_t*)theta_g,
                           (v4i*)rngQ, (uint32_t*)rngC, g, ndtiles_alloc, nct_alloc, grp0, shape16);
        FIC_LAUNCH_CHECK();
        return 0;
    }
    auto pool = g.B == 4 ? k_pool_q<4> : (g.B == 8 ? k_pool_q<8> : k_pool_q<16>);
    hipLaunchKernelGGL(pool, dim3(ndtiles_alloc, g.planes), dim3(256), 0, s, (const uint8_t*)b.scaled, b.pool_pix,
                       b.pool_st, b.pool_var, b.pool_s64, (v4i*)poolQ, (uint32_t*)dflat, g, ndtiles_alloc, mode == 2 ? 1 : 0, shape16);
    FIC_LAUNCH_CHECK();
    const size_t stage_bytes = (size_t)64 * fic_q_cols_per_range(g.B, g.n_iso) * (g.n + 8);
    const int staged = stage_bytes <= 40 * 1024 ? 1 : 0;
    if (g.B == 8 && mode != 1) {
        auto rk = mode == 0 ? k_range_q8<0> : k_range_q8<2>;
        hipLaunchKernelGGL(rk, dim3(ngrp, g.planes), dim3(256), 0, s, (const uint8_t*)b.gray, b.rng_st, (float*)rngE, b.key,
                           (uint32_t*)theta_g, (v4i*)rngQ, (uint32_t*)rngC, g, nct_alloc, grp0, shape16);
    } else {
        hipLaunchKernelGGL(k_range_q, dim3(ngrp, g.planes), dim3(256), staged ? stage_bytes : 0, s, (const uint8_t*)b.gray, b.rng_st,
                           (float*)rngE, b.key, (uint32_t*)theta_g, (v4i*)rngQ, (uint32_t*)rngC, g, nct_alloc, grp0, mode, staged, shape16);
    }
    FIC_LAUNCH_CHECK();
    return 0;
}

int fic_launch_sweep_q(const FicBuffers& b, const void* poolQ, const void* dflat, const void* rngQ, const void* rngC, const void* rngE,
                       void* theta_g, const FicGeom& g, int ct_begin, int ct_end, int ndtiles, int ndtiles_alloc,
                       int nct_alloc, int tiles_per_chunk, int nchunks, hipStream_t s, unsigned long long* stats, int dbg_noflag,
                       const FicOutputs* fin_out, unsigned int* fin_count, int r_begin, int r_count)
{
    QArgs A;
    A.stats = stats;
    A.dbg_noflag = dbg_noflag;
    A.fin_count = fin_out ? fin_count : nullptr;
    if (fin_out) A.out = *fin_out; else memset(&A.out, 0, sizeof(A.out));
    A.geom = g; A.gray = b.gray; A.pool_var = b.pool_var; A.r_begin = r_begin; A.r_end = r_begin + r_count;
    A.poolQ = (const v4i*)poolQ; A.dflat = (const uint32_t*)dflat; A.pool_pix = b.pool_pix; A.pool_st = b.pool_st;
    A.pool_s64 = b.pool_s64; A.rngQ = (const v4i*)rngQ; A.rngC = (const uint32_t*)rngC; A.rng_st = b.rng_st;
    A.rngE = (const float*)rngE; A.key = b.key; A.theta_g = (uint32_t*)theta_g;
    A.Nd = g.Nd; A.Nd_pad = g.Nd_pad; A.Nr = g.Nr; A.Nr_pad = g.Nr_pad; A.n = g.n; A.lgn = g.lgn; A.W = g.W; A.H = g.H; A.Rw = g.Rw;
    const int unroll = fic_q_unroll(g.B, g.n_iso);
    A.ndtiles = ndtiles; A.ndtiles_loop = (ndtiles + unroll - 1) / unroll * unroll; A.ndtiles_alloc = ndtiles_alloc; A.nct_alloc = nct_alloc;
    A.ct_begin = ct_begin; A.ct_end = ct_end; A.tiles_per_chunk = tiles_per_chunk; A.nchunks = nchunks;
    const int CT = fic_q_ct(g.B);
    A.nctg = (ct_end - ct_begin + CT - 1) / CT;
    A.planes = g.planes;
    A.rgb_rng = nullptr; A.rgb_pool = nullptr; A.rgb_dst = nullptr;
    if (ct_begin + A.nctg * CT > nct_alloc || g.Nd >= (1 << 24) || A.ndtiles_loop + unroll > ndtiles_alloc || tiles_per_chunk % unroll)
        return (int)hipErrorInvalidValue;
    dim3 grid((unsigned)(nchunks * g.planes) * (unsigned)A.nctg), block(64 * FIC_Q_WPG);
    const int mode = fic_q_mode(g.B, g.n_iso);
    if (!q_launch(g.B * g.B / 16, mode, fic_q_multi_kind(nchunks, tiles_per_chunk), grid, block, s, A, fic_q_shape16(g))) return (int)hipErrorInvalidValue;
    FIC_LAUNCH_CHECK();
    return 0;
}

__global__ __launch_bounds__(256) void k_pool_qrgb(const uint16_t* __restrict__ pool_sum, const FicRgbDomStat* __restrict__ dst,
                                                   v4i* __restrict__ poolQ, uint32_t* __restrict__ dflat,
                                                   uint32_t* __restrict__ amax, FicGeom g)
{
    __shared__ uint32_t s_norm;
    const int n = g.n, NK = n / 16;
    const int dtile = blockIdx.x;
    if (threadIdx.x == 0) s_norm = 0u;
    __syncthreads();
    if (threadIdx.x < 32) {
        const int d = dtile * 32 + threadIdx.x;
        float norm = 0.0f;
        if (d < g.Nd) {
            const FicRgbDomStat ds = dst[d];
            if (ds.vD != 0) {
                const uint16_t* ps = pool_sum + (size_t)d * n;
                long long s2 = 0;
                for (int i = 0; i < n; i++) {
                    const int gd = (int)ps[i] - ds.msum;
                    s2 += gd * gd;
                }
                norm = __fmul_rn(__fdiv_rn(__fsqrt_rn((float)s2), (float)ds.vD), 1.001f);
            }
        }
        atomicMax(&s_norm, __float_as_uint(norm));
    }
    for (int t = threadIdx.x; t < NK * 64; t += 256) {
        const int lane = t & 63, m = t >> 6;
        const int d = dtile * 32 + (lane & 31), h = lane >> 5;
        v4i v = {0, 0, 0, 0};
        if (d < g.Nd) {
            const FicRgbDomStat ds = dst[d];
            if (ds.vD != 0) {
                const uint16_t* p = pool_sum + (size_t)d * n + 16 * m + 8 * h;
                const float vd = (float)ds.vD;
#pragma unroll
                for (int u = 0; u < 4; u++)
                    v[u] = f16_pair(__fdiv_rn((float)((int)p[2 * u] - ds.msum), vd), __fdiv_rn((float)((int)p[2 * u + 1] - ds.msum), vd));
            }
        }
        poolQ[(size_t)dtile * NK * 64 + t] = v;
    }
    __syncthreads();
    if (threadIdx.x == 0) {
        dflat[dtile] = s_norm ? 0u : 1u;
        if (s_norm) atomicMax(amax, s_norm);
    }
}

__global__ __launch_bounds__(256) void k_range_qrgb(const int16_t* __restrict__ rng_t, const FicRgbRngStat* __restrict__ rst,
                                                    FicRngStat* __restrict__ qst, float* __restrict__ rngE,
                                                    unsigned long long* __restrict__ key, uint32_t* __restrict__ theta_g,
                                                    v4i* __restrict__ rngQ, const uint32_t* __restrict__ amax, FicGeom g,
                                                    int nct_alloc, int cshift)
{
    const int n = g.n, NK = n / 16;
    const int j0 = blockIdx.x * 64;
    if (threadIdx.x < (64 >> cshift)) {
        const int j = (j0 >> cshift) + threadIdx.x;
        if (j < g.Nr) {
            const int16_t* rt = rng_t + (size_t)j * n;
            long long s2 = 0;
            for (int i = 0; i < n; i++) s2 += (int)rt[i] * (int)rt[i];
            const float am = __uint_as_float(*amax);
            FicRngStat st;
            st.rM = 0;
            st.rem = rst[j].vR;
            qst[j] = st;
            rngE[j] = __fmul_rn(__fadd_rn(__fmul_rn(__fmul_rn(__fmul_rn(__fsqrt_rn((float)s2), 1.0001f), am), FIC_Q_ECOEF),
                                          __fmul_rn(FIC_Q_EABS, __fadd_rn(1.0f, am))), q_escale(g));
            key[j] = FIC_KEY_NONE;
            theta_g[j] = FIC_Q_THG_NONE;
        }
    }
    for (int t = threadIdx.x; t < 2 * NK * 64; t += 256) {
        const int lane = t & 63, m = (t >> 6) % NK, ctl = (t >> 6) / NK;
        const int col = j0 + ctl * 32 + (lane & 31), h = lane >> 5;
        const int j = col >> cshift;
        v4i v = {0, 0, 0, 0};
        if (j < g.Nr) {
            if (cshift == 0) {
                const int16_t* p = rng_t + (size_t)j * n + 16 * m + 8 * h;
#pragma unroll
                for (int u = 0; u < 4; u++) v[u] = f16_pair((float)p[2 * u], (float)p[2 * u + 1]);
            } else {
                const int16_t* p = rng_t + (size_t)j * n;
                const int kinv = iso_inverse(col & 7), p0 = 16 * m + 8 * h;
                float f[8];
#pragma unroll
                for (int u = 0; u < 8; u++) f[u] = (float)p[iso_source(kinv, g.B, (p0 + u) % g.B, (p0 + u) / g.B)];
#pragma unroll
                for (int u = 0; u < 4; u++) v[u] = f16_pair(f[2 * u], f[2 * u + 1]);
            }
        }
        const int ct = j0 / 32 + ctl;
        if (ct < nct_alloc) rngQ[((size_t)ct * NK + m) * 64 + lane] = v;
    }
}

int fic_launch_rgbq(const uint16_t* pool_sum, const FicRgbDomStat* pool_st, const int16_t* rng_t, const FicRgbRngStat* rng_st,
                    unsigned long long* key, void* poolQ, void* dflat, void* rngQ, void* qst, void* rngE, void* theta_g, void* amax,
                    const FicGeom& g, int ndtiles, int ndtiles_alloc, int nct_alloc, int tiles_per_chunk, int nchunks, hipStream_t s,
                    unsigned long long* stats)
{
    if (hipMemsetAsync(amax, 0, sizeof(uint32_t), s) != hipSuccess) return (int)hipErrorUnknown;
    hipLaunchKernelGGL(k_pool_qrgb, dim3(ndtiles_alloc), dim3(256), 0, s, pool_sum, pool_st, (v4i*)poolQ, (uint32_t*)dflat,
                       (uint32_t*)amax, g);
    FIC_LAUNCH_CHECK();
    const int CT = fic_q_ct(g.B);
    const int cshift = g.n_iso == 8 ? 3 : 0;
    const int nct = (int)((((long long)g.Nr << cshift) + 31) / 32);
    hipLaunchKernelGGL(k_range_qrgb, dim3(nct_alloc / 2), dim3(256), 0, s, rng_t, rng_st, (FicRngStat*)qst, (float*)rngE, key,
                       (uint32_t*)theta_g, (v4i*)rngQ, (const uint32_t*)amax, g, nct_alloc, cshift);
    FIC_LAUNCH_CHECK();
    QArgs A;
    A.stats = stats;
    A.dbg_noflag = 0;
    A.fin_count = nullptr; memset(&A.out, 0, sizeof(A.out)); A.geom = g; A.gray = nullptr; A.pool_var = nullptr; A.r_begin = 0; A.r_end = 0;
    A.poolQ = (const v4i*)poolQ; A.dflat = (const uint32_t*)dflat; A.pool_pix = nullptr; A.pool_st = nullptr; A.pool_s64 = nullptr;
    A.rngQ = (const v4i*)rngQ; A.rngC = nullptr; A.rng_st = (const FicRngStat*)qst; A.rngE = (const float*)rngE; A.key = key;
    A.theta_g = (uint32_t*)theta_g;
    A.rgb_rng = rng_t; A.rgb_pool = pool_sum; A.rgb_dst = pool_st;
    A.Nd = g.Nd; A.Nd_pad = g.Nd; A.Nr = g.Nr; A.Nr_pad = g.Nr; A.n = g.n; A.lgn = g.lgn; A.W = g.W; A.H = g.H; A.Rw = g.Rw;
    const int unroll = FIC_Q_UNROLL;
    A.ndtiles = ndtiles; A.ndtiles_loop = (ndtiles + unroll - 1) / unroll * unroll; A.ndtiles_alloc = ndtiles_alloc; A.nct_alloc = nct_alloc;
    A.ct_begin = 0; A.ct_end = nct; A.tiles_per_chunk = tiles_per_chunk; A.nchunks = nchunks;
    A.nctg = (nct + CT - 1) / CT;
    A.planes = 1;
    if (A.nctg * CT > nct_alloc || (nct_alloc & 1) || g.Nd >= (1 << 24) || A.ndtiles_loop + unroll > ndtiles_alloc || tiles_per_chunk % unroll)
        return (int)hipErrorInvalidValue;
    dim3 grid((unsigned)nchunks * (unsigned)A.nctg), block(64 * FIC_Q_WPG);
    if (!q_launch(g.B * g.B / 16, cshift ? 4 : 3, fic_q_multi_kind(nchunks, tiles_per_chunk), grid, block, s, A)) return (int)hipErrorInvalidValue;
    FIC_LAUNCH_CHECK();
    return 0;
}
```

### fractal-image-compression_amd/host.py

```python
import ctypes as C
import io

import numpy as np

from . import capi
from .capi import FicError


class RasterImage:

    def __init__(self, width, height, argb=None):
        self.width = int(width)
        self.height = int(height)
        if argb is None:
            argb = np.zeros(self.width * self.height, np.int32)
        self.argb = np.ascontiguousarray(argb, np.int32).reshape(-1)
        if self.argb.size != self.width * self.height:
            raise ValueError("argb has the wrong number of pixels")

    @classmethod
    def from_gray(cls, gray):
        g = np.ascontiguousarray(gray, np.uint8)
        u = g.astype(np.uint32)
        argb = (0xFF000000 | (u << 16) | (u << 8) | u).astype(np.uint32).view(np.int32)
        return cls(g.shape[1], g.shape[0], argb.reshape(-1))

    def red(self):
        return ((self.argb.view(np.uint32) >> 16) & 0xFF).astype(np.uint8).reshape(self.height, self.width)


class _DevArray:

    def __init__(self, ptr, shape, typestr):
        self.__cuda_array_interface__ = {"shape": tuple(shape), "typestr": typestr, "data": (int(ptr), False),
                                         "version": 2, "strides": None}


class Encoder:

    def __init__(self, width, height, B, wK=None, n_iso=1, planes=1, device=0):
        L = capi.lib()
        self.width, self.height, self.B, self.n_iso, self.planes, self.device = width, height, B, n_iso, planes, device
        Rw, Rh, Dw, Dh = capi.geometry(width, height, B)
        if wK is None:
            if Dw != Dh:
                raise FicError(-2, "full search (wK=None) needs a square block grid, as in the reference (FC:89-96)")
            wK = Dw
        self.wK = wK
        self.Rw, self.Rh, self.Dw, self.Dh = Rw, Rh, Dw, Dh
        self.n_ranges, self.n_domains = Rw * Rh, Dw * Dh
        self._h = L.fic_ctx_create(device, width, height, B, wK, n_iso, planes)
        if not self._h:
            raise FicError(L.fic_last_error_code() or -3, capi.last_error())
        self._keep = None
        info = (C.c_int * 10)()
        capi.check(L.fic_ctx_info(self._h, info))
        self.ranges_per_tile = 64 * info[6]

    def close(self):
        if getattr(self, "_h", None):
            capi.lib().fic_ctx_destroy(self._h)
            self._h = None

    def __del__(self):
        try:
            self.close()
        except Exception:
            pass

    def __enter__(self):
        return self

    def __exit__(self, *a):
        self.close()

    def set_gray(self, gray):
        L = capi.lib()
        n = self.planes * self.height * self.width
        if hasattr(gray, "data_ptr"):
            if not gray.is_cuda or gray.dtype.itemsize != 1 or not gray.is_contiguous() or gray.numel() != n:
                raise FicError(-3, "device input must be a contiguous uint8 CUDA tensor [planes,H,W]")
            self._keep = gray
            capi.check(L.fic_ctx_set_gray_device(self._h, C.c_void_p(gray.data_ptr())))
        else:
            g = np.ascontiguousarray(gray, np.uint8)
            if g.size != n:
                raise FicError(-3, f"input has {g.size} pixels, expected {n}")
            capi.check(L.fic_ctx_set_gray_host(self._h, capi.ptr(g, C.c_uint8)))

    def set_argb(self, argb):
        a = np.ascontiguousarray(argb, np.int32)
        if a.size != self.planes * self.height * self.width:
            raise FicError(-3, "argb has the wrong number of pixels")
        capi.check(capi.lib().fic_ctx_set_argb_host(self._h, capi.ptr(a, C.c_int32)))

    def set_option(self, name, value):
        capi.check(capi.lib().fic_ctx_set_option(self._h, name.encode(), int(value)))

    def encode(self, range_begin=0, range_count=-1, stream=None):
        s = 0 if stream is None else int(getattr(stream, "cuda_stream", stream))
        capi.check(capi.lib().fic_ctx_encode(self._h, range_begin, range_count, C.c_void_p(s)))

    def sync(self):
        capi.check(capi.lib().fic_ctx_sync(self._h))

    def sweep_time(self, reset=True):
        ms, n = C.c_double(), C.c_int()
        capi.check(capi.lib().fic_ctx_sweep_time(self._h, C.byref(ms), C.byref(n), 1 if reset else 0))
        return ms.value, n.value

    def sweep_stats(self, reset=True):
        v = (C.c_uint64 * 8)()
        capi.check(capi.lib().fic_ctx_sweep_stats(self._h, v, 1 if reset else 0))
        d = dict(zip(["tiles", "flagged_tiles", "exact_pairs", "waves", "wave_cycles", "wave_ticks", "waves_sampled"], [int(x) for x in v]))
        d["clock_ghz"] = d["wave_cycles"] / d["wave_ticks"] / 10.0 if d["wave_ticks"] else None
        return d

    def last_kernel(self):
        buf = C.create_string_buffer(96)
        capi.check(capi.lib().fic_ctx_last_kernel(self._h, buf, 96))
        return buf.value.decode()

    def info(self):
        v = (C.c_int * 10)()
        capi.check(capi.lib().fic_ctx_info(self._h, v))
        keys = ["Rw", "Rh", "Nr", "Dw", "Dh", "Nd", "NR", "tiles", "chunks", "sweep_kind"]
        return dict(zip(keys, list(v)))

    def results(self):
        P, N = self.planes, self.n_ranges
        r = {
            "idx_local": np.zeros((P, N), np.int32), "a": np.zeros((P, N), np.float32),
            "b": np.zeros((P, N), np.float32), "iso": np.zeros((P, N), np.int32),
            "qrows": np.zeros((P, N, 3), np.int32), "idx_global": np.zeros((P, N), np.int32),
            "err": np.zeros((P, N), np.float32),
        }
        capi.check(capi.lib().fic_ctx_get_results_host(
            self._h, capi.ptr(r["idx_local"], C.c_int32), capi.ptr(r["a"], C.c_float), capi.ptr(r["b"], C.c_float),
            capi.ptr(r["iso"], C.c_int32), capi.ptr(r["qrows"], C.c_int32), capi.ptr(r["idx_global"], C.c_int32),
            capi.ptr(r["err"], C.c_float)))
        return r

    def results_device(self):
        import torch
        p = [C.c_void_p() for _ in range(7)]
        capi.check(capi.lib().fic_ctx_result_device_ptrs(self._h, *[C.byref(x) for x in p]))
        P, N = self.planes, self.n_ranges
        dev = torch.device("cuda", self.device)

        def t(ptr, shape, ts):
            return torch.as_tensor(_DevArray(ptr.value, shape, ts), device=dev)

        return {"idx_local": t(p[0], (P, N), "<i4"), "a": t(p[1], (P, N), "<f4"), "b": t(p[2], (P, N), "<f4"),
                "iso": t(p[3], (P, N), "<i4"), "qrows": t(p[4], (P, N, 3), "<i4"),
                "idx_global": t(p[5], (P, N), "<i4"), "err": t(p[6], (P, N), "<f4")}

    def records_device(self):
        import torch
        p = C.c_void_p()
        capi.check(capi.lib().fic_ctx_records_device_ptr(self._h, C.byref(p)))
        return torch.as_tensor(_DevArray(p.value, (self.planes, self.n_ranges, 6), "<i4"), device=torch.device("cuda", self.device))

    def collage(self):
        out = np.zeros((self.planes, self.height * self.width), np.int32)
        capi.check(capi.lib().fic_ctx_collage_host(self._h, capi.ptr(out, C.c_int32)))
        return out

    def decode(self, zoom=1):
        P = self.planes
        avg = np.zeros(P, np.float32)
        it = np.zeros(P, np.int32)
        if zoom != 1:
            z = int(zoom) if zoom in (1, 2, 4) else 1
            out = np.zeros((P, z * self.height, z * self.width), np.uint8)
            capi.check(capi.lib().fic_ctx_decode_zoom_host(self._h, int(zoom), capi.ptr(out, C.c_uint8), capi.ptr(avg, C.c_float),
                                                           capi.ptr(it, C.c_int)))
            return out, avg, it
        out = np.zeros((P, self.height, self.width), np.uint8)
        capi.check(capi.lib().fic_ctx_decode_host(self._h, capi.ptr(out, C.c_uint8), capi.ptr(avg, C.c_float),
                                                  capi.ptr(it, C.c_int)))
        return out, avg, it

    def debug_pool(self):
        P, Nd, n = self.planes, self.n_domains, self.B * self.B
        pix = np.zeros((P, Nd, n), np.uint8)
        s = np.zeros((P, Nd), np.uint32)
        v = np.zeros((P, Nd), np.uint32)
        sc = np.zeros((P, self.height // 2, self.width // 2), np.uint8)
        capi.check(capi.lib().fic_ctx_debug_pool_host(self._h, capi.ptr(pix, C.c_uint8), capi.ptr(s, C.c_uint32),
                                                      capi.ptr(v, C.c_uint32), capi.ptr(sc, C.c_uint8)))
        return {"pix": pix, "sum": s, "var": v, "scaled": sc}

    Q_STORES = ("pool", "flat", "rng", "E", "rng_st", "rngC")

    def debug_q(self, which):
        i = self.Q_STORES.index(which)
        size = C.c_int64()
        capi.check(capi.lib().fic_ctx_debug_q_host(self._h, i, None, 0, C.byref(size)))
        out = np.zeros(size.value, np.uint8)
        capi.check(capi.lib().fic_ctx_debug_q_host(self._h, i, out.ctypes.data_as(C.c_void_p), out.size, C.byref(size)))
        return out


def encode_rgb_per_channel(rgb, B, wK=None, n_iso=1, device=0, sweep=0):
    a = np.ascontiguousarray(rgb, np.uint8)
    if a.ndim == 3:
        a = a[None]
    n, h, w, _ = a.shape
    planes = np.ascontiguousarray(a.transpose(0, 3, 1, 2)).reshape(n * 3, h, w)
    with Encoder(w, h, B, wK, n_iso, n * 3, device) as enc:
        if sweep:
            enc.set_option("sweep", sweep)
        enc.set_gray(planes)
        enc.encode()
        r = enc.results()
    return {k: v.reshape((n, 3) + v.shape[1:]) for k, v in r.items()}


def encode_gray(gray, B, wK=None, n_iso=1, device=0, sweep=0, chunks=0, q_shape=0):
    g = np.ascontiguousarray(gray, np.uint8)
    with Encoder(g.shape[1], g.shape[0], B, wK, n_iso, 1, device) as enc:
        if sweep:
            enc.set_option("sweep", sweep)
        if chunks:
            enc.set_option("chunks", chunks)
        if q_shape:
            enc.set_option("q_shape", q_shape)
        enc.set_gray(g)
        enc.encode()
        r = enc.results()
        out = {k: v[0] for k, v in r.items()}
        out["wK"] = enc.wK
        return out


class FractalCompression:

    blockgroesse = 8
    widthKernel = 2
    n_iso = 1
    device = 0
    imageInfo = None
    imageIso = None
    _last = None

    @staticmethod
    def isGreyScale(image):
        rc = capi.lib().fic_is_greyscale_argb(capi.ptr(image.argb, C.c_int32), image.width, image.height)
        return bool(capi.check(rc))

    @classmethod
    def encode(cls, image, out):
        if cls.isGreyScale(image):
            return cls.encodeGrayScale(image, out)
        return cls.encodeRGB(image, out)

    avgError = np.float32(0.0)

    @classmethod
    def getAvgError(cls):
        return cls.avgError

    @classmethod
    def decode(cls, inputStream):
        data = inputStream.read() if hasattr(inputStream, "read") else bytes(inputStream)
        if len(data) >= 4 and int.from_bytes(data[:4], "big", signed=True) != 0:
            return cls._decode_rgb(data)
        return cls._decode_gray(data)

    @classmethod
    def _decode_gray(cls, run):
        gray, avg, _ = capi.decode_gray_run(run, cls.device, float(cls.avgError))
        cls.avgError = avg
        return RasterImage.from_gray(gray)

    @classmethod
    def _decode_rgb(cls, run):
        argb, avg, _, w, h = capi.decode_rgb_run(run, cls.device, float(cls.avgError))
        cls.avgError = avg
        return RasterImage(w, h, argb)
# ... 85 lines not shown
```

### include/fic.h

```cpp
#ifndef FIC_H
#define FIC_H

#include <stdint.h>

#ifdef __cplusplus
extern "C" {
#endif

#define FIC_API __attribute__((visibility("default")))

#define FIC_OK 0
#define FIC_E_GEOMETRY (-1)
#define FIC_E_WINDOW (-2)
#define FIC_E_ARGUMENT (-3)
#define FIC_E_NO_DEVICE (-4)
#define FIC_E_HIP (-5)
#define FIC_E_NOT_GREY (-6)
#define FIC_E_STATE (-7)
#define FIC_E_CAPACITY (-8)

typedef struct fic_ctx fic_ctx;

FIC_API const char* fic_version(void);
FIC_API const char* fic_last_error(void);
FIC_API int fic_last_error_code(void);
FIC_API int fic_device_count(void);

FIC_API int fic_geometry(int w, int h, int B, int* Rw, int* Rh, int* Dw, int* Dh);

FIC_API int fic_is_greyscale_argb(const int32_t* argb, int w, int h);

FIC_API int fic_encode_gray_argb(const int32_t* argb, int w, int h, int B, int wK, int n_iso, int device,
                                 int32_t* idx_local, float* a, float* b, int32_t* iso, int32_t* qrows);
FIC_API int fic_encode_gray_u8(const uint8_t* gray, int w, int h, int B, int wK, int n_iso, int device,
                               int32_t* idx_local, float* a, float* b, int32_t* iso, int32_t* qrows);

FIC_API int fic_encode_gray_argb_multi(const int32_t* argb, int w, int h, int B, int wK, int n_iso, int n_gpus,
                                       int32_t* idx_local, float* a, float* b, int32_t* iso, int32_t* qrows);
FIC_API int fic_encode_gray_u8_multi(const uint8_t* gray, int w, int h, int B, int wK, int n_iso, int n_gpus,
                                     int32_t* idx_local, float* a, float* b, int32_t* iso, int32_t* qrows);

FIC_API void fic_release_cache(void);

FIC_API int64_t fic_write_run_gray(const int32_t* qrows, int n_ranges, int w, int h, int B, int wK, uint8_t* out,
                                   int64_t capacity);

FIC_API fic_ctx* fic_ctx_create(int device, int w, int h, int B, int wK, int n_iso, int planes);
FIC_API void fic_ctx_destroy(fic_ctx* ctx);

FIC_API int fic_ctx_set_gray_host(fic_ctx* ctx, const uint8_t* gray);
FIC_API int fic_ctx_set_argb_host(fic_ctx* ctx, const int32_t* argb);
FIC_API int fic_ctx_set_gray_device(fic_ctx* ctx, const void* dev_gray);

FIC_API int fic_ctx_encode(fic_ctx* ctx, int range_begin, int range_count, void* hip_stream);
FIC_API int fic_ctx_sync(fic_ctx* ctx);

FIC_API int fic_ctx_get_results_host(fic_ctx* ctx, int32_t* idx_local, float* a, float* b, int32_t* iso,
                                     int32_t* qrows, int32_t* idx_global, float* err);
FIC_API int fic_ctx_result_device_ptrs(fic_ctx* ctx, void** idx_local, void** a, void** b, void** iso, void** qrows,
                                       void** idx_global, void** err);

FIC_API int fic_ctx_records_device_ptr(fic_ctx* ctx, void** records);

FIC_API int fic_ctx_collage_host(fic_ctx* ctx, int32_t* argb_out);

FIC_API int fic_encode_rgb_argb(const int32_t* argb, int w, int h, int B, int wK, int device, int32_t* idx_local,
                                float* a, float* bR, float* bG, float* bB, int32_t* qrows5, int32_t* collage_argb);
typedef struct fic_rgb_ctx fic_rgb_ctx;
FIC_API fic_rgb_ctx* fic_rgb_ctx_create(int device, int w, int h, int B, int wK, int planes);
FIC_API void fic_rgb_ctx_destroy(fic_rgb_ctx* ctx);
FIC_API int fic_rgb_ctx_set_argb_host(fic_rgb_ctx* ctx, const int32_t* argb);
FIC_API int fic_rgb_ctx_set_argb_device(fic_rgb_ctx* ctx, const void* dev_argb);
FIC_API int fic_rgb_ctx_encode(fic_rgb_ctx* ctx, int with_collage, void* hip_stream);
FIC_API int fic_rgb_ctx_sync(fic_rgb_ctx* ctx);
FIC_API int fic_rgb_ctx_set_option(fic_rgb_ctx* ctx, const char* name, int value);
FIC_API int fic_rgb_ctx_last_sweep(fic_rgb_ctx* ctx);
FIC_API int fic_rgb_ctx_last_kernel(fic_rgb_ctx* ctx, char* out, int capacity);
FIC_API int fic_rgb_ctx_sweep_stats(fic_rgb_ctx* ctx, uint64_t* out8, int reset);
FIC_API int fic_rgb_ctx_get_results_host(fic_rgb_ctx* ctx, int32_t* idx_local, float* a, float* bR, float* bG, float* bB,
                                         int32_t* qrows5, int32_t* collage_argb);
FIC_API int fic_rgb_ctx_decode_host(fic_rgb_ctx* ctx, int32_t* argb_out, float* avg_error_out, int* iterations_out);
FIC_API int fic_encode_rgb_iso_argb(const int32_t* argb, int w, int h, int B, int wK, int n_iso, int device, int32_t* idx_local,
                                    float* a, float* bR, float* bG, float* bB, int32_t* iso, int32_t* qrows5,
                                    int32_t* collage_argb);
FIC_API fic_rgb_ctx* fic_rgb_ctx_create_iso(int device, int w, int h, int B, int wK, int n_iso, int planes);
FIC_API int fic_rgb_ctx_get_iso_host(fic_rgb_ctx* ctx, int32_t* iso);

FIC_API int64_t fic_write_run_rgb(const int32_t* qrows5, int n_ranges, int w, int h, int B, int wK, uint8_t* out,
                                  int64_t capacity);

FIC_API int fic_decode_gray_run(const uint8_t* run, int64_t len, int device, uint8_t* gray_out, int64_t capacity,
                                int* w, int* h, float* avg_error_io, int* iterations);
FIC_API int fic_decode_rgb_run(const uint8_t* run, int64_t len, int device, int32_t* argb_out,
                               int64_t capacity_pixels, int* w, int* h, float* avg_error_io, int* iterations);
FIC_API int fic_ctx_decode_host(fic_ctx* ctx, uint8_t* gray_out, float* avg_error_out, int* iterations_out);

FIC_API int fic_decode_gray_run_zoom(const uint8_t* run, int64_t len, int zoom, int device, uint8_t* gray_out, int64_t capacity,
                                     int* w, int* h, float* avg_error_io, int* iterations);
FIC_API int fic_decode_rgb_run_zoom(const uint8_t* run, int64_t len, int zoom, int device, int32_t* argb_out,
                                    int64_t capacity_pixels, int* w, int* h, float* avg_error_io, int* iterations);
FIC_API int fic_decode_quadtree_run_zoom(const uint8_t* run, int64_t len, int zoom, int device, uint8_t* gray_out, int64_t capacity,
                                         int* w, int* h, float* avg_error_io, int* iterations);
FIC_API int fic_decode_rgb_quadtree_run_zoom(const uint8_t* run, int64_t len, int zoom, int device, int32_t* argb_out,
                                             int64_t capacity_pixels, int* w, int* h, float* avg_error_io, int* iterations);
FIC_API int fic_ctx_decode_zoom_host(fic_ctx* ctx, int zoom, uint8_t* gray_out, float* avg_error_out, int* iterations_out);

FIC_API int fic_encode_gray_quadtree_u8(const uint8_t* gray, int w, int h, int B_max, int B_min, int wK, int n_iso, float threshold,
                                        int device, int32_t* leaves, int64_t capacity, int* n_leaves);
FIC_API int fic_encode_gray_quadtree_argb(const int32_t* argb, int w, int h, int B_max, int B_min, int wK, int n_iso,
                                          float threshold, int device, int32_t* leaves, int64_t capacity, int* n_leaves);
FIC_API int64_t fic_write_run_quadtree(const int32_t* leaves, int n_leaves, int w, int h, int B_max, int B_min, int wK, int n_iso,
                                       uint8_t* out, int64_t capacity);
FIC_API int fic_decode_quadtree_run(const uint8_t* run, int64_t len, int device, uint8_t* gray_out, int64_t capacity, int* w,
                                    int* h, float* avg_error_io, int* iterations);
FIC_API int fic_debug_quadtree_sse(const uint8_t* gray, int w, int h, int B_max, int B_min, int wK, int n_iso, int device,
                                   uint32_t* sse, int64_t capacity);

FIC_API int fic_encode_rgb_quadtree_argb(const int32_t* argb, int w, int h, int B_max, int B_min, int wK, float threshold,
                                         int device, int32_t* leaves, int64_t capacity, int* n_leaves);
FIC_API int64_t fic_write_run_rgb_quadtree(const int32_t* leaves, int n_leaves, int w, int h, int B_max, int B_min, int wK,
                                           uint8_t* out, int64_t capacity);
FIC_API int fic_decode_rgb_quadtree_run(const uint8_t* run, int64_t len, int device, int32_t* argb_out, int64_t capacity_pixels,
                                        int* w, int* h, float* avg_error_io, int* iterations);
FIC_API int fic_debug_rgb_quadtree_sse(const int32_t* argb, int w, int h, int B_max, int B_min, int wK, int device, uint32_t* sse,
                                       int64_t capacity);

FIC_API int fic_ctx_set_option(fic_ctx* ctx, const char* name, int value);
FIC_API int fic_ctx_sweep_time(fic_ctx* ctx, double* total_ms, int* launches, int reset);
FIC_API int fic_ctx_sweep_stats(fic_ctx* ctx, uint64_t* out8, int reset);
FIC_API int fic_ctx_info(fic_ctx* ctx, int* out10);
FIC_API int fic_ctx_last_kernel(fic_ctx* ctx, char* out, int capacity);
FIC_API int fic_sweep_ranges_per_pool_read(int kind, int B, int n_iso);

FIC_API int fic_debug_sqrt_f64(int device, uint32_t first, uint32_t count, double* out);
FIC_API int fic_debug_float_sum(int device, float carry, const uint32_t* vals, int count, float* out);
FIC_API int fic_debug_float_sum_fallbacks(void);
FIC_API int fic_debug_decode_gray_run(const uint8_t* run, int64_t len, int device, uint8_t* gray_out, int64_t capacity,
                                      float* avg_error_io, int* iterations, int* seq_sums);
FIC_API int fic_debug_rccl_selftest(int n);
FIC_API int fic_debug_gather_fallbacks(void);
FIC_API int fic_ctx_debug_pool_host(fic_ctx* ctx, uint8_t* pix, uint32_t* sum, uint32_t* var, uint8_t* scaled);
FIC_API int fic_ctx_debug_q_host(fic_ctx* ctx, int which, void* out, int64_t capacity, int64_t* size);
FIC_API int fic_rgb_ctx_debug_q_host(fic_rgb_ctx* ctx, int which, void* out, int64_t capacity, int64_t* size);

#ifdef __cplusplus
}
#endif
#endif
```

Before: 137.3 million.

## Always fuse prep and finalize for B=8; build range fragments inside sweep

For 8x8 ranges, the fused prep+finalize path is now enabled by default (env/option overridable) instead of only for small grids, cutting the quantised pipeline from five launches to two. When MODE 2 applies and the chunking is suitable, the sweep kernel builds its fp16 range fragments directly from the compact range copy in registers, so prep no longer writes the large rngQ buffer. The scaled-image write in pooling is trimmed to only the bytes later read, and the single-chunk finalize skips the atomic last-block counter. In exchange, sweep blocks do extra per-block work and the fused prep kernel now runs on large grids where it was previously avoided.

```diff
diff --git a/fractal-image-compression_amd/capi.py b/fractal-image-compression_amd/capi.py
--- a/fractal-image-compression_amd/capi.py
+++ b/fractal-image-compression_amd/capi.py
@@ -125,6 +125,8 @@
         "fic_decode_rgb_quadtree_run_zoom": (C.c_int, [u8p, C.c_int64, C.c_int, C.c_int, i32p, C.c_int64, ip, ip, f32p, ip]),
         "fic_ctx_decode_zoom_host": (C.c_int, [vp, C.c_int, u8p, f32p, ip]),
     }
+    optional = {"fic_ctx_last_launches": (C.c_int, [vp, ip, ip])}
+    sig.update({k: v for k, v in optional.items() if hasattr(L, k)})
     for name, (res, args) in sig.items():
         fn = getattr(L, name)
         fn.restype = res
diff --git a/fractal-image-compression_amd/csrc/fic_capi.cpp b/fractal-image-compression_amd/csrc/fic_capi.cpp
--- a/fractal-image-compression_amd/csrc/fic_capi.cpp
+++ b/fractal-image-compression_amd/csrc/fic_capi.cpp
@@ -359,27 +359,35 @@
     q.nct_alloc = (nct + q.CT - 1) / q.CT * q.CT + q.CT;
     return q;
 }
-int q_prep(fic_ctx* c, int tile0, int tile1, hipStream_t s)
+int q_rng_alloc(fic_ctx* c, hipStream_t s)
+{
+    if (c->q_rng) return FIC_OK;
+    const QShape q = q_shape(c->g);
+    const size_t bytes = (size_t)c->g.planes * q.nct_alloc * (c->g.n / 16) * 64 * 16;
+    HIP_TRY(hipMalloc(&c->q_rng, bytes));
+    HIP_TRY(hipMemsetAsync(c->q_rng, 0, bytes, s));
+    return FIC_OK;
+}
+int q_prep(fic_ctx* c, int tile0, int tile1, hipStream_t s, bool fused, bool own_frags)
 {
     const FicGeom& g = c->g;
     const QShape q = q_shape(g);
     const size_t P = (size_t)g.planes, NK = (size_t)g.n / 16;
     if (!c->q_pool) HIP_TRY(hipMalloc(&c->q_pool, P * q.ndtiles_alloc * NK * 64 * 16));
     if (!c->q_flat) HIP_TRY(hipMalloc(&c->q_flat, P * q.ndtiles_alloc * sizeof(uint32_t)));
-    if (!c->q_rng) {
-        HIP_TRY(hipMalloc(&c->q_rng, P * q.nct_alloc * NK * 64 * 16));
-        HIP_TRY(hipMemsetAsync(c->q_rng, 0, P * q.nct_alloc * NK * 64 * 16, s));
-    }
+    if (!own_frags) { int rc = q_rng_alloc(c, s); if (rc) return rc; }
+    c->q_rng_skipped = own_frags;
     if (!c->q_rngC) HIP_TRY(hipMalloc(&c->q_rngC, P * g.Nr_pad * fic_q_cols_per_range(g.B, g.n_iso) * g.n));
     if (!c->q_E) HIP_TRY(hipMalloc(&c->q_E, P * g.Nr_pad * sizeof(float)));
     if (!c->q_thg) HIP_TRY(hipMalloc(&c->q_thg, (P * g.Nr_pad + (size_t)2 * q.CT * 32 + 64) * sizeof(uint32_t)));
     const int tsz = 64 * g.NR;
     const int grp0 = tile0 * tsz / 64, grp1 = tile1 * tsz / 64;
-    if (fic_launch_q_prep(c->b, c->q_pool, c->q_flat, c->q_rng, c->q_rngC, c->q_E, c->q_thg, g, q.ndtiles_alloc, q.nct_alloc, grp0, grp1 - grp0, s))
+    if (fic_launch_q_prep(c->b, c->q_pool, c->q_flat, own_frags ? nullptr : c->q_rng, c->q_rngC, c->q_E, c->q_thg, g, q.ndtiles_alloc, q.nct_alloc,
+                          grp0, grp1 - grp0, s, fused ? 1 : 0))
         return fail(FIC_E_HIP, "k_pool_q / k_range_q launch failed");
     return FIC_OK;
 }
-int q_sweep(fic_ctx* c, int tile0, int tile1, hipStream_t s, int* nchunks_out, bool fused_fin = false, int r_begin = 0, int r_count = 0)
+void q_chunks(const fic_ctx* c, int tile0, int tile1, int* nchunks_out, int* tiles_per_chunk_out)
 {
     const FicGeom& g = c->g;
     const QShape q = q_shape(g);
@@ -403,16 +411,26 @@
     int tiles_per_chunk = (q.ndtiles + nchunks - 1) / nchunks;
     tiles_per_chunk = (tiles_per_chunk + q.unroll - 1) / q.unroll * q.unroll;
     nchunks = (q.ndtiles + tiles_per_chunk - 1) / tiles_per_chunk;
+    *nchunks_out = nchunks;
+    *tiles_per_chunk_out = tiles_per_chunk;
+}
+int q_sweep(fic_ctx* c, int tile0, int tile1, hipStream_t s, int nchunks, int tiles_per_chunk, bool fused_fin, bool own_frags, int r_begin,
+            int r_count)
+{
+    const FicGeom& g = c->g;
+    const QShape q = q_shape(g);
+    const int tsz = 64 * g.NR;
+    const int cpr = fic_q_cols_per_range(g.B, g.n_iso);
+    const int ct_begin = tile0 * tsz * cpr / 32, ct_end = tile1 * tsz * cpr / 32;
     if (fused_fin && !c->q_fin) {
         const size_t nfin = (size_t)g.planes * (q.nct_alloc / q.CT + 1);
         HIP_TRY(hipMalloc((void**)&c->q_fin, nfin * sizeof(unsigned int)));
         HIP_TRY(hipMemsetAsync(c->q_fin, 0, nfin * sizeof(unsigned int), s));
     }
-    if (fic_launch_sweep_q(c->b, c->q_pool, c->q_flat, c->q_rng, c->q_rngC, c->q_E, c->q_thg, g, ct_begin, ct_end, q.ndtiles, q.ndtiles_alloc,
+    if (fic_launch_sweep_q(c->b, c->q_pool, c->q_flat, own_frags ? nullptr : c->q_rng, c->q_rngC, c->q_E, c->q_thg, g, ct_begin, ct_end, q.ndtiles, q.ndtiles_alloc,
                            q.nct_alloc, tiles_per_chunk, nchunks, s, c->q_stats, c->opt_noflag, fused_fin ? &c->o : nullptr, c->q_fin,
                            r_begin, r_count))
         return fail(FIC_E_HIP, "k_sweep_q launch failed");
-    *nchunks_out = nchunks;
     c->last_tiles_per_chunk = tiles_per_chunk;
     return FIC_OK;
 }
@@ -605,14 +623,23 @@
     const int ntiles = tile1 - tile0;
     int nchunks = 1;
     int rc = FIC_OK;
-    bool fused_prep = false;
+    bool fused_prep = false, own_frags = false, small = false;
+    int q_tiles_per_chunk = 0;
     if (kind == 6) {
         const QShape q = q_shape(g);
-        fused_prep = fic_q_prep_fused(g, q.ndtiles_alloc, tile1 * (64 * g.NR) / 64 - tile0 * (64 * g.NR) / 64) != 0;
+        int fuse = c->opt_fuse;
+        if (fuse < 0) {
+            const char* env = getenv("FIC_Q_FUSE");
+            if (env && (env[0] == '0' || env[0] == '1') && env[1] == '\0') fuse = env[0] - '0';
+        }
+        fused_prep = fic_q_fuse_legal(g) && fuse != 0;
+        small = fused_prep && fic_q_prep_fused(g, q.ndtiles_alloc, tile1 * (64 * g.NR) / 64 - tile0 * (64 * g.NR) / 64) != 0;
+        q_chunks(c, tile0, tile1, &nchunks, &q_tiles_per_chunk);
+        own_frags = fused_prep && fic_q_own_frags(g, nchunks, q_tiles_per_chunk) != 0;
     }
     if (!fused_prep && fic_launch_scale(c->b.gray, c->b.scaled, g, s)) return fail(FIC_E_HIP, "k_scale launch failed");
     if (kind == 6) {
-        rc = q_prep(c, tile0, tile1, s);
+        rc = q_prep(c, tile0, tile1, s, fused_prep, own_frags);
     } else {
         if (fic_launch_pool(c->b.scaled, c->b.pool_pix, c->b.pool_st, c->b.pool_var, c->b.pool_s64, g, s))
             return fail(FIC_E_HIP, "k_pool launch failed");
@@ -631,7 +658,7 @@
         if (kind == 1) {
             if (fic_launch_sweep_generic(c->b, g, range_begin, range_count, s)) rc = fail(FIC_E_HIP, "k_sweep_generic launch failed");
         } else if (kind == 6) {
-            rc = q_sweep(c, tile0, tile1, s, &nchunks, fused_prep, range_begin, range_count);
+            rc = q_sweep(c, tile0, tile1, s, nchunks, q_tiles_per_chunk, fused_prep, own_frags, range_begin, range_count);
         } else if (kind == 5) {
             rc = d4_sweep(c, tile0, tile1 - tile0, s, &nchunks);
         } else if (kind >= 3) {
@@ -644,7 +671,9 @@
     if (rc != FIC_OK) return rc;
     c->last_chunks = nchunks;
     c->last_kind = kind;
-    c->last_fused = fused_prep ? 1 : 0;
+    c->last_fused = small ? 1 : 0;
+    c->last_fuse_bits = fused_prep ? (FIC_FUSE_PREP | FIC_FUSE_FINALIZE | (own_frags ? FIC_FUSE_RANGE_FRAGMENTS : 0)) : 0;
+    c->last_launches = kind == 6 ? (fused_prep ? 2 : 5) : 0;
     if (!fused_prep &&
         fic_launch_finalize(c->b, c->o, g, range_begin, range_count, s, (kind == 5 || kind == 6) ? 1 : 0)) return fail(FIC_E_HIP, "k_finalize launch failed");
     c->encoded_any = true;
@@ -739,6 +768,9 @@
     } else if (!strcmp(name, "q_shape")) {
         if (value < 0 || value > 2) return fail(FIC_E_ARGUMENT, "q_shape must be 0 (by pool size), 1 (16x16x32) or 2 (32x32x16)");
         c->g.q_shape = value;
+    } else if (!strcmp(name, "q_fuse")) {
+        if (value < -1 || value > 1) return fail(FIC_E_ARGUMENT, "q_fuse must be -1 (automatic), 0 (five launches) or 1 (two launches)");
+        c->opt_fuse = value;
     } else if (!strcmp(name, "q_eshift")) {
         if (value < -12 || value > 4) return fail(FIC_E_ARGUMENT, "q_eshift must be in -12..4");
         c->g.q_eshift = value;
@@ -898,8 +930,24 @@
     if (!out) return FIC_OK;
     if (capacity < (int64_t)bytes) return fail(FIC_E_CAPACITY, "fic_ctx_debug_q_host: %zu bytes needed", bytes);
     HIP_TRY(hipSetDevice(c->device));
+    if (which == 2 && c->q_rng_skipped) {
+        std::lock_guard<std::mutex> lk(c->mu);
+        int rc = q_rng_alloc(c, c->last_stream);
+        if (rc) return rc;
+        if (fic_launch_q_range_frags(c->b, c->q_rng, g, q.nct_alloc, c->last_stream)) return fail(FIC_E_HIP, "k_range_q8 launch failed");
+        c->q_rng_skipped = false;
+        src = c->q_rng;
+    }
     HIP_TRY(hipStreamSynchronize(c->last_stream));
     HIP_TRY(hipMemcpy(out, src, bytes, hipMemcpyDeviceToHost));
+    return FIC_OK;
+}
+
+int fic_ctx_last_launches(fic_ctx* c, int* launches, int* fuse_bits)
+{
+    if (!c) return fail(FIC_E_ARGUMENT, "fic_ctx_last_launches: null context");
+    if (launches) *launches = c->last_launches;
+    if (fuse_bits) *fuse_bits = c->last_fuse_bits;
     return FIC_OK;
 }
 
diff --git a/fractal-image-compression_amd/csrc/fic_internal.h b/fractal-image-compression_amd/csrc/fic_internal.h
--- a/fractal-image-compression_amd/csrc/fic_internal.h
+++ b/fractal-image-compression_amd/csrc/fic_internal.h
@@ -118,7 +118,10 @@
     hipStream_t last_stream = nullptr;
     hipStream_t own_stream = nullptr;
     int opt_sweep = 0, opt_chunks = 0, opt_time = 0, opt_noflag = 0;
+    int opt_fuse = -1;
     int last_chunks = 0, last_kind = 0, last_fused = 0, last_tiles_per_chunk = 0;
+    int last_launches = 0, last_fuse_bits = 0;
+    bool q_rng_skipped = false;
     std::vector<hipEvent_t> ev;
     double acc_ms = 0.0;
     int acc_n = 0;
diff --git a/fractal-image-compression_amd/csrc/fic_launch.h b/fractal-image-compression_amd/csrc/fic_launch.h
--- a/fractal-image-compression_amd/csrc/fic_launch.h
+++ b/fractal-image-compression_amd/csrc/fic_launch.h
@@ -139,13 +139,16 @@
 int fic_q_ct(int B);
 int fic_q_ctw_host(int B);
 int fic_q_prep_fused(const FicGeom& g, int ndtiles_alloc, int ngrp);
+int fic_q_fuse_legal(const FicGeom& g);
+int fic_q_own_frags(const FicGeom& g, int nchunks, int tiles_per_chunk);
+int fic_launch_q_range_frags(const FicBuffers& b, void* rngQ, const FicGeom& g, int nct_alloc, hipStream_t s);
 int fic_q_shape16(const FicGeom& g);
 int fic_q_multi_kind(int nchunks, int tiles_per_chunk);
 int fic_q_cols_per_range(int B, int n_iso);
 int fic_q_unroll(int B, int n_iso);
 int fic_q_resident(int B);
 int fic_launch_q_prep(const FicBuffers& b, void* poolQ, void* dflat, void* rngQ, void* rngC, void* rngE, void* theta_g,
-                      const FicGeom& g, int ndtiles_alloc, int nct_alloc, int grp0, int ngrp, hipStream_t s);
+                      const FicGeom& g, int ndtiles_alloc, int nct_alloc, int grp0, int ngrp, hipStream_t s, int fused);
 int fic_launch_sweep_q(const FicBuffers& b, const void* poolQ, const void* dflat, const void* rngQ, const void* rngC, const void* rngE,
                        void* theta_g, const FicGeom& g, int ct_begin, int ct_end, int ndtiles, int ndtiles_alloc,
                        int nct_alloc, int tiles_per_chunk, int nchunks, hipStream_t s, unsigned long long* stats = nullptr, int dbg_noflag = 0,
diff --git a/fractal-image-compression_amd/csrc/fic_q.hip b/fractal-image-compression_amd/csrc/fic_q.hip
--- a/fractal-image-compression_amd/csrc/fic_q.hip
+++ b/fractal-image-compression_amd/csrc/fic_q.hip
@@ -108,7 +108,11 @@
                     const int m = (int)(t2 & 0xffu) + (int)((t2 >> 8) & 0xffu) + (int)(b2 & 0xffu) + tap4;
                     w[x >> 2] |= (uint32_t)(m / 4) << (8 * (x & 3));
                 }
-                __builtin_memcpy(scaled_out + so, w, B);
+                constexpr int AB = B / 4;
+                if (ry < AB || r == g.Dh - 1) {
+                    if (c == g.Dw - 1) __builtin_memcpy(scaled_out + so, w, B);
+                    else __builtin_memcpy(scaled_out + so, w, AB);
+                }
             }
         }
         uint32_t sum = 0, sq = 0;
@@ -337,6 +341,20 @@
     }
 }
 
+__device__ __forceinline__ v4i q_fold8_f16(uint2 w, uint2 v, int rM, bool odd)
+{
+    int a[8];
+#pragma unroll
+    for (int u = 0; u < 8; u++) {
+        const int c0 = (int)(((u < 4 ? w.x : w.y) >> (8 * (u & 3))) & 0xffu);
+        const int c1 = (int)(((u < 4 ? v.y : v.x) >> (8 * (3 - (u & 3)))) & 0xffu);
+        a[u] = odd ? c0 - c1 : c0 + c1 - 2 * rM;
+    }
+    v4i r;
+#pragma unroll
+    for (int u = 0; u < 4; u++) r[u] = f16_pair((float)a[2 * u], (float)a[2 * u + 1]);
+    return r;
+}
 __device__ __forceinline__ void t4x4_bytes(uint32_t a, uint32_t b, uint32_t c, uint32_t d, uint32_t& o0, uint32_t& o1, uint32_t& o2, uint32_t& o3)
 {
     const uint32_t t0 = __builtin_amdgcn_perm(b, a, 0x06020400u), t1 = __builtin_amdgcn_perm(b, a, 0x07030501u);
@@ -401,7 +419,7 @@
         const int rM = (int)(S >> 6);
         if (part == 0) {
             s_rM[l] = rM;
-            if (j < g.Nr_pad) {
+            if (j < g.Nr_pad && rng_st != nullptr) {
                 const int ss = (int)Q - 2 * rM * (int)S + n * rM * rM;
                 const size_t o = (size_t)plane * g.Nr_pad + j;
                 FicRngStat st;
@@ -441,11 +459,12 @@
     const uint8_t* const cps = MODE == 0 ? blk : cpy;
     constexpr int cols = 64 * CPR;
     const int ct0 = (j0 * CPR) / 32;
-    for (int t = threadIdx.x; t < cols * 4; t += 256) {
+    for (int t = threadIdx.x; t < cols * 4 && rngC != nullptr; t += 256) {
         const int col = t >> 2, q = t & 3;
         if (j0 + col / CPR < g.Nr_pad)
             *(uint4*)(rngC + ((size_t)plane * g.Nr_pad * CPR + (size_t)j0 * CPR + col) * DW + 4 * q) = *(const uint4*)(cps + col * STR + 16 * q);
     }
+    if (rngQ == nullptr) return;
     for (int t = threadIdx.x; t < (cols / 32) * NK * 64; t += 256) {
         const int lane = t & 63, m = (t >> 6) % NK, ctl = (t >> 6) / NK;
         int c32, pos0;
@@ -455,25 +474,20 @@
         const int rM = s_rM[l];
         const bool real = j0 + l < g.Nr;
         const uint8_t* cp = cps + col * STR;
-        int a[8];
+        v4i v;
         if constexpr (MODE != 2) {
+            int a[8];
             const uint2 w = *(const uint2*)(cp + pos0);
 #pragma unroll
             for (int u = 0; u < 8; u++) a[u] = (int)(((u < 4 ? w.x : w.y) >> (8 * (u & 3))) & 0xffu) - rM;
+#pragma unroll
+            for (int u = 0; u < 4; u++) v[u] = f16_pair((float)a[2 * u], (float)a[2 * u + 1]);
         } else {
             const bool odd = m >= NK / 2;
             const int q0 = 16 * (odd ? m - NK / 2 : m) + 8 * h;
-            const uint2 w = *(const uint2*)(cp + q0), v = *(const uint2*)(cp + n - 8 - q0);
-#pragma unroll
-            for (int u = 0; u < 8; u++) {
-                const int c0 = (int)(((u < 4 ? w.x : w.y) >> (8 * (u & 3))) & 0xffu);
-                const int c1 = (int)(((u < 4 ? v.y : v.x) >> (8 * (3 - (u & 3)))) & 0xffu);
-                a[u] = odd ? c0 - c1 : c0 + c1 - 2 * rM;
-            }
-        }
-        v4i v;
-#pragma unroll
-        for (int u = 0; u < 4; u++) v[u] = real ? f16_pair((float)a[2 * u], (float)a[2 * u + 1]) : 0;
+            v = q_fold8_f16(*(const uint2*)(cp + q0), *(const uint2*)(cp + n - 8 - q0), rM, odd);
+        }
+        if (!real) v = v4i{0, 0, 0, 0};
         if (ct0 + ctl < nct_alloc) rngQ[((size_t)plane * nct_alloc + ct0 + ctl) * NK * 64 + (size_t)m * 64 + lane] = v;
     }
 }
@@ -687,28 +701,32 @@
 }
 
 template <int NK, int MODE>
-__device__ __forceinline__ void q_finalize_tail(const QArgs& A, int plane, int gx, int* s_wdone, int lane)
-{
-    (void)lane;
+__device__ __forceinline__ void q_finalize_tail(const QArgs& A, int plane, int gx, int* s_wdone, int lane, int ctw0)
+{
     if constexpr (QMode<MODE>::RGB) {
         return;
     } else {
         constexpr int CSHIFT = QMode<MODE>::CSHIFT, NISO = QMode<MODE>::NISO;
         constexpr int B = NK == 1 ? 4 : (NK == 4 ? 8 : 16);
-        constexpr int CT = FIC_Q_WPG * fic_q_ctw(NK);
+        constexpr int CTW = fic_q_ctw(NK), CT = FIC_Q_WPG * CTW;
         asm volatile("s_waitcnt vmcnt(0) lgkmcnt(0)" ::: "memory");
-        __syncthreads();
-        if (threadIdx.x == 0) {
-            unsigned int* cnt = A.fin_count + (size_t)plane * A.nctg + gx;
-            const int last = __hip_atomic_fetch_add(cnt, 1u, __ATOMIC_RELAXED, __HIP_MEMORY_SCOPE_AGENT) == (unsigned)A.nchunks - 1u;
-            if (last) __hip_atomic_store(cnt, 0u, __ATOMIC_RELAXED, __HIP_MEMORY_SCOPE_AGENT);
-            *s_wdone = last;
-        }
-        __syncthreads();
-        if (!*(volatile int*)s_wdone) return;
+        const bool own = A.nchunks == 1;
+        if (!own) {
+            __syncthreads();
+            if (threadIdx.x == 0) {
+                unsigned int* cnt = A.fin_count + (size_t)plane * A.nctg + gx;
+                const int last = __hip_atomic_fetch_add(cnt, 1u, __ATOMIC_RELAXED, __HIP_MEMORY_SCOPE_AGENT) == (unsigned)A.nchunks - 1u;
+                if (last) __hip_atomic_store(cnt, 0u, __ATOMIC_RELAXED, __HIP_MEMORY_SCOPE_AGENT);
+                *s_wdone = last;
+            }
+            __syncthreads();
+            if (!*(volatile int*)s_wdone) return;
+        } else if (ctw0 >= A.ct_end) {
+            return;
+        }
         const FicGeom& g = A.geom;
-        const int j0 = ((A.ct_begin + gx * CT) * 32) >> CSHIFT, nj = (CT * 32) >> CSHIFT;
-        for (int jj = (int)threadIdx.x; jj < nj; jj += 64 * FIC_Q_WPG) {
+        const int j0 = ((own ? ctw0 : A.ct_begin + gx * CT) * 32) >> CSHIFT, nj = ((own ? CTW : CT) * 32) >> CSHIFT;
+        for (int jj = own ? lane : (int)threadIdx.x; jj < nj; jj += own ? 64 : 64 * FIC_Q_WPG) {
             const int j = j0 + jj;
             if (j < A.r_begin || j >= A.r_end) continue;
             unsigned long long kk;
@@ -748,7 +766,7 @@
     if (dt1 > A.ndtiles_loop) dt1 = A.ndtiles_loop;
     __shared__ int s_wdone;
     if (dt0 >= A.ndtiles || ctw0 >= A.ct_end) {
-        if (A.fin_count) q_finalize_tail<NK, MODE>(A, plane, gx_, &s_wdone, lane);
+        if (A.fin_count) q_finalize_tail<NK, MODE>(A, plane, gx_, &s_wdone, lane, ctw0);
         return;
     }
     const unsigned long long clk0 = A.stats ? clock64() : 0ull, tick0 = A.stats ? wall_clock64() : 0ull;
@@ -764,7 +782,28 @@
     if (lane == 0) *myqn = 0u;
 
     v4i rb[CTW][NK];
-    {
+    if constexpr (FOLD && NK == 4 && !GFAST) {
+        if (A.rngQ == nullptr) {
+            const uint8_t* cb = (const uint8_t*)A.rngC + (size_t)plane * A.Nr_pad * (4 * 64);
+#pragma unroll
+            for (int ci = 0; ci < CTW; ci++) {
+                const int col = (ctw0 + ci) * 32 + jcol, j = col >> 2;
+                uint2 w0 = make_uint2(0u, 0u), w1 = w0, v0 = w0, v1 = w0;
+                int rM = 0;
+                if (j < A.Nr) {
+                    const uint8_t* cp = cb + (size_t)col * 64;
+                    w0 = *(const uint2*)(cp + 8 * half); v0 = *(const uint2*)(cp + 56 - 8 * half);
+                    w1 = *(const uint2*)(cp + 16 + 8 * half); v1 = *(const uint2*)(cp + 40 - 8 * half);
+                    rM = rst[j].rM;
+                }
+                rb[ci][0] = q_fold8_f16(w0, v0, rM, false);
+                rb[ci][1] = q_fold8_f16(w1, v1, rM, false);
+                rb[ci][2] = q_fold8_f16(w0, v0, rM, true);
+                rb[ci][3] = q_fold8_f16(w1, v1, rM, true);
+            }
+        }
+    }
+    if (!(FOLD && NK == 4 && !GFAST) || A.rngQ != nullptr) {
         const v4i* rp = A.rngQ + ((size_t)plane * A.nct_alloc + ctw0) * NK * 64 + lane;
 #pragma unroll
         for (int ci = 0; ci < CTW; ci++)
@@ -976,7 +1015,7 @@
             atomicAdd(&A.stats[6], 1ull);
         }
     }
-    if (A.fin_count) q_finalize_tail<NK, MODE>(A, plane, gx_, &s_wdone, lane);
+    if (A.fin_count) q_finalize_tail<NK, MODE>(A, plane, gx_, &s_wdone, lane, ctw0);
 }
 
 typedef float v4f __attribute__((ext_vector_type(4)));
@@ -1016,7 +1055,7 @@
     if (dt1 > A.ndtiles_loop) dt1 = A.ndtiles_loop;
     __shared__ int s_wdone;
     if (dt0 >= A.ndtiles || ctw0 >= A.ct_end) {
-        if (A.fin_count) q_finalize_tail<NK, 0>(A, plane, gx_, &s_wdone, lane);
+        if (A.fin_count) q_finalize_tail<NK, 0>(A, plane, gx_, &s_wdone, lane, ctw0);
         return;
     }
     const unsigned long long clk0 = A.stats ? clock64() : 0ull, tick0 = A.stats ? wall_clock64() : 0ull;
@@ -1186,7 +1225,7 @@
             atomicAdd(&A.stats[6], 1ull);
         }
     }
-    if (A.fin_count) q_finalize_tail<NK, 0>(A, plane, gx_, &s_wdone, lane);
+    if (A.fin_count) q_finalize_tail<NK, 0>(A, plane, gx_, &s_wdone, lane, ctw0);
 }
 
 template <int NK, int MODE, bool MULTI>
@@ -1265,12 +1304,26 @@
 {
     return (g.B == 8 && (long long)g.planes * (ndtiles_alloc + ngrp) <= 1024) ? 1 : 0;
 }
+int fic_q_fuse_legal(const FicGeom& g) { return g.B == 8 ? 1 : 0; }
+int fic_q_own_frags(const FicGeom& g, int nchunks, int tiles_per_chunk)
+{
+    return (g.B == 8 && fic_q_mode(g.B, g.n_iso) == 2 && fic_q_multi_kind(nchunks, tiles_per_chunk) != 2) ? 1 : 0;
+}
+int fic_launch_q_range_frags(const FicBuffers& b, void* rngQ, const FicGeom& g, int nct_alloc, hipStream_t s)
+{
+    if (g.B != 8 || fic_q_mode(g.B, g.n_iso) != 2) return (int)hipErrorInvalidValue;
+    hipLaunchKernelGGL(k_range_q8<2>, dim3(g.Nr_pad / 64, g.planes), dim3(256), 0, s, (const uint8_t*)b.gray, (FicRngStat*)nullptr,
+                       (float*)nullptr, (unsigned long long*)nullptr, (uint32_t*)nullptr, (v4i*)rngQ, (uint32_t*)nullptr, g, nct_alloc, 0, 0);
+    FIC_LAUNCH_CHECK();
+    return 0;
+}
 int fic_launch_q_prep(const FicBuffers& b, void* poolQ, void* dflat, void* rngQ, void* rngC, void* rngE, void* theta_g,
-                      const FicGeom& g, int ndtiles_alloc, int nct_alloc, int grp0, int ngrp, hipStream_t s)
+                      const FicGeom& g, int ndtiles_alloc, int nct_alloc, int grp0, int ngrp, hipStream_t s, int fused)
 {
     const int mode = fic_q_mode(g.B, g.n_iso);
     const int shape16 = fic_q_shape16(g);
-    if (fic_q_prep_fused(g, ndtiles_alloc, ngrp)) {
+    if (fused) {
+        if (!fic_q_fuse_legal(g)) return (int)hipErrorInvalidValue;
         auto pk = mode == 0 ? k_prep_q8<0> : k_prep_q8<2>;
         hipLaunchKernelGGL(pk, dim3(ndtiles_alloc + ngrp, g.planes), dim3(256), 0, s, (const uint8_t*)b.gray, b.scaled, b.pool_pix, b.pool_st,
                            b.pool_var, b.pool_s64, (v4i*)poolQ, (uint32_t*)dflat, b.rng_st, (float*)rngE, b.key, (uint32_t*)theta_g,
@@ -1320,6 +1373,7 @@
     A.rgb_rng = nullptr; A.rgb_pool = nullptr; A.rgb_dst = nullptr;
     if (ct_begin + A.nctg * CT > nct_alloc || g.Nd >= (1 << 24) || A.ndtiles_loop + unroll > ndtiles_alloc || tiles_per_chunk % unroll)
         return (int)hipErrorInvalidValue;
+    if (!rngQ && !fic_q_own_frags(g, nchunks, tiles_per_chunk)) return (int)hipErrorInvalidValue;
     dim3 grid((unsigned)(nchunks * g.planes) * (unsigned)A.nctg), block(64 * FIC_Q_WPG);
     const int mode = fic_q_mode(g.B, g.n_iso);
     if (!q_launch(g.B * g.B / 16, mode, fic_q_multi_kind(nchunks, tiles_per_chunk), grid, block, s, A, fic_q_shape16(g))) return (int)hipErrorInvalidValue;
diff --git a/fractal-image-compression_amd/host.py b/fractal-image-compression_amd/host.py
--- a/fractal-image-compression_amd/host.py
+++ b/fractal-image-compression_amd/host.py
@@ -125,7 +125,15 @@
         v = (C.c_int * 10)()
         capi.check(capi.lib().fic_ctx_info(self._h, v))
         keys = ["Rw", "Rh", "Nr", "Dw", "Dh", "Nd", "NR", "tiles", "chunks", "sweep_kind"]
-        return dict(zip(keys, list(v)))
+        d = dict(zip(keys, list(v)))
+        n, bits = C.c_int(), C.c_int()
+        if hasattr(capi.lib(), "fic_ctx_last_launches"):
+            capi.check(capi.lib().fic_ctx_last_launches(self._h, C.byref(n), C.byref(bits)))
+            d["launches"] = n.value
+            d["fused"] = [name for b, name in ((1, "prep"), (2, "finalize"), (4, "range_fragments")) if bits.value & b]
+        else:
+            d["launches"], d["fused"] = None, []
+        return d
 
     def results(self):
         P, N = self.planes, self.n_ranges
diff --git a/include/fic.h b/include/fic.h
--- a/include/fic.h
+++ b/include/fic.h
@@ -130,6 +130,10 @@
 FIC_API int fic_ctx_sweep_stats(fic_ctx* ctx, uint64_t* out8, int reset);
 FIC_API int fic_ctx_info(fic_ctx* ctx, int* out10);
 FIC_API int fic_ctx_last_kernel(fic_ctx* ctx, char* out, int capacity);
+#define FIC_FUSE_PREP 1
+#define FIC_FUSE_FINALIZE 2
+#define FIC_FUSE_RANGE_FRAGMENTS 4
+FIC_API int fic_ctx_last_launches(fic_ctx* ctx, int* launches, int* fuse_bits);
 FIC_API int fic_sweep_ranges_per_pool_read(int kind, int B, int n_iso);
 
 FIC_API int fic_debug_sqrt_f64(int device, uint32_t first, uint32_t count, double* out);
```

Result: no change. 138.5 million, median of 6 (+0.9%).
